# ntampellini/FIRECODE

Measured on AMD Instinct MI355X. Metric: conformer-pair RMSD alignments/s, higher is better.
Workload: dtype f64

## Files before the change

### firecode_amd/_lib.py

```python

from __future__ import annotations

import ctypes as C
import os

import numpy as np

_HERE = os.path.dirname(os.path.abspath(__file__))
LIB_PATH = os.environ.get("FC_LIB_PATH") or os.path.join(_HERE, "libfc_hip.so")

FC_OK = 0
FC_E_INVALID, FC_E_NODEVICE, FC_E_HIP, FC_E_NOMEM, FC_E_LIMIT = -1, -2, -3, -4, -5


class FirecodeHipError(RuntimeError):

    def __init__(self, code, message):
        super().__init__(f"libfc_hip error {code}: {message}")
        self.code = code


class FirecodeHipInputError(FirecodeHipError, ValueError):
    """FC_E_INVALID / FC_E_LIMIT: the arguments were rejected before any launch."""


class FirecodeHipDeviceError(FirecodeHipError):
    """FC_E_NODEVICE / FC_E_HIP / FC_E_NOMEM."""


_lib = None

_p_f64 = C.POINTER(C.c_double)
_p_i64 = C.POINTER(C.c_int64)
_p_u64 = C.POINTER(C.c_uint64)
_p_u8 = C.POINTER(C.c_uint8)
_i64 = C.c_int64
_f64 = C.c_double
_ens = C.c_void_p

_SIGNATURES = {
    "fc_abi_version": [],
    "fc_device_count": [],
    "fc_init": [C.c_int],
    "fc_shutdown": [],
    "fc_warmup": [],
    "fc_device_info": [C.c_char_p, _i64, _p_i64, _p_i64],
    "fc_ensemble_create": [_p_f64, _i64, _i64, _p_u8, C.c_int, C.POINTER(_ens)],
    "fc_ensemble_destroy": [_ens],
    "fc_ensemble_shape": [_ens, _p_i64, _p_i64],
    "fc_kabsch_rmsd_pairs": [_p_f64, _i64, _i64, _p_u8, _p_i64, _p_i64, _i64, C.c_int, _p_f64, _p_f64],
    "fc_ensemble_rmsd_pairs": [_ens, _p_i64, _p_i64, _i64, _p_f64, _p_f64],
    "fc_ensemble_rmsd_matrix": [_ens, _p_f64, _p_f64],
    "fc_ensemble_rmsd_values": [_ens, _p_f64, _p_f64],
    "fc_ensemble_rmsd_and_max_all": [_ens, _p_f64, _p_f64, _p_f64],
    "fc_bench_rmsd_and_max_all": [_ens, _i64, _p_f64, _p_f64, _p_i64],
    "fc_bench_rmsd_and_max_all_sampled": [_ens, _i64, _p_i64, _p_i64, _i64, _p_f64, _p_f64, _p_f64, _p_f64, _p_i64],
    "fc_bench_refine": [_ens, _f64, _f64, _i64, _p_f64, _p_i64],
    "fc_screen_select": [C.c_int],
    "fc_prune_conventions": [C.c_int],
    "fc_prune_similarity": [_p_f64, _i64, _i64, _p_u8, _p_f64, C.c_int, _f64, C.c_int, _f64, _f64, _p_f64, _f64, _i64,
                            _p_u8, _p_u8, _p_i64],
    "fc_alignment_matrices": [_p_f64, _p_f64, _i64, _i64, _p_f64],
    "fc_rmsd_simbits": [_ens, _f64, _f64, _p_f64, _f64, _i64, _i64, _p_u64, _p_i64],
    "fc_prune_rmsd": [_ens, _f64, _f64, _p_f64, _f64, _i64, _p_u8, _p_i64],
    "fc_prune_rmsd_host": [_p_f64, _i64, _i64, _p_u8, C.c_int, _f64, _f64, _p_f64, _f64, _i64, _p_u8, _p_i64],
    "fc_greedy_prune_from_bits": [_p_u64, _i64, _i64, _p_u8],
    "fc_prune_rmsd_begin": [_ens, _f64, _f64, _p_f64, _f64, _i64, _i64, _i64, _p_i64],
    "fc_prune_level": [_ens, _i64, _p_u8, _p_u8],
    "fc_prune_similar_pairs": [_ens, _p_u64, _i64, _p_i64],
    "fc_prune_from_pairs": [_ens, _p_u64, _i64, _i64, _p_u8],
    "fc_prune_rmsd_begin_async": [_ens, _f64, _f64, _i64, _i64, _i64],
    "fc_prune_export_pairs_dev": [_ens, C.c_void_p, _i64],
    "fc_prune_from_gathered_dev": [_ens, C.c_void_p, _i64, _i64, _i64, _p_u8, _p_i64],
    "fc_prune_from_gathered_dev_enqueue": [_ens, C.c_void_p, _i64, _i64, _i64, _i64, _i64],
    "fc_prune_collect": [_ens, _i64, _i64, _p_u8, _p_i64],
    "fc_stream_set": [C.c_void_p],
    "fc_memory_trim": [],
    "fc_host_alloc_pinned": [C.c_int64, C.POINTER(C.c_void_p)],
    "fc_host_free_pinned": [C.c_void_p],
    "fc_inertia_moments": [_p_f64, _i64, _i64, _p_f64, _p_f64],
    "fc_prune_rmsd_rot_corr": [_p_f64, _i64, _i64, _p_u8, _p_i64, _i64, _p_u8, _p_f64, C.POINTER(C.c_int32), _i64,
                               _f64, _f64, _p_f64, _f64, _i64, _p_u8, _p_u64],
    "fc_align_by_moi": [_p_f64, _i64, _i64, _p_f64, _p_f64],
    "fc_prune_moi": [_p_f64, _i64, _i64, _p_f64, _f64, _p_f64, _f64, _i64, _p_u8],
    "fc_align_to_first": [_p_f64, _i64, _i64, _p_i64, _i64, _p_f64],
    "fc_rototranslate": [_p_f64, _i64, _i64, _p_f64, _p_f64, _p_f64],
    "fc_clash_self": [_p_f64, _i64, _i64, _f64, _f64, _p_i64],
    "fc_clash_fragments": [_p_f64, _i64, _i64, _p_i64, _i64, _f64, _i64, _p_i64, _p_u8],
    "fc_clash_graph": [_p_f64, _i64, _i64, _p_u8, _f64, _p_i64],
    "fc_fitness_check": [_p_f64, _i64, _i64, _p_i64, _p_f64, _i64, _f64, _p_f64, _p_u8],
    "fc_embed_poses_clash": [_p_f64, _i64, _i64, _p_f64, _i64, _i64, _p_i64, _p_i64, _p_f64, _p_f64,
                             _p_f64, _p_f64, _i64, _f64, _i64, _p_i64, _p_u8, _p_f64],
    "fc_embed_mol_transforms": [_p_f64, _i64, _i64, _p_i64, _i64, _p_f64, _p_f64, _i64, _p_f64, _i64, _p_f64, _p_f64],
    "fc_embed_trimolecular": [C.POINTER(_p_f64), _p_i64, _p_i64, C.POINTER(_p_i64), _p_i64, _i64, _p_i64, _p_f64,
                              _p_f64, _p_f64, _p_f64, _p_u8, _p_i64, _p_f64, _p_f64, _i64, C.POINTER(C.c_int32),
                              _i64, _f64, _i64, _f64, _p_f64, _p_f64, _p_u8, _p_u8],
    "fc_embed_grid_clash": [_p_f64, _i64, _i64, _p_i64, _i64, _p_f64, _p_f64, _p_f64, _i64, _i64, _p_i64, _i64,
                            _p_f64, _p_f64, _p_f64, _i64, _p_f64, _i64, _f64, _i64, _p_u8,
                            C.POINTER(C.c_int32), _p_f64],
    "fc_embed_grid_dedupe": [_p_f64, _i64, _i64, _p_i64, _i64, _p_f64, _p_f64, _p_f64, _i64, _i64, _p_i64, _i64,
                             _p_f64, _p_f64, _p_f64, _i64, _p_f64, _i64, _f64, _i64, _f64, _p_u8, _p_u8],
    "fc_string_embed": [_p_f64, _i64, _i64, _p_f64, _p_f64, _i64, _p_f64, _i64, _i64, _p_f64, _p_f64, _i64, _p_f64, _i64,
                        _p_i64, _i64, _f64, _i64, _f64, _p_u8, _p_u8, _p_f64, _p_f64],
    "fc_torsion_scan": [_p_f64, _i64, _p_i64, _i64, _p_u8, _p_i64, _i64, _f64, _i64, _p_f64, _p_i64],
    "fc_torsion_scan_fingerprints": [_p_f64, _i64, _p_i64, _i64, _p_u8, _p_i64, _i64, _f64, _i64, _p_i64, _i64,
                                     _p_f64, _p_i64, _p_f64],
    "fc_torsion_scan_tfd": [_p_f64, _i64, _p_i64, _i64, _p_u8, _p_i64, _i64, _f64, _i64, _p_i64, _i64, _f64, _p_i64, _p_u8],
    "fc_torsion_scan_tfd_grid": [_p_f64, _i64, _p_i64, _i64, _p_u8, _p_i64, _p_i64, _f64, _i64, _p_i64, _i64, _f64, _p_i64, _p_u8],
    "fc_torsion_fingerprint": [_p_f64, _i64, _i64, _p_i64, _i64, _p_f64],
    "fc_tfd_simbits": [_p_f64, _i64, _i64, _f64, _i64, _i64, _p_u64],
    "fc_tfd_first_match": [_p_f64, _i64, _i64, _f64, _p_i64],
    "fc_tfd_ladder_from_first_match": [_p_i64, _i64, _p_u8],
    "fc_tfd_prune": [_p_f64, _i64, _i64, _f64, _p_u8],
    "fc_debug_pyset_order_ints": [_p_i64, _i64, _p_i64, _p_i64],
    "fc_debug_pyset_order_pairs": [_p_i64, _i64, _p_i64, _p_i64],
    "fc_debug_pyset_order_pairs_device": [_p_i64, _i64, _p_i64],
    "fc_debug_tfd_ladder_emulate": [_p_i64, _i64, _p_u8],
    "fc_xyz_write": [C.c_char_p, C.POINTER(C.c_char_p), _i64, _p_f64, _i64, C.c_char_p, C.c_int],
    "fc_xyz_scan": [C.c_char_p, _p_i64, _p_i64],
    "fc_cartesian_product_i64": [_p_i64, _p_i64, _i64, _p_i64],
    "fc_cartesian_product_f64": [_p_f64, _p_i64, _i64, _p_f64],
    "fc_xyz_read": [C.c_char_p, _i64, _i64, C.c_char_p, _p_f64],
    "fc_bench_prune_rmsd": [_ens, _f64, _f64, _i64, _p_f64, _p_f64, _p_u8, _p_i64],
    "fc_stream_use": [C.c_void_p],
    "fc_ensemble_twin": [_ens, C.POINTER(_ens)],
    "fc_prune_rmsd_begin_split_async": [_ens, _f64, _f64, _i64, _i64, _i64, C.c_void_p, C.c_int],
    "fc_screen_last_kind": [],
    "fc_debug_mfma_f16_model": [_i64, _p_i64, _p_f64],
    "fc_debug_h2_covariance": [_ens, _i64, _i64, C.POINTER(C.c_float), _p_f64, _p_f64],
    "fc_comm_unique_id": [_p_u8],
    "fc_comm_init": [_i64, _i64, _p_u8],
    "fc_comm_destroy": [],
    "fc_comm_info": [_p_i64, _p_i64],
    "fc_allgather_mask": [_p_u8, _i64, _p_u8],
    "fc_allgather_u8_dev": [C.c_void_p, C.c_void_p, _i64],
    "fc_comm_barrier": [],
    "fc_debug_comm_loopback": [_i64, _i64],
    "fc_prune_rmsd_sharded": [_ens, _f64, _f64, _i64, _i64, _p_u8, _p_i64],
    "fc_bench_prune_rmsd_sharded": [_ens, _f64, _f64, _i64, C.c_int, _p_f64, _p_f64, _p_u8, _p_i64],
    "fc_ensemble_select_diverse": [_ens, _i64, _i64, _f64, _p_i64, _p_f64, C.POINTER(C.c_int32), _p_f64, _p_i64],
    "fc_bench_select_diverse": [_ens, _i64, _i64, _f64, _i64, _p_f64, _p_f64, _p_i64, _p_i64, _p_i64],
    "fc_prune_rmsd_many": [C.POINTER(_ens), _i64, _f64, _f64, _i64, C.POINTER(_p_u8), _p_i64],
}

EXPORTED_SYMBOLS = tuple(_SIGNATURES) + ("fc_last_error",)


def _hip_runtime_mode():
    want = os.environ.get("FC_HIP_RUNTIME", "system")
    if want not in ("system", "torch", "auto"):
        raise FirecodeHipInputError(FC_E_INVALID, f"FC_HIP_RUNTIME={want!r}: expected 'system' or 'torch'")
    return "system" if want == "auto" else want


def _mapped_hip_runtimes():
    try:
        with open("/proc/self/maps") as fh:
            return sorted({ln.split()[-1] for ln in fh if "libamdhip64" in ln})
    except OSError:
        return []


HIP_RUNTIME = None


def _share_torch_hip_runtime():
    import importlib.util
    import sys

    mapped = _mapped_hip_runtimes()
    if "torch" in sys.modules:
        return mapped[0] if mapped else None
    try:
        spec = importlib.util.find_spec("torch")
    except (ImportError, ValueError):
        spec = None
    if spec is None or not spec.origin:
        raise FirecodeHipDeviceError(FC_E_NODEVICE, "FC_HIP_RUNTIME=torch but PyTorch is not installed")
    path = os.path.join(os.path.dirname(spec.origin), "lib", "libamdhip64.so")
    if mapped and os.path.realpath(mapped[0]) != os.path.realpath(path):
        raise FirecodeHipDeviceError(
            FC_E_NODEVICE, f"FC_HIP_RUNTIME=torch but {mapped[0]} is already mapped: a second HIP runtime "
            "in this process would see no GPU")
    if not os.path.exists(path):
        raise FirecodeHipDeviceError(FC_E_NODEVICE, f"FC_HIP_RUNTIME=torch but {path} does not exist")
    with open(path, "rb") as fh:
        if b"libamdhip64.so.7" not in fh.read():
            raise FirecodeHipDeviceError(
                FC_E_NODEVICE, f"{path} does not carry the soname libamdhip64.so.7 that libfc_hip.so binds to")
    C.CDLL(path, mode=C.RTLD_GLOBAL)
    return path


def load():
    global _lib, HIP_RUNTIME
    if _lib is not None:
        return _lib
    import sys

    mode = _hip_runtime_mode()
    if mode == "torch":
        _share_torch_hip_runtime()
    HIP_RUNTIME = "torch" if (mode == "torch" or "torch" in sys.modules) else "system"
    if not os.path.exists(LIB_PATH):
        raise FirecodeHipDeviceError(
            FC_E_NODEVICE,
            f"{LIB_PATH} is missing: build it with `python -c 'import __graft_entry__ as g; g.build()'` "
            "or `make -C firecode_amd/csrc`; firecode_amd has no CPU fallback",
        )
    lib = C.CDLL(LIB_PATH)
    for name, argtypes in _SIGNATURES.items():
        fn = getattr(lib, name)
        fn.argtypes = argtypes
        fn.restype = C.c_int
    lib.fc_last_error.argtypes = []
    lib.fc_last_error.restype = C.c_char_p
    _lib = lib
    return lib


def check(rc):
    if rc == FC_OK:
        return
    msg = load().fc_last_error().decode("utf-8", "replace")
    if rc in (FC_E_INVALID, FC_E_LIMIT):
        raise FirecodeHipInputError(rc, msg)
    raise FirecodeHipDeviceError(rc, msg)


def call(name, *args):
    check(getattr(load(), name)(*args))


def f64(a):
    return np.ascontiguousarray(a, dtype=np.float64)


def i64(a):
    return np.ascontiguousarray(a, dtype=np.int64)


def u8(a):
    return np.ascontiguousarray(a, dtype=np.uint8)


def ptr(a, ctype):
    if a is None:
        return None
    return a.ctypes.data_as(C.POINTER(ctype))


def pf(a):
    return ptr(a, C.c_double)


def pi(a):
    return ptr(a, C.c_int64)


def pb(a):
    return ptr(a, C.c_uint8)


def pw(a):
    return ptr(a, C.c_uint64)


def init(device=0):
    call("fc_init", int(device))


def shutdown():
    call("fc_shutdown")


def stream_set(hip_stream):
    call("fc_stream_set", C.c_void_p(int(hip_stream) if hip_stream else None))


def stream_use(hip_stream):
# ... 7 lines not shown
def screen_select(kind=0):
    call("fc_screen_select", int(kind))


def comm_unique_id():
    buf = np.zeros(128, dtype=np.uint8)
    call("fc_comm_unique_id", pb(buf))
    return buf.tobytes()


def comm_init(rank, world, unique_id):
    buf = np.frombuffer(bytes(unique_id), dtype=np.uint8).copy()
    if buf.shape[0] != 128:
        raise FirecodeHipInputError(FC_E_INVALID, "the RCCL unique id has 128 bytes")
    call("fc_comm_init", int(rank), int(world), pb(buf))


def comm_destroy():
    call("fc_comm_destroy")


def comm_info():
    r, w = C.c_int64(0), C.c_int64(1)
    call("fc_comm_info", C.byref(r), C.byref(w))
    return r.value, w.value


def comm_barrier():
    call("fc_comm_barrier")


def allgather_mask(mask_u8):
    m = u8(mask_u8).reshape(-1)
    _, world = comm_info()
    out = np.zeros((world, m.shape[0]), dtype=np.uint8)
    call("fc_allgather_mask", pb(m), int(m.shape[0]), pb(out))
    return out


def warmup():
    call("fc_warmup")


def memory_trim():
    call("fc_memory_trim")


def device_count():
    return int(load().fc_device_count())


def device_info():
    name = C.create_string_buffer(160)
    ncu, hbm = C.c_int64(0), C.c_int64(0)
    call("fc_device_info", name, 160, C.byref(ncu), C.byref(hbm))
    return {"name": name.value.decode(), "n_cu": ncu.value, "hbm_bytes": hbm.value}


class DeviceEnsemble:

    def __init__(self, coords, atom_mask=None, center=True):
        coords = f64(coords)
        if coords.ndim != 3 or coords.shape[2] != 3:
            raise FirecodeHipInputError(FC_E_INVALID, f"coords must be (N, A, 3), got {coords.shape}")
        self.N, self.A_all = int(coords.shape[0]), int(coords.shape[1])
        m = None if atom_mask is None else u8(np.asarray(atom_mask, dtype=bool))
        if m is not None and m.shape != (self.A_all,):
            raise FirecodeHipInputError(FC_E_INVALID, "atom_mask must have one entry per atom")
        self._h = _ens()
        call("fc_ensemble_create", pf(coords), self.N, self.A_all, pb(m), int(bool(center)), C.byref(self._h))
        self.W = (max(self.N, 1) + 63) // 64

    def close(self):
        if getattr(self, "_h", None):
            load().fc_ensemble_destroy(self._h)
            self._h = None

    def __del__(self):
        try:
            self.close()
        except Exception:
            pass

    def __enter__(self):
        return self

    def __exit__(self, *exc):
        self.close()

    @property
    def handle(self):
        if not self._h:
            raise FirecodeHipInputError(FC_E_INVALID, "ensemble already destroyed")
        return self._h

    def rmsd_pairs(self, pair_i, pair_j):
        pi_, pj_ = i64(pair_i), i64(pair_j)
        P = int(pi_.shape[0])
        r, m = np.empty(P), np.empty(P)
        call("fc_ensemble_rmsd_pairs", self.handle, pi(pi_), pi(pj_), P, pf(r), pf(m))
        return r, m

    def select_diverse(self, n_max, start=0, stop_rmsd=None):
        n_max, start = int(n_max), int(start)
        stop = -1.0 if stop_rmsd is None else float(stop_rmsd)
        if stop_rmsd is not None and not stop >= 0.0:
            raise FirecodeHipInputError(FC_E_INVALID, f"stop_rmsd={stop_rmsd!r} must be >= 0")
        cap = max(1, min(n_max, self.N))
        idx, rad = np.empty(cap, dtype=np.int64), np.empty(cap)
        lab, dist = np.empty(self.N, dtype=np.int32), np.empty(self.N)
        k = C.c_int64(0)
        call("fc_ensemble_select_diverse", self.handle, n_max, start, stop, pi(idx), pf(rad),
             ptr(lab, C.c_int32), pf(dist), C.byref(k))
        return idx[:k.value], lab, dist, rad[:k.value]

    def bench_select_diverse(self, n_max, start=0, stop_rmsd=None, reps=3):
        stop = -1.0 if stop_rmsd is None else float(stop_rmsd)
        idx = np.empty(max(1, min(int(n_max), self.N)), dtype=np.int64)
        dev, host, k, lanes = C.c_double(0), C.c_double(0), C.c_int64(0), C.c_int64(0)
        call("fc_bench_select_diverse", self.handle, int(n_max), int(start), stop, int(reps), C.byref(dev),
             C.byref(host), pi(idx), C.byref(k), C.byref(lanes))
        return dev.value, host.value, idx[:k.value], lanes.value

    def rmsd_matrix(self):
        r = np.zeros((self.N, self.N))
        m = np.zeros((self.N, self.N))
        call("fc_ensemble_rmsd_matrix", self.handle, pf(r), pf(m))
        return r, m

    def rmsd_values(self, want_matrix=True):
        r = np.zeros((self.N, self.N)) if want_matrix else None
        ms = C.c_double(0)
        call("fc_ensemble_rmsd_values", self.handle, pf(r), C.byref(ms))
        return r, ms.value

    def rmsd_and_max_all(self, want_matrices=True):
        r = np.zeros((self.N, self.N)) if want_matrices else None
        m = np.zeros((self.N, self.N)) if want_matrices else None
        ms = C.c_double(0)
        call("fc_ensemble_rmsd_and_max_all", self.handle, pf(r), pf(m), C.byref(ms))
        return r, m, ms.value

    def bench_refine(self, max_rmsd, max_dev, reps=10):
        ms, n = C.c_double(0), C.c_int64(0)
        call("fc_bench_refine", self.handle, float(max_rmsd), float(max_dev), int(reps), C.byref(ms), C.byref(n))
        return ms.value, n.value

    def bench_rmsd_and_max_all(self, reps=1):
        k, t = C.c_double(0), C.c_double(0)
        stats = np.zeros(3, dtype=np.int64)
        call("fc_bench_rmsd_and_max_all", self.handle, int(reps), C.byref(k), C.byref(t), pi(stats))
        return k.value, t.value, stats

    def bench_rmsd_and_max_all_sampled(self, pair_i, pair_j, reps=1):
        pi_, pj_ = i64(pair_i), i64(pair_j)
        P = int(pi_.shape[0])
        r, m = np.empty(P), np.empty(P)
        k, t = C.c_double(0), C.c_double(0)
        stats = np.zeros(3, dtype=np.int64)
        call("fc_bench_rmsd_and_max_all_sampled", self.handle, int(reps), pi(pi_), pi(pj_), P, pf(r), pf(m),
             C.byref(k), C.byref(t), pi(stats))
        return k.value, t.value, stats, r, m

    def simbits(self, max_rmsd, max_dev, energies=None, max_dE=0.0, row_begin=0, row_end=None):
        row_end = self.N if row_end is None else int(row_end)
        bits = np.zeros((row_end - row_begin, self.W), dtype=np.uint64)
        grey = C.c_int64(0)
        en = None if energies is None else f64(energies)
        call("fc_rmsd_simbits", self.handle, float(max_rmsd), float(max_dev), pf(en), float(max_dE),
             int(row_begin), row_end, pw(bits), C.byref(grey))
        return bits, grey.value

    def prune(self, max_rmsd, max_dev, energies=None, max_dE=0.0, min_per_group=20):
        mask = np.zeros(self.N, dtype=np.uint8)
        stats = np.zeros(6, dtype=np.int64)
        en = None if energies is None else f64(energies)
        call("fc_prune_rmsd", self.handle, float(max_rmsd), float(max_dev), pf(en), float(max_dE),
             int(min_per_group), pb(mask), pi(stats))
        return mask.astype(bool), stats

    def prune_begin(self, max_rmsd, max_dev, rank, world, row_block=128, energies=None, max_dE=0.0):
        stats = np.zeros(6, dtype=np.int64)
        en = None if energies is None else f64(energies)
        call("fc_prune_rmsd_begin", self.handle, float(max_rmsd), float(max_dev), pf(en), float(max_dE),
             int(rank), int(world), int(row_block), pi(stats))
        return stats

    def prune_level(self, k, mask_in):
        mi = u8(mask_in)
        mo = np.zeros(self.N, dtype=np.uint8)
        call("fc_prune_level", self.handle, int(k), pb(mi), pb(mo))
        return mo

    def similar_pairs(self, count_hint=None):
        n = C.c_int64(0)
        if count_hint is None:
            call("fc_prune_similar_pairs", self.handle, None, 0, C.byref(n))
            count_hint = n.value
        out = np.zeros(int(count_hint), dtype=np.uint64)
        call("fc_prune_similar_pairs", self.handle, pw(out), out.shape[0], C.byref(n))
        return out[: n.value]

    def prune_from_pairs(self, pairs, min_per_group=20):
        pairs = np.ascontiguousarray(pairs, dtype=np.uint64)
        mask = np.zeros(self.N, dtype=np.uint8)
        call("fc_prune_from_pairs", self.handle, pw(pairs), int(pairs.shape[0]), int(min_per_group), pb(mask))
        return mask.astype(bool)

    def prune_begin_async(self, max_rmsd, max_dev, rank, world, row_block=128):
        call("fc_prune_rmsd_begin_async", self.handle, float(max_rmsd), float(max_dev), int(rank), int(world),
             int(row_block))

    def prune_begin_split_async(self, max_rmsd, max_dev, rank, world, screen_stream, row_block=128, timed=True):
        call("fc_prune_rmsd_begin_split_async", self.handle, float(max_rmsd), float(max_dev), int(rank),
             int(world), int(row_block), C.c_void_p(int(screen_stream)), int(bool(timed)))

    def twin(self):
        t = getattr(self, "_twin", None)
        if t is None:
            h = _ens()
            call("fc_ensemble_twin", self.handle, C.byref(h))
            t = self._twin = _EnsembleView(self, h)
        return t

    def export_pairs_dev(self, dev_ptr, cap):
        call("fc_prune_export_pairs_dev", self.handle, C.c_void_p(int(dev_ptr)), int(cap))

    def prune_from_gathered_dev(self, dev_ptr, world, cap, min_per_group=20):
        mask = np.zeros(self.N, dtype=np.uint8)
        stats = np.zeros(6, dtype=np.int64)
        call("fc_prune_from_gathered_dev", self.handle, C.c_void_p(int(dev_ptr)), int(world), int(cap),
             int(min_per_group), pb(mask), pi(stats))
        return mask.astype(bool), stats

    def prune_from_gathered_enqueue(self, dev_ptr, world, cap, slot, n_slots, min_per_group=20):
        call("fc_prune_from_gathered_dev_enqueue", self.handle, C.c_void_p(int(dev_ptr)), int(world), int(cap),
             int(min_per_group), int(slot), int(n_slots))

    def prune_collect(self, slot, n_slots):
        mask = np.zeros(self.N, dtype=np.uint8)
        stats = np.zeros(6, dtype=np.int64)
        call("fc_prune_collect", self.handle, int(slot), int(n_slots), pb(mask), pi(stats))
        return mask.astype(bool), stats

    def prune_sharded(self, max_rmsd, max_dev, min_per_group=20, row_block=0):
        mask = np.zeros(self.N, dtype=np.uint8)
        stats = np.zeros(6, dtype=np.int64)
        call("fc_prune_rmsd_sharded", self.handle, float(max_rmsd), float(max_dev), int(min_per_group),
             int(row_block), pb(mask), pi(stats))
        return mask.astype(bool), stats

    def bench_prune_sharded(self, max_rmsd, max_dev, reps=1, overlap=True):
        mask = np.zeros(self.N, dtype=np.uint8)
        stats = np.zeros(8, dtype=np.int64)
        t_k, t_s = C.c_double(0), C.c_double(0)
        call("fc_bench_prune_rmsd_sharded", self.handle, float(max_rmsd), float(max_dev), int(reps),
             int(bool(overlap)), C.byref(t_k), C.byref(t_s), pb(mask), pi(stats))
        return t_k.value, t_s.value, mask.astype(bool), stats

    def bench_prune(self, max_rmsd, max_dev, reps=1, want_mask=True):
        mask = np.zeros(self.N, dtype=np.uint8) if want_mask else None
        stats = np.zeros(8, dtype=np.int64)
        t_k, t_s = C.c_double(0), C.c_double(0)
        call("fc_bench_prune_rmsd", self.handle, float(max_rmsd), float(max_dev), int(reps),
             C.byref(t_k), C.byref(t_s), pb(mask), pi(stats))
        return t_k.value, t_s.value, (None if mask is None else mask.astype(bool)), stats


class _EnsembleView(DeviceEnsemble):

    def __init__(self, parent, handle):
        self._parent = parent
        self._view_h = handle
        self.N, self.A_all, self.W = parent.N, parent.A_all, parent.W

    @property
    def handle(self):
        self._parent.handle
        return self._view_h

    def close(self):
        pass

    def twin(self):
        return self._parent


def prune_many(ensembles, max_rmsd, max_dev, min_per_group=20):
    n = len(ensembles)
    handles = (_ens * max(n, 1))(*[e.handle for e in ensembles])
    masks = [np.zeros(max(int(e.N), 1), dtype=np.uint8) for e in ensembles]
    ptrs = (_p_u8 * max(n, 1))(*[m.ctypes.data_as(_p_u8) for m in masks])
    survivors = np.zeros(max(n, 1), dtype=np.int64)
    call("fc_prune_rmsd_many", handles, n, float(max_rmsd), float(max_dev), int(min_per_group), ptrs,
         survivors.ctypes.data_as(_p_i64))
    return [m[: int(e.N)].astype(bool) for m, e in zip(masks, ensembles)], survivors[:n]


def unpack_bits(bits, n):
    b = np.unpackbits(bits.view(np.uint8), axis=1, bitorder="little")
    return b[:, :n].astype(bool)


def xyz_write(path, atoms, coords, label="", mode=0):
    X = f64(coords)
    if X.ndim == 2:
# ... 43 lines not shown
```

### firecode_amd/csrc/fc_api.cpp

```cpp
#include <algorithm>
#include <atomic>
#include <chrono>
#include <cmath>
#include <cstdlib>
#include <memory>

#include <map>
#include <mutex>
#include <thread>
#include "fc_common.h"
#include "fc_kabsch_math.h"

namespace fc {
struct LadderKs {
  int n;
  int64_t k[24];
};
__global__ void k_store_ladder_ks(LadderKs a, int64_t *__restrict__ out) {
  if ((int)threadIdx.x < a.n) out[threadIdx.x] = a.k[threadIdx.x];
}
}

namespace fc {

// ... 877 lines not shown
}

int fc_memory_trim(void) {
  FC_API_LOCK;
  if (ctx().ready) (void)hipStreamSynchronize(ctx().stream);
  pool_trim();
  return FC_OK;
}

int fc_host_alloc_pinned(int64_t bytes, void **out) {
  FC_API_LOCK;
  FC_REQUIRE(out != nullptr && bytes >= 0, "bad arguments");
  *out = nullptr;
  if (bytes == 0) return FC_OK;
  FC_TRY(ensure_init());
  void *p = nullptr;
  if (hipHostMalloc(&p, (size_t)bytes, hipHostMallocDefault) != hipSuccess) {
    (void)hipGetLastError();
    return set_error(FC_E_NOMEM, "hipHostMalloc of %lld bytes failed", (long long)bytes);
  }
  *out = p;
  return FC_OK;
}

int fc_host_free_pinned(void *p) {
  FC_API_LOCK;
  if (p == nullptr) return FC_OK;
  if (hipHostFree(p) != hipSuccess) return set_error(FC_E_HIP, "hipHostFree failed: %s", hipGetErrorString(hipGetLastError()));
  return FC_OK;
}

int fc_stream_set(void *hip_stream) {
  FC_API_LOCK;
  FC_TRY(ensure_init());
  Context &c = ctx();
  FC_HIP_TRY(hipStreamSynchronize(c.stream));
  c.stream = hip_stream ? static_cast<hipStream_t>(hip_stream) : c.own_stream;
  return FC_OK;
}

int fc_stream_use(void *hip_stream) {
  FC_API_LOCK;
  FC_TRY(ensure_init());
  Context &c = ctx();
  c.stream = hip_stream ? static_cast<hipStream_t>(hip_stream) : c.own_stream;
  return FC_OK;
}

int fc_device_info(char *name, int64_t name_len, int64_t *n_cu, int64_t *hbm_bytes) {
  FC_API_LOCK;
  FC_TRY(ensure_init());
  if (name && name_len > 0) std::snprintf(name, (size_t)name_len, "%s", ctx().name);
  if (n_cu) *n_cu = ctx().n_cu;
  if (hbm_bytes) *hbm_bytes = (int64_t)ctx().hbm;
  return FC_OK;
}

int fc_ensemble_create(const double *coords, int64_t N, int64_t A, const uint8_t *atom_mask,
                       int center, fc_ensemble **out) {
  FC_API_LOCK;
  FC_REQUIRE(out != nullptr, "out is NULL");
  *out = nullptr;
  FC_REQUIRE(coords != nullptr || N == 0, "coords is NULL");
  FC_REQUIRE(N >= 0 && A >= 1, "bad shape N=%lld A=%lld", (long long)N, (long long)A);
  FC_REQUIRE(A <= 32767, "A=%lld exceeds 32767 atoms", (long long)A);
  FC_TRY(ensure_init());
  std::unique_ptr<fc_ensemble> e(new (std::nothrow) fc_ensemble);
  if (!e) return set_error(FC_E_NOMEM, "host allocation failed");
  e->epoch = ctx().epoch;
  FC_TRY(ensemble_build(coords, N, A, atom_mask, center, e.get()));
  *out = e.release();
  return FC_OK;
}

int fc_ensemble_destroy(fc_ensemble *ens) {
  FC_API_LOCK;
  delete ens;
  return FC_OK;
}

int fc_ensemble_shape(const fc_ensemble *ens, int64_t *N, int64_t *A_selected) {
  FC_API_LOCK;
  FC_REQUIRE(ens != nullptr, "ens is NULL");
  if (N) *N = ens->N;
  if (A_selected) *A_selected = ens->A;
  return FC_OK;
}

int fc_ensemble_rmsd_pairs(fc_ensemble *ens, const int64_t *pair_i, const int64_t *pair_j,
                           int64_t P, double *rmsd_out, double *maxdev_out) {
  FC_API_LOCK;
  FC_REQUIRE(ens != nullptr, "ens is NULL");
  FC_REQUIRE(ens->epoch == ctx().epoch, "this ensemble was created before fc_shutdown / a device switch: create it again");
  FC_REQUIRE(P >= 0, "P < 0");
  if (P == 0) return FC_OK;
  FC_REQUIRE(pair_i && pair_j && rmsd_out && maxdev_out, "NULL pointer argument");
  for (int64_t k = 0; k < P; ++k)
    FC_REQUIRE(pair_i[k] >= 0 && pair_i[k] < ens->N && pair_j[k] >= 0 && pair_j[k] < ens->N,
               "pair %lld = (%lld, %lld) out of range [0, %lld)", (long long)k,
               (long long)pair_i[k], (long long)pair_j[k], (long long)ens->N);
  FC_TRY(ensure_init());
  DevBuf di, dj, dr, dm;
  FC_TRY(upload(di, pair_i, (size_t)P));
  FC_TRY(upload(dj, pair_j, (size_t)P));
  FC_TRY(dr.reserve((size_t)P * sizeof(double)));
  FC_TRY(dm.reserve((size_t)P * sizeof(double)));
  FC_TRY(launch_pairs_exact(ens, di.as<int64_t>(), dj.as<int64_t>(), P, dr.as<double>(),
                            dm.as<double>(), nullptr));
  FC_TRY(d2h(rmsd_out, dr.p, (size_t)P * sizeof(double)));
  FC_TRY(d2h(maxdev_out, dm.p, (size_t)P * sizeof(double)));
  return sync();
}

int fc_kabsch_rmsd_pairs(const double *coords, int64_t N, int64_t A, const uint8_t *atom_mask,
                         const int64_t *pair_i, const int64_t *pair_j, int64_t P, int center,
                         double *rmsd_out, double *maxdev_out) {
  FC_API_LOCK;
  fc_ensemble *e = nullptr;
  FC_TRY(fc_ensemble_create(coords, N, A, atom_mask, center, &e));
  const int rc = fc_ensemble_rmsd_pairs(e, pair_i, pair_j, P, rmsd_out, maxdev_out);
  fc_ensemble_destroy(e);
  return rc;
}

static bool rmsd_and_max_tiled(const fc_ensemble *ens) {
  const size_t lds_m = ((size_t)(((ens->A + 3) / 4 + 1) / 2) * 384 + 16 + 128) * sizeof(double) + 1024;
  return lds_m <= (size_t)160 * 1024 && (uint64_t)((ens->A + 3) / 4 * 4) * 3 * (uint64_t)ens->Npad < (1ull << 32);
}

static int rmsd_and_max_all(fc_ensemble *ens, double *rmsd_out, double *maxdev_out, double *ms_kernel) {
  FC_TRY(ensure_init());
  const int64_t N = ens->N;
  if (N == 0) return FC_OK;
  Context &c = ctx();
  DevBuf dr, dm;
  const size_t bytes = (size_t)N * N * sizeof(double);
  FC_TRY(dr.reserve(bytes));
  FC_TRY(dm.reserve(bytes));
  const bool tiled = rmsd_and_max_tiled(ens);
  unsigned long long cnt[16] = {0};
  if (tiled) {
    FC_TRY(ensemble_shard(ens, 0, 1, 256));
    FC_HIP_TRY(hipMemsetAsync(ens->counters.p, 0, 16 * sizeof(uint64_t), c.stream));
  } else {
    FC_HIP_TRY(hipMemsetAsync(dr.p, 0, bytes, c.stream));
    FC_HIP_TRY(hipMemsetAsync(dm.p, 0, bytes, c.stream));
  }
  FC_HIP_TRY(hipEventRecord(c.ev0, c.stream));
  if (tiled) FC_TRY(launch_rmsd_values(ens, 0.0, dr.as<double>(), dm.as<double>()));
  else FC_TRY(launch_matrix_exact(ens, dr.as<double>(), dm.as<double>()));
  FC_HIP_TRY(hipEventRecord(c.ev1, c.stream));
  if (tiled) FC_TRY(d2h(cnt, ens->counters.p, sizeof cnt));
  FC_TRY(sync());
  if (ms_kernel) {
    float ms = 0.f;
    FC_HIP_TRY(hipEventElapsedTime(&ms, c.ev0, c.ev1));
    *ms_kernel = ms;
  }
  if (tiled && cnt[6] > (unsigned long long)ens->pairq_cap) {
    FC_HIP_TRY(hipMemsetAsync(ens->counters.p, 0, 16 * sizeof(uint64_t), c.stream));
    FC_TRY(launch_rmsd_values(ens, 0.0, dr.as<double>(), dm.as<double>(), 0, 1, true));
    FC_TRY(d2h(cnt, ens->counters.p, sizeof cnt));
    FC_TRY(sync());
  }
  if (tiled && cnt[6] > (unsigned long long)ens->pairq_cap) {
    FC_HIP_TRY(hipMemsetAsync(dr.p, 0, bytes, c.stream));
    FC_HIP_TRY(hipMemsetAsync(dm.p, 0, bytes, c.stream));
    FC_TRY(launch_matrix_exact(ens, dr.as<double>(), dm.as<double>()));
  }
  if (rmsd_out) FC_TRY(launch_mirror_upper(dr.as<double>(), N));
  if (maxdev_out) FC_TRY(launch_mirror_upper(dm.as<double>(), N));
  if (rmsd_out) FC_TRY(d2h(rmsd_out, dr.p, bytes));
  if (maxdev_out) FC_TRY(d2h(maxdev_out, dm.p, bytes));
  return sync();
}

static int bench_rmsd_and_max_all(fc_ensemble *ens, int64_t reps, double *ms_kernel_mean, double *ms_total,
                                  int64_t *stats, const int64_t *sample_i = nullptr, const int64_t *sample_j = nullptr,
                                  int64_t P = 0, double *sample_rmsd = nullptr, double *sample_maxdev = nullptr) {
  FC_TRY(ensure_init());
  const int64_t N = ens->N;
  FC_REQUIRE(N >= 2, "needs at least two conformers");
  Context &c = ctx();
  DevBuf dr, dm;
  const size_t bytes = (size_t)N * N * sizeof(double);
  FC_TRY(dr.reserve(bytes));
  FC_TRY(dm.reserve(bytes));
  const bool tiled = rmsd_and_max_tiled(ens);
  const int64_t rank = comm_rank(), world = comm_world();
  FC_REQUIRE(tiled || world == 1, "structures beyond the tiled kernel are not sharded");
  if (tiled) FC_TRY(ensemble_shard(ens, 0, 1, 256));
  std::vector<hipEvent_t> &ev = c.ev_pool;
  while ((int64_t)ev.size() < 2 * reps + 2) {
    hipEvent_t e = nullptr;
    FC_HIP_TRY(hipEventCreate(&e));
    ev.push_back(e);
  }
  FC_HIP_TRY(hipEventRecord(ev[2 * reps], c.stream));
  for (int64_t r = 0; r < reps; ++r) {
    if (tiled) {
      FC_HIP_TRY(hipMemsetAsync(ens->counters.p, 0, 16 * sizeof(uint64_t), c.stream));
      FC_HIP_TRY(hipEventRecord(ev[2 * r], c.stream));
      c.mark_after_screen = ev[2 * r + 1];
      const int rc = launch_rmsd_values(ens, 0.0, dr.as<double>(), dm.as<double>(), rank, world);
      c.mark_after_screen = nullptr;
      FC_TRY(rc);
    } else {
      FC_HIP_TRY(hipEventRecord(ev[2 * r], c.stream));
      FC_TRY(launch_matrix_exact(ens, dr.as<double>(), dm.as<double>()));
      FC_HIP_TRY(hipEventRecord(ev[2 * r + 1], c.stream));
    }
  }
  FC_HIP_TRY(hipEventRecord(ev[2 * reps + 1], c.stream));
  unsigned long long cnt[16] = {0};
  if (tiled) FC_TRY(d2h(cnt, ens->counters.p, sizeof cnt));
  FC_TRY(sync());
  double sum = 0.0;
  for (int64_t r = 0; r < reps; ++r) {
    float ms = 0.f;
    FC_HIP_TRY(hipEventElapsedTime(&ms, ev[2 * r], ev[2 * r + 1]));
    sum += ms;
  }
  float tot = 0.f;
  FC_HIP_TRY(hipEventElapsedTime(&tot, ev[2 * reps], ev[2 * reps + 1]));
  if (ms_kernel_mean) *ms_kernel_mean = sum / (double)reps;
  if (ms_total) *ms_total = tot;
  if (stats) {
    int64_t own = 0;
    const int64_t nb = ceil_div(N, (int64_t)128);
    for (int64_t lb = 0, b; (b = global_block(lb, rank, world)) < nb; ++lb)
      for (int64_t i = b * 128; i < std::min<int64_t>(N, (b + 1) * 128); ++i) own += N - 1 - i;
    stats[0] = own;
    stats[1] = (int64_t)cnt[6];
    stats[2] = tiled ? 1 : 0;
  }
  if (tiled && cnt[6] > (unsigned long long)ens->pairq_cap)
    return set_error(FC_E_LIMIT, "%llu degenerate pairs exceed the fix-up queue (%lld)", cnt[6], (long long)ens->pairq_cap);
  if (P > 0) {
    DevBuf di, dj, sr, sm;
    FC_TRY(upload(di, sample_i, (size_t)P));
    FC_TRY(upload(dj, sample_j, (size_t)P));
    FC_TRY(sr.reserve((size_t)P * sizeof(double)));
    FC_TRY(sm.reserve((size_t)P * sizeof(double)));
    FC_TRY(launch_gather_matrix_pairs(dr.as<double>(), dm.as<double>(), N, di.as<int64_t>(), dj.as<int64_t>(), P,
                                      sr.as<double>(), sm.as<double>()));
    FC_TRY(d2h(sample_rmsd, sr.p, (size_t)P * sizeof(double)));
    FC_TRY(d2h(sample_maxdev, sm.p, (size_t)P * sizeof(double)));
    FC_TRY(sync());
  }
  return FC_OK;
}

static int select_diverse_checked(fc_ensemble *ens, int64_t n_max, int64_t start, double stop_rmsd, int64_t *indices_out,
                                  double *radii_out, int32_t *labels_out, double *dist_out, int64_t *n_selected,
                                  double *ms_device) {
  FC_REQUIRE(ens != nullptr, "ens is NULL");
  FC_REQUIRE(indices_out != nullptr && n_selected != nullptr, "indices_out / n_selected is NULL");
  FC_REQUIRE(n_max >= 1, "n_max=%lld < 1", (long long)n_max);
  FC_REQUIRE(!(stop_rmsd != stop_rmsd), "stop_rmsd is NaN");
  FC_REQUIRE(ens->epoch == ctx().epoch, "this ensemble was created before fc_shutdown / a device switch: create it again");
  *n_selected = 0;
  if (ens->N == 0) return FC_OK;
  FC_REQUIRE(start >= 0 && start < ens->N, "start=%lld outside [0, %lld)", (long long)start, (long long)ens->N);
  FC_REQUIRE(ens->N <= (int64_t)INT32_MAX - 256, "N=%lld: the selection indexes conformers with 32 bits", (long long)ens->N);
  FC_TRY(ensure_init());
  return select_diverse(ens, n_max, start, stop_rmsd, indices_out, radii_out, labels_out, dist_out, n_selected, ms_device);
}

int fc_ensemble_select_diverse(fc_ensemble *ens, int64_t n_max, int64_t start, double stop_rmsd, int64_t *indices_out,
                               double *radii_out, int32_t *labels_out, double *dist_out, int64_t *n_selected) {
  FC_API_LOCK;
  return select_diverse_checked(ens, n_max, start, stop_rmsd, indices_out, radii_out, labels_out, dist_out, n_selected,
                                nullptr);
}

int fc_bench_select_diverse(fc_ensemble *ens, int64_t n_max, int64_t start, double stop_rmsd, int64_t reps,
                            double *ms_device_mean, double *ms_host_mean, int64_t *indices_out, int64_t *n_selected,
                            int64_t *lanes_out) {
  FC_API_LOCK;
  FC_REQUIRE(reps >= 1 && reps <= 4096 && ms_device_mean && ms_host_mean, "bad arguments");
  double dev = 0.0, host = 0.0;
  for (int64_t r = 0; r < reps; ++r) {
    double ms = 0.0;
    const auto t0 = std::chrono::steady_clock::now();
    FC_TRY(select_diverse_checked(ens, n_max, start, stop_rmsd, indices_out, nullptr, nullptr, nullptr, n_selected, &ms));
    host += std::chrono::duration<double, std::milli>(std::chrono::steady_clock::now() - t0).count();
    dev += ms;
  }
  *ms_device_mean = dev / (double)reps;
  *ms_host_mean = host / (double)reps;
  if (lanes_out) *lanes_out = diverse_lanes(ens->N);
  return FC_OK;
}

int fc_ensemble_rmsd_matrix(fc_ensemble *ens, double *rmsd_out, double *maxdev_out) {
  FC_API_LOCK;
  FC_REQUIRE(ens && rmsd_out && maxdev_out, "NULL pointer argument");
  return rmsd_and_max_all(ens, rmsd_out, maxdev_out, nullptr);
}

int fc_ensemble_rmsd_and_max_all(fc_ensemble *ens, double *rmsd_out, double *maxdev_out, double *ms_kernel) {
  FC_API_LOCK;
  FC_REQUIRE(ens != nullptr, "ens is NULL");
  return rmsd_and_max_all(ens, rmsd_out, maxdev_out, ms_kernel);
}

int fc_bench_rmsd_and_max_all(fc_ensemble *ens, int64_t reps, double *ms_kernel_mean, double *ms_total,
                              int64_t *stats) {
  FC_API_LOCK;
  FC_REQUIRE(ens != nullptr && reps >= 1 && reps <= 4096, "bad arguments");
  return bench_rmsd_and_max_all(ens, reps, ms_kernel_mean, ms_total, stats);
}

int fc_bench_rmsd_and_max_all_sampled(fc_ensemble *ens, int64_t reps, const int64_t *pair_i, const int64_t *pair_j,
                                      int64_t P, double *rmsd_out, double *maxdev_out, double *ms_kernel_mean,
                                      double *ms_total, int64_t *stats) {
  FC_API_LOCK;
  FC_REQUIRE(ens != nullptr && reps >= 1 && reps <= 4096, "bad arguments");
  FC_REQUIRE(P >= 0 && (P == 0 || (pair_i && pair_j && rmsd_out && maxdev_out)), "NULL sample arrays");
  for (int64_t p = 0; p < P; ++p)
    FC_REQUIRE(pair_i[p] >= 0 && pair_i[p] < ens->N && pair_j[p] >= 0 && pair_j[p] < ens->N,
               "sample pair %lld out of range", (long long)p);
  return bench_rmsd_and_max_all(ens, reps, ms_kernel_mean, ms_total, stats, pair_i, pair_j, P, rmsd_out, maxdev_out);
}

int fc_ensemble_rmsd_values(fc_ensemble *ens, double *rmsd_out, double *ms_kernel) {
  FC_API_LOCK;
  FC_REQUIRE(ens != nullptr, "ens is NULL");
  FC_TRY(ensure_init());
  const int64_t N = ens->N;
  if (N == 0) return FC_OK;
  FC_TRY(ensemble_shard(ens, 0, 1, 256));
  Context &c = ctx();
  DevBuf dr;
  const size_t bytes = (size_t)N * N * sizeof(double);
  FC_TRY(dr.reserve(bytes));
  FC_HIP_TRY(hipMemsetAsync(dr.p, 0, bytes, c.stream));
  FC_HIP_TRY(hipMemsetAsync(ens->counters.p, 0, 16 * sizeof(uint64_t), c.stream));
  FC_HIP_TRY(hipEventRecord(c.ev0, c.stream));
  FC_TRY(launch_rmsd_values(ens, 0.02, dr.as<double>(), nullptr));
  FC_HIP_TRY(hipEventRecord(c.ev1, c.stream));
  unsigned long long cnt[16];
  FC_TRY(d2h(cnt, ens->counters.p, sizeof cnt));
  if (rmsd_out) {
    FC_TRY(launch_mirror_upper(dr.as<double>(), N));
    FC_TRY(d2h(rmsd_out, dr.p, bytes));
  }
  FC_TRY(sync());
  if (cnt[6] > (unsigned long long)ens->pairq_cap)
    return set_error(FC_E_LIMIT, "%llu pairs closer than 0.02 A exceed the fix-up queue (%lld): "
                     "use fc_ensemble_rmsd_matrix", cnt[6], (long long)ens->pairq_cap);
  if (ms_kernel) {
    float ms = 0.f;
    FC_HIP_TRY(hipEventElapsedTime(&ms, c.ev0, c.ev1));
    *ms_kernel = ms;
  }
  return FC_OK;
}

int fc_alignment_matrices(const double *p, const double *q, int64_t n_pairs, int64_t A,
                          double *M_out) {
  FC_API_LOCK;
  FC_REQUIRE(n_pairs >= 0 && A >= 1, "bad shape");
  if (n_pairs == 0) return FC_OK;
  FC_REQUIRE(p && q && M_out, "NULL pointer argument");
  FC_TRY(ensure_init());
  DevBuf dp, dq, dM;
  FC_TRY(upload(dp, p, (size_t)n_pairs * A * 3));
  FC_TRY(upload(dq, q, (size_t)n_pairs * A * 3));
// ... 1587 lines not shown
    c.stream = overlap ? c.s_lane[k & 1] : home;
    const bool timed = k % stride_ev == 0;
    FC_TRY(begin_split(e, max_rmsd, max_dev, rank, world, row_block, overlap ? c.s_screen : c.stream,
                       timed ? ev[2 * k] : nullptr, timed ? ev[2 * k + 1] : nullptr));
    FC_TRY(fc_prune_export_pairs_dev(e, e->msg_send.as<uint64_t>(), cap));
    FC_TRY(comm_allgather_dev(e->msg_send.p, e->msg_recv.p, (size_t)(cap + 1) * sizeof(uint64_t), (int)(k & 1)));
    FC_TRY(fc_prune_from_gathered_dev_enqueue(e, e->msg_recv.as<uint64_t>(), world, cap, min_per_group, k, steps));
  }
  c.stream = home;
  if (overlap)
    for (hipStream_t s : {c.s_lane[0], c.s_lane[1], c.s_screen}) {
      FC_HIP_TRY(hipEventRecord(ev[2 * steps + 2], s));
      FC_HIP_TRY(hipStreamWaitEvent(home, ev[2 * steps + 2], 0));
    }
  FC_HIP_TRY(hipEventRecord(ev_end, home));
  FC_HIP_TRY(hipEventSynchronize(ev_end));
  if (total_ms) {
    float t = 0.f;
    FC_HIP_TRY(hipEventElapsedTime(&t, ev_begin, ev_end));
    *total_ms = t;
  }
  if (screen_ms_mean) {
    double sum = 0.0;
    int64_t n_timed = 0;
    for (int64_t k = 0; k < steps; k += stride_ev) {
      float a = 0.f;
      FC_HIP_TRY(hipEventElapsedTime(&a, ev[2 * k], ev[2 * k + 1]));
      sum += a;
      ++n_timed;
    }
    *screen_ms_mean = sum / (double)std::max<int64_t>(n_timed, 1);
  }
  return FC_OK;
}

static int64_t owned_pairs(const fc_ensemble *ens) {
  int64_t n = 0;
  const int64_t nb = ceil_div(ens->N, ens->row_block);
  for (int64_t lb = 0, b; (b = global_block(lb, ens->rank, ens->world)) < nb; ++lb)
    for (int64_t i = b * ens->row_block; i < std::min(ens->N, (b + 1) * ens->row_block); ++i) n += ens->N - 1 - i;
  return n;
}

static int sharded_levels_fallback(fc_ensemble *ens, double max_rmsd, double max_dev, int64_t min_per_group,
                                   int64_t row_block, uint8_t *mask_out, int64_t *stats) {
  const int64_t rank = comm_rank(), world = comm_world(), N = ens->N;
  int64_t st[6] = {0};
  FC_TRY(fc_prune_rmsd_begin(ens, max_rmsd, max_dev, nullptr, 0.0, rank, world, row_block, st));
  std::vector<uint8_t> mask((size_t)N, 1), mine((size_t)N), all((size_t)N * (size_t)world);
  for (int64_t k : kLadder) {
    int64_t alive = 0;
    for (uint8_t m : mask) alive += m;
    if (!(k == 1 || min_per_group * k < alive)) continue;
    FC_TRY(fc_prune_level(ens, k, mask.data(), mine.data()));
    FC_TRY(fc_allgather_mask(mine.data(), N, all.data()));
    for (int64_t i = 0; i < N; ++i) {
      uint8_t m = 1;
      for (int64_t r = 0; r < world; ++r) m = std::min(m, all[(size_t)r * N + i]);
      mask[(size_t)i] = m;
    }
  }
  int64_t alive = 0;
  for (int64_t i = 0; i < N; ++i) {
    mask_out[i] = mask[(size_t)i];
    alive += mask[(size_t)i];
  }
  if (stats) {
    for (int k = 0; k < 5; ++k) stats[k] = st[k];
    stats[5] = alive;
  }
  return FC_OK;
}

static int sharded_collect(fc_ensemble *ens, int64_t steps, bool overlap, uint8_t *mask_out, int64_t *stats,
                           bool *all_ok, int64_t *units = nullptr) {
  const int64_t W = ens->W;
  *all_ok = true;
  int64_t survivors = 0;
  for (int64_t k = 0; k < steps; ++k)
    if (!ladder_collect(ens, k, k == steps - 1 ? mask_out : nullptr, nullptr, &survivors, nullptr)) *all_ok = false;
  if (*all_ok && stats) {
    const unsigned long long *local = static_cast<const unsigned long long *>(ctx().pinned) +
                                      (size_t)steps * (size_t)(W + 16) + (size_t)(steps - 1) * 8;
    stats[0] = owned_pairs(ens);
    stats[1] = (int64_t)local[1];
    stats[2] = (int64_t)local[2];
    stats[3] = (int64_t)local[3];
    stats[4] = 0;
    stats[5] = survivors;
  }
  (void)overlap;
  if (*all_ok && units) {
    const uint64_t *cnt_last = static_cast<const uint64_t *>(ctx().pinned) + (size_t)(steps - 1) * (size_t)(W + 16) + W;
    units[0] = (int64_t)cnt_last[13];
    units[1] = (int64_t)cnt_last[15];
  }
  return FC_OK;
}

extern "C" {

int fc_prune_rmsd_sharded(fc_ensemble *ens, double max_rmsd, double max_dev, int64_t min_per_group,
                          int64_t row_block, uint8_t *mask_out, int64_t *stats) {
  FC_API_LOCK;
  FC_REQUIRE(ens && mask_out, "NULL pointer argument");
  FC_REQUIRE(max_rmsd > 0.0 && max_dev > 0.0 && min_per_group >= 1, "bad arguments");
  FC_TRY(ensure_init());
  if (ens->N == 0) return FC_OK;
  if (row_block <= 0) row_block = default_row_block();
  bool ok = false;
  const int64_t world = comm_world();
  const int64_t cap = 1024 + 4 * ens->N / world;
  const bool device_path = (uint64_t)world * (uint64_t)cap <= kPairLadderCap && (size_t)2 * ens->W * sizeof(uint64_t) <= 60 * 1024;
  if (device_path) {
    double ms = 0.0;
    FC_TRY(sharded_pipeline(ens, 1, max_rmsd, max_dev, min_per_group, row_block, false, &ms, nullptr));
    FC_TRY(sharded_collect(ens, 1, false, mask_out, stats, &ok));
    if (ok && stats) stats[4] = (int64_t)(ms * 1e6);
  }
  if (!ok) FC_TRY(sharded_levels_fallback(ens, max_rmsd, max_dev, min_per_group, row_block, mask_out, stats));
  return FC_OK;
}

int fc_bench_prune_rmsd_sharded(fc_ensemble *ens, double max_rmsd, double max_dev, int64_t reps, int overlap,
                                double *ms_screen_kernel, double *ms_step, uint8_t *mask_out, int64_t *stats) {
  FC_API_LOCK;
  FC_REQUIRE(ens && reps >= 1 && reps <= 1024, "bad arguments");
  FC_REQUIRE(max_rmsd > 0.0 && max_dev > 0.0, "thresholds must be positive");
  FC_TRY(ensure_init());
  FC_REQUIRE(ens->N > 0, "empty ensemble");
  const int64_t row_block = default_row_block();
  double ms = 0.0, total = 0.0;
  FC_TRY(sharded_pipeline(ens, reps, max_rmsd, max_dev, 20, row_block, overlap != 0, &ms, &total));
  bool ok = false;
  std::vector<uint8_t> scratch;
  if (!mask_out) {
    scratch.resize((size_t)ens->N);
    mask_out = scratch.data();
  }
  if (stats) stats[6] = stats[7] = 0;
  FC_TRY(sharded_collect(ens, reps, overlap != 0, mask_out, stats, &ok, stats ? stats + 6 : nullptr));
  if (!ok) FC_TRY(sharded_levels_fallback(ens, max_rmsd, max_dev, 20, row_block, mask_out, stats));
  if (ms_screen_kernel) *ms_screen_kernel = ms;
  if (ms_step) *ms_step = total / (double)reps;
  return FC_OK;
}

}

extern "C" {

int fc_screen_last_kind(void) { return last_screen_kind(); }

int fc_prune_conventions(int drop_later) {
  FC_API_LOCK;
  prune_conventions_set(drop_later);
  return FC_OK;
}

int fc_debug_mfma_f16_model(int64_t trials, int64_t *flags_out, double *worst_out) {
  FC_API_LOCK;
  FC_REQUIRE(flags_out && worst_out && trials >= 0 && trials <= (1 << 24), "NULL output or trials outside 0..2^24");
  FC_TRY(ensure_init());
  return h2_model_report(trials, flags_out, worst_out);
}

int fc_debug_h2_covariance(fc_ensemble *ens, int64_t ib, int64_t jb, float *B_out, double *scale_out, double *entry_bound_out) {
  FC_API_LOCK;
  FC_REQUIRE(ens && B_out && scale_out && entry_bound_out, "NULL argument");
  FC_REQUIRE(ib >= 0 && jb >= 0 && ib % 16 == 0 && jb % 16 == 0 && ib + 16 <= ens->Npad && jb + 16 <= ens->Npad,
             "tile origin must be a multiple of 16 inside the padded ensemble");
  FC_TRY(ensure_init());
  FC_REQUIRE(ens->epoch == ctx().epoch, "ensemble belongs to a context that was shut down");
  double scale = 0.0;
  FC_TRY(ensure_h2_operands(ens, &scale));
  *scale_out = scale;
  const int64_t KS2 = (ens->A + 31) / 32;
  *entry_bound_out = kabsch_h2_entry_bound(KS2);
  if (scale == 0.0) return FC_OK;
  DevBuf out;
  FC_TRY(out.reserve(256 * 9 * sizeof(float)));
  FC_TRY(launch_h2_cov_tile(ens, ib, jb, out.as<float>()));
  FC_TRY(d2h(B_out, out.p, 256 * 9 * sizeof(float)));
  return sync();
}

int fc_screen_select(int kind) {
  FC_API_LOCK;
  FC_REQUIRE(kind == 0 || kind == 16 || kind == 32 || kind == 64, "kind must be 0 (automatic), 16, 32 or 64");
  screen_select(kind);
  return FC_OK;
}

int fc_bench_refine(fc_ensemble *ens, double max_rmsd, double max_dev, int64_t reps, double *ms_refine,
                    int64_t *n_candidates) {
  FC_API_LOCK;
  FC_REQUIRE(ens && reps >= 1 && reps <= 4096, "bad arguments");
  FC_TRY(ensure_init());
  FC_TRY(ensemble_shard(ens, 0, 1, default_row_block()));
  Context &c = ctx();
  ens->lean = true;
  FC_HIP_TRY(hipMemsetAsync(ens->counters.p, 0, kCounters * sizeof(uint64_t), c.stream));
  FC_TRY(launch_simbits_screen(ens, max_rmsd * max_rmsd + kScreenMargin));
  {
    unsigned long long h0[8] = {0};
    FC_TRY(d2h(h0, ens->counters.p, sizeof h0));
    FC_TRY(sync());
    note_candidates(ens, h0[6], ens->last_similar < 0 ? 0 : (unsigned long long)ens->last_similar);
  }
  std::vector<hipEvent_t> &ev = c.ev_pool;
  while ((int64_t)ev.size() < 2 * reps) {
    hipEvent_t e = nullptr;
    FC_HIP_TRY(hipEventCreate(&e));
    ev.push_back(e);
  }
  auto *cnt = reinterpret_cast<unsigned long long *>(ens->counters.p);
  for (int64_t r = 0; r < reps; ++r) {
    FC_HIP_TRY(hipMemsetAsync(cnt + 1, 0, 3 * sizeof(uint64_t), c.stream));
    FC_HIP_TRY(hipEventRecord(ev[2 * r], c.stream));
    FC_TRY(launch_simbits_refine(ens, max_rmsd, max_dev, nullptr, 0.0));
    FC_HIP_TRY(hipEventRecord(ev[2 * r + 1], c.stream));
  }
  unsigned long long h[32] = {0};
  FC_TRY(d2h(h, ens->counters.p, sizeof h));
  FC_TRY(sync());
  if (getenv("FC_DEBUG") && h[22])
    fprintf(stderr, "[fc] refine buckets: %llu wave-items, %llu with pairs; mean ticks (100 MHz) staging %.1f, compute %.1f\n", h[22], h[23],
            (double)h[20] / (double)h[22], (double)h[21] / (double)h[22]);
  if (getenv("FC_DEBUG") && h[27])
    fprintf(stderr, "[fc] refine buckets, wave 0 per item (%llu rounds): covariance pass %.1f ticks, polynomial + rotation %.1f, + deviation pass %.1f\n",
            h[27], (double)h[26] / (double)h[27], (double)h[24] / (double)h[27], (double)h[25] / (double)h[27]);
  double sum = 0.0;
  for (int64_t r = 0; r < reps; ++r) {
    float ms = 0.f;
    FC_HIP_TRY(hipEventElapsedTime(&ms, ev[2 * r], ev[2 * r + 1]));
    sum += ms;
  }
  if (ms_refine) *ms_refine = sum / (double)reps;
  if (n_candidates) *n_candidates = (int64_t)h[1];
  if (h[6] > (unsigned long long)ens->pairq_cap)
    return set_error(FC_E_LIMIT, "the candidate-pair queue overflowed (%llu > %lld): this probe times the pair refine only",
                     h[6], (long long)ens->pairq_cap);
  return FC_OK;
}

int fc_bench_prune_rmsd(fc_ensemble *ens, double max_rmsd, double max_dev, int64_t reps,
                        double *ms_simbits_kernel, double *ms_step, uint8_t *mask_out,
                        int64_t *stats) {
  FC_API_LOCK;
  FC_REQUIRE(ens && reps >= 1 && reps <= 4096, "bad arguments");
  FC_TRY(ensure_init());
  FC_TRY(ensemble_shard(ens, 0, 1, default_row_block()));
  static const bool two_lanes = [] {
    const char *v = getenv("FC_BENCH_LANES");
    return !(v && atoi(v) == 1);
  }();
  const bool lanes = two_lanes && reps > 1;
  const int64_t stride = ens->W + 16;
  fc_ensemble *ws[kPruneLanes] = {ens, ens, ens};
  if (lanes) {
    const bool fresh = !ens->twin || !ens->twin->twin;
    for (int l = 1; l < kPruneLanes; ++l) FC_TRY(ensemble_twin(ws[l - 1], &ws[l]));
    if (fresh) FC_TRY(prune_pipeline(ws, kPruneLanes, max_rmsd, max_dev, 20, false, stride, nullptr, nullptr));
  }
  std::vector<fc_ensemble *> work((size_t)reps);
  for (int64_t r = 0; r < reps; ++r) work[(size_t)r] = ws[lanes ? r % kPruneLanes : 0];
  double t_kernel = 0.0, total = 0.0;
  FC_TRY(prune_pipeline(work.data(), reps, max_rmsd, max_dev, 20, lanes, stride, &t_kernel, &total));
  int64_t levels = 0, survivors = 0;
  unsigned long long cnt[8] = {0};
  bool redo = false;
  for (int64_t r = 0; r < reps; ++r)
    if (!ladder_collect(ens, r, mask_out, &levels, &survivors, cnt, stride)) redo = true;
  Context &c = ctx();
  if (redo) {
    ens->lean = false;
    FC_HIP_TRY(hipMemsetAsync(ens->counters.p, 0, kCounters * sizeof(uint64_t), c.stream));
    FC_TRY(launch_simbits_screen(ens, max_rmsd * max_rmsd + kScreenMargin));
    FC_TRY(launch_simbits_refine(ens, max_rmsd, max_dev, nullptr, 0.0));
    FC_TRY(ladder_single(ens, ens->bits.as<uint64_t>(), 20, mask_out, &levels, &survivors, cnt,
                         ens->simq.as<uint64_t>(), false, true));
  }
  if (getenv("FC_DEBUG")) {
    const uint64_t *cnt_host = static_cast<const uint64_t *>(c.pinned) + (size_t)(reps - 1) * (size_t)stride + ens->W;
    fprintf(stderr, "[fc] bench prune: candidates %llu, similar %llu, screen units the subset stage queued: %llu\n",
            (unsigned long long)cnt_host[1], (unsigned long long)cnt_host[2], (unsigned long long)cnt_host[13]);
  }
  if (ms_simbits_kernel) *ms_simbits_kernel = t_kernel;
  if (ms_step) *ms_step = total / (double)reps;
  if (stats) {
    stats[0] = ens->N * (ens->N - 1) / 2;
    stats[1] = (int64_t)cnt[1];
    stats[2] = (int64_t)cnt[2];
    stats[3] = (int64_t)cnt[3];
    stats[4] = levels;
    stats[5] = survivors;
    const uint64_t *cnt_last = static_cast<const uint64_t *>(c.pinned) + (size_t)(reps - 1) * (size_t)stride + ens->W;
    stats[6] = redo ? 0 : (int64_t)cnt_last[13];
    stats[7] = redo ? 0 : (int64_t)cnt_last[15];
  }
  return FC_OK;
}

}
```

### firecode_amd/csrc/fc_common.h

```cpp
#pragma once

#include <hip/hip_runtime.h>

#include <cstdarg>
#include <cstdint>
#include <cstdio>
#include <cstring>
#include <mutex>
#include <new>
#include <string>
#include <vector>

#include "../../include/fc_hip.h"
#include "fc_tuning.h"

namespace fc {

std::string &last_error();
int set_error(int code, const char *fmt, ...);

#define FC_HIP_TRY(expr)                                                              \
  do {                                                                                \
    hipError_t _e = (expr);                                                           \
    if (_e != hipSuccess)                                                             \
// ... 71 lines not shown
inline DevArena *&thread_arena() {
  static thread_local DevArena *a = nullptr;
  return a;
}

struct DevBuf {
  void *p = nullptr;
  size_t bytes = 0;
  uint64_t epoch = 0;
  bool owned = true;
  DevBuf() = default;
  DevBuf(const DevBuf &) = delete;
  DevBuf &operator=(const DevBuf &) = delete;
  ~DevBuf() { release(); }
  void release() {
    if (p && owned) {
      if (ctx().ready && epoch == ctx().epoch) pool_give(p, bytes);
      else (void)hipFree(p);
    }
    p = nullptr;
    bytes = 0;
    owned = true;
  }
  void alias(const DevBuf &o) {
    release();
    p = o.p;
    bytes = o.bytes;
    epoch = o.epoch;
    owned = false;
  }
  int reserve(size_t n, bool any_larger = false) {
    if (n <= bytes && p) return FC_OK;
    release();
    if (n == 0) n = 8;
    if (DevArena *a = thread_arena()) {
      if (void *q = a->take(n)) {
        p = q;
        bytes = (n + 255) & ~(size_t)255;
        epoch = ctx().epoch;
        owned = false;
        return FC_OK;
      }
    }
    size_t cap = 0;
    p = pool_take(n, &cap, any_larger);
    if (!p) return set_error(FC_E_NOMEM, "device allocation of %zu bytes failed", n);
    bytes = cap;
    epoch = ctx().epoch;
    return FC_OK;
  }
  template <class T>
  T *as() const { return static_cast<T *>(p); }
};

struct ArenaScope {
  DevBuf block;
  DevArena arena;
  DevArena *prev = nullptr;
  bool active = false;
  int begin(size_t bytes) {
    prev = thread_arena();
    thread_arena() = nullptr;
    const int rc = block.reserve(bytes, true);
    if (rc != FC_OK) {
      thread_arena() = prev;
      return rc;
    }
    arena.base = static_cast<char *>(block.p), arena.size = block.bytes, arena.used = 0;
    thread_arena() = &arena;
    active = true;
    return FC_OK;
  }
  ~ArenaScope();
};

inline hipStream_t &thread_stream_override() {
  static thread_local hipStream_t s = nullptr;
  return s;
}
inline hipStream_t cur_stream() {
  hipStream_t s = thread_stream_override();
  return s ? s : ctx().stream;
}
inline ArenaScope::~ArenaScope() {
  if (!active) return;
  thread_arena() = prev;
  if (ctx().ready) (void)hipStreamSynchronize(cur_stream());
}

constexpr size_t kStagedCopyMin = (size_t)64 << 10;
#ifndef FC_RB_COLSHIFT
#define FC_RB_COLSHIFT 6
#endif
constexpr int kBucketColShift = FC_RB_COLSHIFT;
#ifndef FC_RB_ROWS
#define FC_RB_ROWS 1024
#endif
constexpr int kBucketRows = FC_RB_ROWS;
bool host_memory_is_pinned(const void *p);
bool staged_uploads();
int h2d_staged(void *dst_dev, const void *src, size_t n, hipStream_t st);
inline int h2d(void *dst, const void *src, size_t n) {
  if (n == 0) return FC_OK;
  if (n >= kStagedCopyMin && staged_uploads() && !host_memory_is_pinned(src)) return h2d_staged(dst, src, n, cur_stream());
  FC_HIP_TRY(hipMemcpyAsync(dst, src, n, hipMemcpyHostToDevice, cur_stream()));
  return FC_OK;
}
inline int d2h(void *dst, const void *src, size_t n) {
  if (n == 0) return FC_OK;
  if (n >= kStagedCopyMin && !host_memory_is_pinned(dst)) return d2h_staged(dst, src, n, cur_stream());
  FC_HIP_TRY(hipMemcpyAsync(dst, src, n, hipMemcpyDeviceToHost, cur_stream()));
  return FC_OK;
}
inline int sync() {
  FC_HIP_TRY(hipStreamSynchronize(cur_stream()));
  return FC_OK;
}
inline int check_launch(const char *what) {
  hipError_t e = hipGetLastError();
  if (e != hipSuccess) return set_error(FC_E_HIP, "launch of %s failed: %s", what, hipGetErrorString(e));
  return FC_OK;
}

inline int64_t ceil_div(int64_t a, int64_t b) { return (a + b - 1) / b; }

constexpr double kScreenMargin = 1e-6;
constexpr unsigned long long kRefineLanesMin = 1ull << 17;

constexpr size_t kCounters = 64 + 20 * 16;
constexpr int kCntLevel = 64, kCntLevelStride = 16;

__host__ __device__ inline int64_t global_block(int64_t local_block, int64_t rank, int64_t world) {
  return local_block * world + ((local_block & 1) ? (world - 1 - rank) : rank);
}
inline int64_t local_block_count(int64_t n_gblocks, int64_t rank, int64_t world) {
  int64_t n = 0;
  while (global_block(n, rank, world) < n_gblocks) ++n;
  return n;
}

}

struct fc_ensemble {
  uint64_t epoch = 0;
  int64_t N = 0, A = 0;
  int64_t Npad = 0, W = 0;
  fc::DevBuf Xs;
  fc::DevBuf Xa;
  fc::DevBuf G;
  fc::DevBuf Xsf;
  fc::DevBuf sub;
  fc::DevBuf unitq;
  bool xsf_valid = false;
  fc::DevBuf Xh;
  bool xh_valid = false;
  double xh_scale = 0.0;
  double g_max = -1.0;
  bool g_max_pending = false;
  std::vector<int32_t> sel_host;
  fc::DevBuf bits;
  fc::DevBuf cand;
  fc::DevBuf pairq;
  int64_t pairq_cap = 0;
  fc::DevBuf simq;
  fc::DevBuf bk, bk_off, bk_list, sortq;
  int64_t bk_buckets = 0;
  int64_t last_candidates = -1;
  int64_t last_similar = -1;
  fc::DevBuf bits_full;
  fc::DevBuf item_table;
  int64_t item_key[4] = {-1, -1, -1, -1}, item_total = 0;
  std::vector<uint64_t> item_host;
  fc::DevBuf gathered;
  fc::DevBuf msg_send, msg_recv;
  fc::DevBuf energies;
  fc::DevBuf maskA, maskB;
  fc::DevBuf mbits;
  fc::DevBuf ladder;
  fc::DevBuf ladder_k;
  fc::DevBuf levelmask;
  std::vector<int64_t> ladder_k_host;
  int ladder_k_n = -1;
  int64_t ladder_k_mpg = -1;
  fc::DevBuf counters;
  int64_t rank = 0, world = 1, row_block = 64;
  int64_t rows_local = 0;
  bool bits_valid = false;
  bool lean = false;
  fc_ensemble *twin = nullptr;
  fc_ensemble *head = nullptr;
  fc_ensemble() = default;
  fc_ensemble(const fc_ensemble &) = delete;
  fc_ensemble &operator=(const fc_ensemble &) = delete;
  ~fc_ensemble() { delete twin; }
};
```

### firecode_amd/csrc/fc_kabsch.hip

```cpp
#include <type_traits>

#include "fc_common.h"
#include <vector>
#include "fc_kabsch_math.h"

#include <algorithm>
#include <cstdlib>

namespace fc {

static constexpr size_t kLdsLimit = 160 * 1024;

__global__ void __launch_bounds__(256)
k_prep(const double *__restrict__ coords, int64_t N, int64_t A_all, const int32_t *__restrict__ sel,
       int64_t A, int center, int64_t Npad, double *__restrict__ Xs, double *__restrict__ G,
       double *__restrict__ Xa, unsigned long long *__restrict__ gmax_bits,
       const int32_t *__restrict__ conf_idx) {
  const int64_t n = (int64_t)blockIdx.x * blockDim.x + threadIdx.x;
  if (n >= Npad) return;
  for (int64_t a = A; a < ((A + 3) & ~(int64_t)3); ++a) {
    Xs[(a * 3 + 0) * Npad + n] = 0.0;
    Xs[(a * 3 + 1) * Npad + n] = 0.0;
    Xs[(a * 3 + 2) * Npad + n] = 0.0;
  }
// ... 372 lines not shown
  if (lane == 0) scnt[2] = (unsigned)__popcll(m);
  return;
#endif
  const unsigned n = (unsigned)__popcll(m);
  unsigned base = 0;
  if (lane == 0) base = atomicAdd(scnt, n);
  base = (unsigned)__builtin_amdgcn_readfirstlane((int)base);
  if (base + n <= (unsigned)CAP) {
    if (may) sq[base + (unsigned)__popcll(m & ((1ull << lane) - 1ull))] = ((uint64_t)i << 32) | (uint64_t)j;
  } else {
#ifndef FC_ABLATE_OVERFLOW
    push_pairs(m, may, i, j, pairq, Q, counters, lane);
#endif
  }
}

template <int WCAP>
__device__ __forceinline__ void stage_pairs_wave(uint64_t m, bool may, unsigned i, unsigned j, uint64_t *__restrict__ sq_wave,
                                                 int &n_staged, uint64_t *__restrict__ pairq, unsigned long long Q,
                                                 unsigned long long *__restrict__ counters, int lane) {
  if (m == 0) return;
  const int n = (int)__popcll(m);
  if (n_staged + n <= WCAP) {
    if (may) sq_wave[n_staged + (int)__popcll(m & ((1ull << lane) - 1ull))] = ((uint64_t)i << 32) | (uint64_t)j;
    n_staged += n;
  } else {
    push_pairs(m, may, i, j, pairq, Q, counters, lane);
  }
}

__device__ __forceinline__ void flush_pairs_wave32(const uint32_t *__restrict__ sq_wave, int n_staged, unsigned i0, unsigned j0,
                                                   uint64_t *__restrict__ pairq, unsigned long long Q,
                                                   unsigned long long *__restrict__ counters, int lane) {
  if (n_staged == 0) return;
  unsigned long long base = 0;
  if (lane == 0) base = atomicAdd(&counters[6], (unsigned long long)n_staged);
  base = __shfl(base, 0);
  for (int idx = lane; idx < n_staged; idx += 64) {
    const uint32_t e = sq_wave[idx];
    const unsigned long long slot = base + (unsigned long long)idx;
    if (slot < Q) pairq[slot] = ((uint64_t)(i0 + (e >> 6)) << 32) | (uint64_t)(j0 + (e & 63u));
  }
}
template <int WCAP>
__device__ __forceinline__ void stage_pairs_wave32(uint64_t m, bool may, unsigned i, unsigned j, unsigned i0, unsigned j0,
                                                   uint32_t *__restrict__ sq_wave, int &n_staged,
                                                   uint64_t *__restrict__ pairq, unsigned long long Q,
                                                   unsigned long long *__restrict__ counters, int lane) {
  if (m == 0) return;
  const int n = (int)__popcll(m);
  if (n > WCAP) {
    push_pairs(m, may, i, j, pairq, Q, counters, lane);
    return;
  }
  if (n_staged + n > WCAP) {
    flush_pairs_wave32(sq_wave, n_staged, i0, j0, pairq, Q, counters, lane);
    n_staged = 0;
  }
  if (may) sq_wave[n_staged + (int)__popcll(m & ((1ull << lane) - 1ull))] = ((i - i0) << 6) | (j - j0);
  n_staged += n;
}

template <bool USE_LDS, int TI, int NW>
__global__ void __launch_bounds__(NW * 64)
k_simbits_screen(const double *__restrict__ Xs, const double *__restrict__ G, int64_t N,
                 int64_t Npad, int A, double A_thr2, int IB, int64_t rank, int64_t world,
                 uint64_t *__restrict__ bits, int64_t W, uint32_t *__restrict__ cand,
                 unsigned long long *__restrict__ counters, uint64_t *__restrict__ pairq,
                 unsigned long long Q) {
  extern __shared__ double lds[];
  const int tid = threadIdx.x;
  const int lane = tid & 63;
  const int wv = __builtin_amdgcn_readfirstlane(tid >> 6);
  const int64_t jt = blockIdx.x;
  const int64_t lb = blockIdx.y;
  const int64_t gb = global_block(lb, rank, world);
  const int64_t i0 = gb * IB;
  if (i0 >= N) return;
  if (jt * 64 + 63 <= i0) return;
  const int64_t j = jt * 64 + lane;

  if (USE_LDS) {
    const int total = A * 3 * 64;
    for (int idx = tid; idx < total; idx += NW * 64) {
      const int ac = idx >> 6, l = idx & 63;
      lds[idx] = Xs[(int64_t)ac * Npad + jt * 64 + l];
    }
    __syncthreads();
  }
  const double Gq = G[j];
  const double *__restrict__ xq = Xs + jt * 64 + lane;

  for (int it = wv; it * TI < IB; it += NW) {
    const int64_t ib = i0 + (int64_t)it * TI;
    if (ib >= N) break;
    if (jt * 64 + 63 <= ib) break;
    double acc[TI][9];
#pragma unroll
    for (int k = 0; k < TI; ++k)
#pragma unroll
      for (int e = 0; e < 9; ++e) acc[k][e] = 0.0;

    const double *__restrict__ xp = Xs + ib;
#pragma unroll 2
    for (int a = 0; a < A; ++a) {
      double qx, qy, qz;
      if (USE_LDS) {
        qx = lds[(a * 3 + 0) * 64 + lane];
        qy = lds[(a * 3 + 1) * 64 + lane];
        qz = lds[(a * 3 + 2) * 64 + lane];
      } else {
        qx = xq[(int64_t)(a * 3 + 0) * Npad];
        qy = xq[(int64_t)(a * 3 + 1) * Npad];
        qz = xq[(int64_t)(a * 3 + 2) * Npad];
      }
      const double *__restrict__ px = xp + (int64_t)(a * 3 + 0) * Npad;
      const double *__restrict__ py = xp + (int64_t)(a * 3 + 1) * Npad;
      const double *__restrict__ pz = xp + (int64_t)(a * 3 + 2) * Npad;
#pragma unroll
      for (int k = 0; k < TI; ++k) {
        const double x = px[k], y = py[k], z = pz[k];
        acc[k][0] = fma(x, qx, acc[k][0]);
        acc[k][1] = fma(x, qy, acc[k][1]);
        acc[k][2] = fma(x, qz, acc[k][2]);
        acc[k][3] = fma(y, qx, acc[k][3]);
        acc[k][4] = fma(y, qy, acc[k][4]);
        acc[k][5] = fma(y, qz, acc[k][5]);
        acc[k][6] = fma(z, qx, acc[k][6]);
        acc[k][7] = fma(z, qy, acc[k][7]);
        acc[k][8] = fma(z, qz, acc[k][8]);
      }
    }
#pragma unroll
    for (int k = 0; k < TI; ++k) {
      const int64_t i = ib + k;
      const double Gp = G[i];
      bool may = kabsch_may_be_below(acc[k], Gp + Gq, A_thr2);
      may = may && (j > i) && (j < N) && (i < N);
      const uint64_t word = __ballot(may);
      push_pairs(word, may, (unsigned)i, (unsigned)j, pairq, Q, counters, lane);
      if (lane == 0 && i < N) {
        const int64_t lrow = (int64_t)(lb * IB) + (int64_t)it * TI + k;
        bits[lrow * W + jt] = word;
        if (word) {
          const unsigned long long slot = atomicAdd(&counters[4], 1ull);
          cand[slot] = (uint32_t)(lrow * W + jt);
        }
      }
    }
  }
}

typedef double d4_t __attribute__((ext_vector_type(4)));

template <int NW, int MODE = 0, int TC = 64, bool EIG = false>
__global__ void __launch_bounds__(NW * 64, 2)
k_simbits_screen_mfma(const double *__restrict__ Xs, const double *__restrict__ G, int64_t N,
                      int64_t Npad, int A, double A_thr2, int IB, int64_t rank, int64_t world,
                      uint64_t *__restrict__ bits, int64_t W, uint32_t *__restrict__ cand,
                      unsigned long long *__restrict__ counters, uint64_t *__restrict__ pairq,
                      unsigned long long Q, const uint64_t *__restrict__ item_table, unsigned long long n_items,
                      double *__restrict__ rmsd_out = nullptr, const unsigned long long *__restrict__ gate = nullptr,
                      double *__restrict__ maxdev_out = nullptr) {
  static_assert(!EIG || MODE == 2, "EIG: the complete alignments");
  constexpr bool VALUES = MODE != 0;
  constexpr int NT = MODE == 2 ? 1 : 2;
  static_assert(TC == 64 || ((TC == 32 || TC == 16) && MODE == 2), "column tiles: 64, or 32 / 16 for the complete alignments");
  constexpr int NU = (TC / 16) / NT;
  constexpr int KPR = TC == 64 ? 2 : 4;
  constexpr int SST = 2048 / TC;
  constexpr int CST = TC == 64 ? 256 : 128;
  auto koff = [](int sl) { return TC == 16 ? (sl >> 1) * 384 + (sl & 1) * 64 : sl * (12 * TC); };
  if (gate != nullptr && *gate == 0ull) return;
  extern __shared__ double lds[];
  const int tid = threadIdx.x;
  const int lane = tid & 63;
  const int wv = __builtin_amdgcn_readfirstlane(tid >> 6);
  const int KS = (A + 3) >> 2;
  double *__restrict__ ldsG = lds + (TC == 16 ? ((KS + 1) >> 1) * 384 : KS * 12 * TC);
  uint64_t *__restrict__ stageQ = reinterpret_cast<uint64_t *>(ldsG + TC + IB);
  uint32_t *__restrict__ stageW = reinterpret_cast<uint32_t *>(stageQ + kStagePairs);
  unsigned *__restrict__ stageN = reinterpret_cast<unsigned *>(stageW + kStageWords);
#ifdef FC_TIMELINE
  unsigned long long *tl = reinterpret_cast<unsigned long long *>(rmsd_out);
#endif
  const unsigned long long b = blockIdx.x;
  if (b >= n_items) return;
#ifdef FC_TIMELINE
  if (!VALUES && tl && tid == 0) {
    tl[(size_t)b * 4] = wall_clock64();
    tl[(size_t)b * 4 + 3] = b;
  }
#endif
  int64_t jt, lb;
  int it_first = 0, it_last = IB >> 4;
  if (item_table != nullptr) {
    const uint64_t it = item_table[b];
    lb = (int64_t)((it >> 32) & 0x7fffffffull);
    jt = (int64_t)(it & 0x7fffffffull);
    if (it & (1ull << 31)) it_last = IB >> 5;
    if (it & (1ull << 63)) it_first = IB >> 5;
  } else {
    const int64_t NT = Npad / TC;
    jt = (int64_t)(b % (unsigned long long)NT);
    lb = (int64_t)(b / (unsigned long long)NT);
  }
  const int64_t j0 = jt * TC;
  const int64_t i0 = global_block(lb, rank, world) * IB;
  if (i0 >= N) return;
  if (j0 + TC - 1 <= i0) return;
  uint32_t *__restrict__ sq32_wave = reinterpret_cast<uint32_t *>(stageQ) + wv * (kStagePairs * 2 / NW);
  int n_staged32 = 0;
  (void)sq32_wave;
  (void)n_staged32;

  {
    const int n_runs = TC == 64 ? KS * 6 : (TC == 32 ? KS * 3 : ((KS + 1) >> 1) * 3);
    const int cs_l = TC == 64 ? lane >> 4 : lane >> 5, k1_l = TC == 64 ? (lane >> 3) & 1 : (lane >> 3) & 3, c15_l = (lane & 7) * 2;
    for (int q = wv; q < n_runs; q += NW) {
      const int sc = TC == 64 ? q >> 1 : q, kh = TC == 64 ? q & 1 : 0;
      const int sg = sc / 3, c = sc - sg * 3;
      int a = sg * 4 + kh * 2 + k1_l;
      if (TC == 16) {
        a = (sg * 2 + cs_l) * 4 + k1_l;
        a = a < KS * 4 ? a : KS * 4 - 1;
      }
      const double *src = Xs + (int64_t)(a * 3 + c) * Npad + j0 + (TC == 16 ? 0 : cs_l * 16) + c15_l;
      __builtin_amdgcn_global_load_lds((const __attribute__((address_space(1))) void *)src,
                                       (__attribute__((address_space(3))) void *)(lds + q * 128), 16, 0, 0);
    }
    for (int idx = tid; idx < TC + IB; idx += NW * 64) {
      const int64_t g = idx < TC ? j0 + idx : i0 + (idx - TC);
      ldsG[idx] = g < Npad ? G[g] : 0.0;
    }
    if (tid < kStagePairs) stageQ[tid] = ~0ull;
    if (tid < kStageWords) stageW[tid] = ~0u;
    if (tid < 2) stageN[tid] = 0u;
    __syncthreads();
#ifdef FC_TIMELINE
    if (!VALUES && tl && tid == 0) tl[(size_t)b * 4 + 1] = wall_clock64();
#endif
  }
  const int kq = lane >> 4, l15 = lane & 15;
  const int lcol = MODE == 2 ? 4 * (l15 & 3) + (l15 >> 2) : l15;
  const int boff = (kq / KPR) * 128 + (kq % KPR) * 16 + lcol;
  uint16_t *bits16 = reinterpret_cast<uint16_t *>(bits);

  double a0[3], a1[3], a2[3];
  int pre_it = -1;
  auto row_offsets = [&](int it_, unsigned (&vo)[3]) {
    const int64_t ib_ = i0 + (int64_t)it_ * 16;
#pragma unroll
    for (int c = 0; c < 3; ++c) vo[c] = (unsigned)(((int64_t)(kq * 3 + c) * Npad + ib_ + l15) * 8);
  };
  auto fetch_a_at = [&](double (&a)[3], unsigned (&vo)[3], int sx) {
    const int sl = sx < KS ? sx : KS - 1;
    const char *__restrict__ xs_s = reinterpret_cast<const char *>(Xs + (int64_t)sl * 12 * Npad);
#pragma unroll
    for (int c = 0; c < 3; ++c) {
      asm volatile("" : "+v"(vo[c]));
      a[c] = *reinterpret_cast<const double *>(xs_s + vo[c]);
    }
  };

  for (int it = it_first + wv; it < it_last; it += NW) {
    const int64_t ib = i0 + (int64_t)it * 16;
    if (ib >= N) break;
    if (j0 + TC - 1 <= ib) break;
    const int64_t lrow0 = lb * IB + (int64_t)it * 16;
    unsigned nz = 0;
    unsigned voff[3];
    row_offsets(it, voff);

#pragma unroll 1
    for (int half = 0; half < NU; ++half) {
      const int cs0 = half * NT;
      if (j0 + (cs0 + NT) * 16 - 1 <= ib) {
        if (!VALUES && lane < 16 && ib + lane < N) {
          bits16[((lrow0 + lane) * W + jt) * 4 + cs0] = 0;
          bits16[((lrow0 + lane) * W + jt) * 4 + cs0 + 1] = 0;
        }
        continue;
      }
      d4_t acc[NT][9];

      const double *__restrict__ lb0 = lds + cs0 * SST + boff;
      double b0[NT][3], b1[NT][3];
      const int KSe = KS;
      auto fetch_a = [&](double (&a)[3], int sx) {
        fetch_a_at(a, voff, sx);
      };
      auto fetch_b = [&](double (&b)[NT][3], int sx) {
        const int sl = sx < KS ? sx : KS - 1;
        const double *__restrict__ lb_s = lb0 + koff(sl);
#pragma unroll
        for (int t = 0; t < NT; ++t)
#pragma unroll
          for (int c = 0; c < 3; ++c) b[t][c] = lb_s[c * CST + t * SST];
      };
      auto mma = [&](const double (&a)[3], const double (&b)[NT][3], auto first_) {
        constexpr bool first = decltype(first_)::value;
#pragma unroll
        for (int x = 0; x < 3; ++x)
#pragma unroll
          for (int y = 0; y < 3; ++y)
#pragma unroll
            for (int t = 0; t < NT; ++t) {
              const d4_t c_in = first ? d4_t{0.0, 0.0, 0.0, 0.0} : acc[t][x * 3 + y];
              acc[t][x * 3 + y] = MODE == 2 ? __builtin_amdgcn_mfma_f64_16x16x4f64(b[t][y], a[x], c_in, 0, 0, 0)
                                            : __builtin_amdgcn_mfma_f64_16x16x4f64(a[x], b[t][y], c_in, 0, 0, 0);
            }
      };
      if (pre_it != it) {
        fetch_a_at(a0, voff, 0);
        fetch_a_at(a1, voff, 1);
        fetch_a_at(a2, voff, 2);
      }
      fetch_b(b0, 0);
      fetch_b(b1, 1);
#define FC_KSTEP(AX, BX, U)             \
  if (sgrp + (U) < KSe) {               \
    mma(AX, BX, std::false_type{});     \
    fetch_a(AX, sgrp + (U) + 3);        \
    fetch_b(BX, sgrp + (U) + 2);        \
  }
      mma(a0, b0, std::true_type{});
      fetch_a(a0, 3);
      fetch_b(b0, 2);
      for (int sgrp = 1; sgrp < KSe; sgrp += 6) {
        FC_KSTEP(a1, b1, 0)
        FC_KSTEP(a2, b0, 1)
        FC_KSTEP(a0, b1, 2)
        FC_KSTEP(a1, b0, 3)
        FC_KSTEP(a2, b1, 4)
        FC_KSTEP(a0, b0, 5)
      }
#undef FC_KSTEP
      {
        const int nit = half < NU - 1 ? it : it + NW;
        const bool more = half < NU - 1 || ((nit < it_last) && (i0 + (int64_t)nit * 16 < N) &&
                                        !(j0 + TC - 1 <= i0 + (int64_t)nit * 16));
        if (more) {
          unsigned vn[3];
          row_offsets(nit, vn);
          fetch_a_at(a0, vn, 0);
          fetch_a_at(a1, vn, 1);
          fetch_a_at(a2, vn, 2);
          pre_it = nit;
        } else {
          pre_it = -1;
        }
      }
      const int n32 = (int)N, ib32 = (int)ib;
#pragma unroll
      for (int t = 0; t < NT; ++t) {
        const int cs = cs0 + t;
        const int j = (int)j0 + cs * 16 + l15;
        const double Gq = ldsG[cs * 16 + l15];
        uint64_t mr[4] = {0, 0, 0, 0};
        if (MODE == 2) {
          const int i = ib32 + l15;
          const int jb = (int)j0 + cs * 16 + 4 * kq;
          const double Gp = ldsG[TC + it * 16 + l15];
          double nR[4][9];
          bool ok4[4];
          double msdA4[4] = {0.0, 0.0, 0.0, 0.0};
          {
            double B4[4][9], GG[4], Q44[4][4], nq4[4], lam4[4];
#pragma unroll
            for (int r = 0; r < 4; ++r) {
              GG[r] = Gp + ldsG[cs * 16 + 4 * kq + r];
#pragma unroll
              for (int e = 0; e < 9; ++e) B4[r][e] = acc[t][e][r];
            }
            kabsch_quaternion_qcp_lean4(B4, GG, Q44, nq4, ok4, EIG ? lam4 : nullptr);
            if constexpr (EIG) {
              const double k_small = 2e-10 / (double)A;
#pragma unroll
              for (int r = 0; r < 4; ++r) {
                msdA4[r] = GG[r] - 2.0 * lam4[r];
                if (!(msdA4[r] > k_small * GG[r] * GG[r])) ok4[r] = false, msdA4[r] = 0.0;
              }
            }
#pragma unroll
            for (int r = 0; r < 4; ++r) {
              if (!ok4[r]) Q44[r][0] = 1.0, Q44[r][1] = 0.0, Q44[r][2] = 0.0, Q44[r][3] = 0.0, nq4[r] = 1.0;
              neg_rotation_from_raw_quaternion(Q44[r], nq4[r], nR[r]);
            }
          }
          typedef double d2_t __attribute__((ext_vector_type(2)));
          const double *__restrict__ qcol = lds + cs * SST + 4 * kq;
          const double *__restrict__ prow_u = Xs + ib;
          const unsigned l15u = (unsigned)l15;
          const int n_rounds = (A + 1) >> 1, n_groups = n_rounds >> 1;
          const bool odd_round = (n_rounds & 1) != 0;
          double ssq[4] = {0.0, 0.0, 0.0, 0.0}, mx[4] = {0.0, 0.0, 0.0, 0.0};
          const int64_t Npad3 = 3 * Npad;
          const double *__restrict__ pa0 = prow_u, *__restrict__ pa1 = prow_u + Npad, *__restrict__ pa2 = prow_u + 2 * Npad;
          const double *__restrict__ qg = qcol;
          auto load_pq = [&](auto u_, double (&P)[3], d2_t (&Qv)[3][2]) {
            constexpr int u = decltype(u_)::value;
            const double *__restrict__ ql = qg + (u / KPR) * 128 + (u % KPR) * 16;
#pragma unroll
            for (int c = 0; c < 3; ++c) {
              Qv[c][0] = *reinterpret_cast<const d2_t *>(ql + c * CST);
              Qv[c][1] = *reinterpret_cast<const d2_t *>(ql + c * CST + 2);
            }
            P[0] = pa0[l15u];
            P[1] = pa1[l15u];
            P[2] = pa2[l15u];
            pa0 += Npad3;
            pa1 += Npad3;
            pa2 += Npad3;
          };
          auto accumulate = [&](const double (&P)[3], const d2_t (&Qv)[3][2]) {
#pragma clang fp contract(fast)
#pragma unroll
            for (int r = 0; r < 4; ++r) {
              const double qx = Qv[0][r >> 1][r & 1], qy = Qv[1][r >> 1][r & 1], qz = Qv[2][r >> 1][r & 1];
              const double dx = fma(nR[r][0], qx, fma(nR[r][1], qy, fma(nR[r][2], qz, P[0])));
              const double dy = fma(nR[r][3], qx, fma(nR[r][4], qy, fma(nR[r][5], qz, P[1])));
              const double dz = fma(nR[r][6], qx, fma(nR[r][7], qy, fma(nR[r][8], qz, P[2])));
              const double s2 = fma(dz, dz, fma(dy, dy, dx * dx));
              if constexpr (!EIG) ssq[r] += s2;
              asm("v_max_f64 %0, %1, %2" : "=v"(mx[r]) : "v"(mx[r]), "v"(s2));
            }
          };
          using U0 = std::integral_constant<int, 0>;
          using U1 = std::integral_constant<int, 1>;
          using U2 = std::integral_constant<int, 2>;
          using U3 = std::integral_constant<int, 3>;
          double PA[3], PB[3];
          d2_t QA[3][2], QB[3][2];
          load_pq(U0{}, PA, QA);
          for (int g = 0; g < n_groups; ++g) {
            load_pq(U1{}, PB, QB);
            __builtin_amdgcn_sched_barrier(0);
            accumulate(PA, QA);
            __builtin_amdgcn_sched_barrier(0);
            load_pq(U2{}, PA, QA);
            __builtin_amdgcn_sched_barrier(0);
            accumulate(PB, QB);
            __builtin_amdgcn_sched_barrier(0);
            load_pq(U3{}, PB, QB);
            __builtin_amdgcn_sched_barrier(0);
            accumulate(PA, QA);
            __builtin_amdgcn_sched_barrier(0);
            qg = TC == 16 ? qcol + koff(g + 1) : qg + 12 * TC;
            if (g + 1 < n_groups || odd_round) load_pq(U0{}, PA, QA);
            __builtin_amdgcn_sched_barrier(0);
            accumulate(PB, QB);
            __builtin_amdgcn_sched_barrier(0);
          }
          if (odd_round) {
            load_pq(U1{}, PB, QB);
            __builtin_amdgcn_sched_barrier(0);
            accumulate(PA, QA);
            __builtin_amdgcn_sched_barrier(0);
            accumulate(PB, QB);
          }
          if constexpr (EIG) {
#pragma unroll
            for (int r = 0; r < 4; ++r) ssq[r] = msdA4[r];
          }
          const bool row_in = i < n32;
          double *__restrict__ ro = rmsd_out + (int64_t)i * N + jb;
          double *__restrict__ mo = maxdev_out + (int64_t)i * N + jb;
          const double invA = 1.0 / (double)A;
          if (row_in && jb > i && jb + 3 < n32 && ((((int64_t)i * N) & 1) == 0)) {
            *reinterpret_cast<d2_t *>(ro) = d2_t{fc_sqrt_nonneg(ssq[0] * invA), fc_sqrt_nonneg(ssq[1] * invA)};
            *reinterpret_cast<d2_t *>(ro + 2) = d2_t{fc_sqrt_nonneg(ssq[2] * invA), fc_sqrt_nonneg(ssq[3] * invA)};
            *reinterpret_cast<d2_t *>(mo) = d2_t{fc_sqrt_nonneg(mx[0]), fc_sqrt_nonneg(mx[1])};
            *reinterpret_cast<d2_t *>(mo + 2) = d2_t{fc_sqrt_nonneg(mx[2]), fc_sqrt_nonneg(mx[3])};
          } else {
#pragma unroll
            for (int r = 0; r < 4; ++r) {
              const int j = jb + r;
              if (row_in && j >= i && j < n32) {
                ro[r] = j == i ? 0.0 : fc_sqrt_nonneg(ssq[r] * invA);
                mo[r] = j == i ? 0.0 : fc_sqrt_nonneg(mx[r]);
              }
            }
          }
#pragma unroll
          for (int r = 0; r < 4; ++r) {
            const int j = jb + r;
            const bool redo = row_in && (j > i) && (j < n32) && !ok4[r];
            stage_pairs(__ballot(redo), redo, (unsigned)i, (unsigned)j, stageQ, stageN, pairq, Q, counters, lane);
          }
          continue;
        }
#pragma unroll
        for (int r = 0; r < 4; ++r) {
          const int i = ib32 + kq + 4 * r;
          const double Gp = ldsG[TC + it * 16 + kq + 4 * r];
          double B9[9];
#pragma unroll
          for (int e = 0; e < 9; ++e) B9[e] = acc[t][e][r];
          if (VALUES) {
            const double lam = kabsch_lambda_max(B9, Gp + Gq);
            const double msdA = (Gp + Gq) - 2.0 * lam;
            const bool in = (j > i) && (j < n32) && (i < n32);
            if (in) rmsd_out[(int64_t)i * N + j] = sqrt(fmax(msdA, 0.0) / (double)A);
            const bool redo = in && (msdA < A_thr2);
            stage_pairs(__ballot(redo), redo, (unsigned)i, (unsigned)j, stageQ, stageN, pairq, Q, counters, lane);
            continue;
          }
          bool may = kabsch_may_be_below(B9, Gp + Gq, A_thr2);
          may = may && (j > i) && (j < n32) && (i < n32);
          mr[r] = __ballot(may);
          if constexpr (MODE == 0)
            stage_pairs_wave32<kStagePairs * 2 / NW>(mr[r], may, (unsigned)i, (unsigned)j, (unsigned)i0, (unsigned)j0, sq32_wave,
                                                     n_staged32, pairq, Q, counters, lane);
          else
            stage_pairs(mr[r], may, (unsigned)i, (unsigned)j, stageQ, stageN, pairq, Q, counters, lane);
        }
        if (!VALUES && lane < 16 && ib32 + lane < n32) {
          const int rr = lane >> 2;
          const uint64_t mine = rr == 0 ? mr[0] : rr == 1 ? mr[1] : rr == 2 ? mr[2] : mr[3];
          const unsigned piece = (unsigned)((mine >> (16 * (lane & 3))) & 0xffffull);
          bits16[((lrow0 + lane) * W + jt) * 4 + cs] = (uint16_t)piece;
          nz |= piece;
        }
      }
    }
    if (!VALUES) {
#ifndef FC_ABLATE_PUSH
      const bool has = lane < 16 && nz != 0;
      const uint64_t mw = __ballot(has);
      if (mw != 0) {
        const unsigned n = (unsigned)__popcll(mw);
        const uint32_t word = (uint32_t)((lrow0 + lane) * W + jt);
        unsigned base = 0;
        if (lane == 0) base = atomicAdd(stageN + 1, n);
        base = (unsigned)__builtin_amdgcn_readfirstlane((int)base);
        const unsigned rank_in = (unsigned)__popcll(mw & ((1ull << lane) - 1ull));
        if (base + n <= (unsigned)kStageWords) {
          if (has) stageW[base + rank_in] = word;
        } else {
          unsigned long long gbase = 0;
          if (lane == 0) gbase = atomicAdd(&counters[4], (unsigned long long)n);
          gbase = __shfl(gbase, 0);
          if (has) cand[gbase + rank_in] = word;
        }
      }
#endif
    }
  }
  if constexpr (MODE == 0) flush_pairs_wave32(sq32_wave, n_staged32, (unsigned)i0, (unsigned)j0, pairq, Q, counters, lane);
  __syncthreads();
#ifdef FC_TIMELINE
  if (!VALUES && tl && tid == 0) tl[(size_t)b * 4 + 2] = wall_clock64();
#endif
  if (wv == 0) {
    if constexpr (MODE != 0) {
      const uint64_t e = lane < kStagePairs ? stageQ[lane] : ~0ull;
      const bool valid = e != ~0ull;
      const uint64_t mv = __ballot(valid);
      if (mv != 0) {
        unsigned long long gbase = 0;
        if (lane == 0) gbase = atomicAdd(&counters[6], (unsigned long long)__popcll(mv));
        gbase = __shfl(gbase, 0);
        if (valid) {
          const unsigned long long slot = gbase + (unsigned long long)__popcll(mv & ((1ull << lane) - 1ull));
          if (slot < Q) pairq[slot] = e;
        }
      }
    }
    if (!VALUES) {
      const uint32_t wq = lane < kStageWords ? stageW[lane] : ~0u;
      const bool valid = wq != ~0u;
      const uint64_t mv = __ballot(valid);
      if (mv != 0) {
        unsigned long long gbase = 0;
        if (lane == 0) gbase = atomicAdd(&counters[4], (unsigned long long)__popcll(mv));
        gbase = __shfl(gbase, 0);
        if (valid) cand[gbase + (unsigned long long)__popcll(mv & ((1ull << lane) - 1ull))] = wq;
      }
    }
  }
}

typedef float f4_t __attribute__((ext_vector_type(4)));

#ifndef FC_F32_WGS
#define FC_F32_WGS 3
#endif
template <int NW, bool BITS = true, bool STAGED = false, int TC = 64>
__global__ void __launch_bounds__(NW * 64, FC_F32_WGS)
k_simbits_screen_mfma_f32(const float *__restrict__ Xsf, const double *__restrict__ G, int64_t N,
                          int64_t Npad, int A, double A_thr2, KabschF32Bounds bd, int IB, int64_t rank,
                          int64_t world, uint64_t *__restrict__ bits, int64_t W, uint32_t *__restrict__ cand,
                          unsigned long long *__restrict__ counters, uint64_t *__restrict__ pairq,
                          unsigned long long Q, const uint64_t *__restrict__ item_table,
                          unsigned long long n_items, const float *__restrict__ sub, KabschF32Bounds bd1,
                          float inv_AS, uint64_t *__restrict__ unitq, int part, int gate) {
  if ((gate == 1 && counters[15] != 0ull) || (gate == 2 && counters[15] == 0ull)) return;
  extern __shared__ double lds_raw[];
  float *__restrict__ lds = reinterpret_cast<float *>(lds_raw);
  static_assert(TC == 64 || (TC == 32 && !BITS && !STAGED), "32-column tiles: lean single-stage launches only");
  const int tid = threadIdx.x;
  const int lane = tid & 63;
  const int wv = __builtin_amdgcn_readfirstlane(tid >> 6);
  const int KS = (A + 3) >> 2;
  constexpr bool two = STAGED;
  static_assert(!(STAGED && BITS), "the subset stage belongs to the lean kernel");
  const float half_A_thr2 = (float)(0.5 * A_thr2);
  float *__restrict__ ldsG = lds + KS * 12 * TC;
  float *__restrict__ ldsS = ldsG + TC + IB;
  uint64_t *__restrict__ stageQ = reinterpret_cast<uint64_t *>(ldsS + (two ? (TC + IB) * 5 : 0));
  uint32_t *__restrict__ stageW = reinterpret_cast<uint32_t *>(stageQ + kStagePairsF32);
  unsigned *__restrict__ stageN = reinterpret_cast<unsigned *>(stageW + kStageWordsF32);
// ... 1733 lines not shown
      pair_exact(Xs, Npad, A, i, j, r, m);
      sim = (r < max_rmsd) && (m < max_dev);
      grey = (fabs(r - max_rmsd) < 1e-9) || (r < max_rmsd && fabs(m - max_dev) < 1e-9);
      if (energies != nullptr) sim = sim && (fabs(energies[i] - energies[j]) < max_dE);
    }
    out = __ballot(sim);
    g = __ballot(grey);
  }
  if (lane == 0) {
    bits[lrow * W + jt] = out;
    atomicAdd(&counters[1], (unsigned long long)__popcll(word));
    atomicAdd(&counters[2], (unsigned long long)__popcll(out));
    if (g) atomicAdd(&counters[3], (unsigned long long)__popcll(g));
  }
  }
}

__global__ void __launch_bounds__(64)
k_align_to_first(const double *__restrict__ coords, int64_t N, int64_t A,
                 const int64_t *__restrict__ idx, int64_t n_idx, double *__restrict__ out) {
  const int64_t t = (int64_t)blockIdx.x * blockDim.x + threadIdx.x;
  if (t >= N) return;
  const double *ref = coords;
  const double *tgt = coords + t * A * 3;
  double rc[3] = {0, 0, 0}, tc[3] = {0, 0, 0};
  for (int64_t k = 0; k < n_idx; ++k) {
    const int64_t a = idx ? idx[k] : k;
    for (int c = 0; c < 3; ++c) {
      rc[c] += ref[a * 3 + c];
      tc[c] += tgt[a * 3 + c];
    }
  }
  for (int c = 0; c < 3; ++c) {
    rc[c] /= (double)n_idx;
    tc[c] /= (double)n_idx;
  }
  double R[9] = {1, 0, 0, 0, 1, 0, 0, 0, 1};
  if (t != 0) {
    double B[9] = {0, 0, 0, 0, 0, 0, 0, 0, 0};
    for (int64_t k = 0; k < n_idx; ++k) {
      const int64_t a = idx ? idx[k] : k;
      const double px = ref[a * 3 + 0] - rc[0], py = ref[a * 3 + 1] - rc[1], pz = ref[a * 3 + 2] - rc[2];
      const double qx = tgt[a * 3 + 0] - tc[0], qy = tgt[a * 3 + 1] - tc[1], qz = tgt[a * 3 + 2] - tc[2];
      B[0] = fma(px, qx, B[0]); B[1] = fma(px, qy, B[1]); B[2] = fma(px, qz, B[2]);
      B[3] = fma(py, qx, B[3]); B[4] = fma(py, qy, B[4]); B[5] = fma(py, qz, B[5]);
      B[6] = fma(pz, qx, B[6]); B[7] = fma(pz, qy, B[7]); B[8] = fma(pz, qz, B[8]);
    }
    (void)kabsch_rotation(B, R);
  }
  double *o = out + t * A * 3;
  for (int64_t a = 0; a < A; ++a) {
    const double x = tgt[a * 3 + 0] - tc[0], y = tgt[a * 3 + 1] - tc[1], z = tgt[a * 3 + 2] - tc[2];
    o[a * 3 + 0] = R[0] * x + R[1] * y + R[2] * z;
    o[a * 3 + 1] = R[3] * x + R[4] * y + R[5] * z;
    o[a * 3 + 2] = R[6] * x + R[7] * y + R[8] * z;
  }
}

__global__ void __launch_bounds__(64)
k_alignment_matrices(const double *__restrict__ p, const double *__restrict__ q, int64_t n,
                     int64_t A, double *__restrict__ M) {
  const int64_t k = (int64_t)blockIdx.x * blockDim.x + threadIdx.x;
  if (k >= n) return;
  const double *pp = p + k * A * 3, *qq = q + k * A * 3;
  double B[9] = {0, 0, 0, 0, 0, 0, 0, 0, 0};
  for (int64_t a = 0; a < A; ++a) {
    const double px = pp[a * 3], py = pp[a * 3 + 1], pz = pp[a * 3 + 2];
    const double qx = qq[a * 3], qy = qq[a * 3 + 1], qz = qq[a * 3 + 2];
    B[0] = fma(px, qx, B[0]); B[1] = fma(px, qy, B[1]); B[2] = fma(px, qz, B[2]);
    B[3] = fma(py, qx, B[3]); B[4] = fma(py, qy, B[4]); B[5] = fma(py, qz, B[5]);
    B[6] = fma(pz, qx, B[6]); B[7] = fma(pz, qy, B[7]); B[8] = fma(pz, qz, B[8]);
  }
  double R[9];
  (void)kabsch_rotation(B, R);
  for (int e = 0; e < 9; ++e) M[k * 9 + e] = R[e];
}

__global__ void __launch_bounds__(256)
k_rmsd_fix_small(const double *__restrict__ Xa, int A, int64_t N, const uint64_t *__restrict__ pairq,
                 const unsigned long long *__restrict__ counters, unsigned long long Q,
                 double *__restrict__ rmsd_out, double *__restrict__ maxdev_out) {
  const int lane = threadIdx.x & 63, sub = lane & 7, slot = lane >> 3;
  const int64_t wave0 = ((int64_t)blockIdx.x * blockDim.x + threadIdx.x) >> 6;
  const int64_t nwaves = ((int64_t)gridDim.x * blockDim.x) >> 6;
  unsigned long long n = counters[6];
  if (n > Q) n = Q;
  for (int64_t base = wave0 * 8; base < (int64_t)n; base += nwaves * 8) {
    const int64_t p = base + slot;
    if (p < (int64_t)n) {
      const uint64_t e = pairq[p];
      const int64_t i = (int64_t)(e >> 32), j = (int64_t)(e & 0xffffffffull);
      double r, m;
      pair_exact_group8(Xa, A, i, j, sub, r, m);
      if (sub == 0) {
        rmsd_out[i * N + j] = r;
        if (maxdev_out) maxdev_out[i * N + j] = m;
      }
    }
  }
}

__global__ void __launch_bounds__(256)
k_scatter_pairs(const uint64_t *__restrict__ pairs, int64_t n_pairs, int64_t N, int64_t W,
                uint64_t *__restrict__ bits) {
  const int64_t p = (int64_t)blockIdx.x * blockDim.x + threadIdx.x;
  if (p >= n_pairs) return;
  const uint64_t e = pairs[p];
  const int64_t i = (int64_t)(e >> 32), j = (int64_t)(e & 0xffffffffull);
  if (i < 0 || j <= i || j >= N) return;
  atomicOr(reinterpret_cast<unsigned long long *>(&bits[i * W + (j >> 6)]), 1ull << (j & 63));
}

static int screen_item_table(fc_ensemble *e, int64_t NT, int64_t n_lblocks, bool halves = true, int64_t tc = 64) {
  const int64_t rb_key = (e->row_block * 2 + (halves ? 1 : 0)) * 128 + tc;
  if (e->item_key[0] == e->N && e->item_key[1] == e->rank && e->item_key[2] == e->world &&
      e->item_key[3] == rb_key)
    return FC_OK;
  e->item_total = 0;
  e->item_key[0] = e->N; e->item_key[1] = e->rank; e->item_key[2] = e->world; e->item_key[3] = rb_key;
  if (e->row_block % tc != 0) return FC_OK;
  const int64_t r = e->row_block / tc;
  std::vector<uint64_t> items;
  for (int64_t l = 0; l < n_lblocks; ++l) {
    const int64_t first = r * global_block(l, e->rank, e->world);
    for (int64_t jt = first; jt < NT; ++jt) items.push_back(((uint64_t)l << 32) | (uint64_t)jt);
  }
  {
    int64_t tail = 2 * (int64_t)ctx().n_cu;
    if (const char *v = getenv("FC_SCREEN_TAIL_SLOTS")) tail = std::strtoll(v, nullptr, 10);
    if (halves && e->row_block == 128 && tail > 0 && (int64_t)items.size() > 4 * tail && e->A <= 52) {
      std::vector<uint64_t> halves;
      for (int64_t k = (int64_t)items.size() - tail; k < (int64_t)items.size(); ++k) {
        halves.push_back(items[(size_t)k] | (1ull << 31));
        halves.push_back(items[(size_t)k] | (1ull << 63));
      }
      items.resize(items.size() - (size_t)tail);
      items.insert(items.end(), halves.begin(), halves.end());
    }
  }
  if (items.empty() || items.size() >= (1ull << 31)) return FC_OK;
  FC_TRY(e->item_table.reserve(items.size() * sizeof(uint64_t)));
  e->item_host.swap(items);
  FC_TRY(h2d(e->item_table.p, e->item_host.data(), e->item_host.size() * sizeof(uint64_t)));
  e->item_total = (int64_t)e->item_host.size();
  return FC_OK;
}

int prebuild_screen_items(fc_ensemble *e) {
  const int64_t n_lblocks = local_block_count(ceil_div(e->N, e->row_block), e->rank, e->world);
  if (n_lblocks <= 0 || (e->Npad >> 6) == 0) return FC_OK;
  return screen_item_table(e, e->Npad >> 6, n_lblocks, true, 64);
}

template <int NW, int TC, bool EIG>
static int launch_complete_variant(fc_ensemble *e, dim3 grid, size_t lds_m, double A_small, int64_t rb, int64_t rank, int64_t world,
                                   unsigned long long *cnt, const uint64_t *item_table_dev, unsigned long long n_items,
                                   double *rmsd_dev, double *maxdev_dev) {
  if (lds_m > 64 * 1024) {
    hipError_t err = hipFuncSetAttribute(reinterpret_cast<const void *>(k_simbits_screen_mfma<NW, 2, TC, EIG>),
                                         hipFuncAttributeMaxDynamicSharedMemorySize, (int)lds_m);
    if (err != hipSuccess) return set_error(FC_E_HIP, "hipFuncSetAttribute failed: %s", hipGetErrorString(err));
  }
  hipLaunchKernelGGL((k_simbits_screen_mfma<NW, 2, TC, EIG>), grid, dim3(NW * 64), lds_m, ctx().stream, e->Xs.as<double>(),
                     e->G.as<double>(), e->N, e->Npad, (int)e->A, A_small, (int)rb, rank, world, nullptr, e->W, nullptr, cnt,
                     e->pairq.as<uint64_t>(), (unsigned long long)e->pairq_cap, item_table_dev, n_items, rmsd_dev, nullptr,
                     maxdev_dev);
  return FC_OK;
}

int launch_rmsd_values(fc_ensemble *e, double small_rmsd, double *rmsd_dev, double *maxdev_dev, int64_t rank,
                       int64_t world, bool explicit_sum) {
  const int64_t rb = 128;
  const int64_t n_lblocks = local_block_count(ceil_div(e->N, rb), rank, world);
  if (n_lblocks <= 0) return FC_OK;
  const size_t lds_64 = ((size_t)((e->A + 3) / 4) * 4 * 3 * 64 + 64 + (size_t)rb) * sizeof(double) + kStageBytes;
  const size_t lds_32 = ((size_t)((e->A + 3) / 4) * 4 * 3 * 32 + 32 + (size_t)rb) * sizeof(double) + kStageBytes;
  const size_t lds_16 = ((size_t)(((e->A + 3) / 4 + 1) / 2) * 384 + 16 + (size_t)rb) * sizeof(double) + kStageBytes;
  const bool narrow = lds_64 > kLdsLimit && maxdev_dev != nullptr;
  const int64_t tc = !narrow ? 64 : (lds_32 <= kLdsLimit ? 32 : 16);
  const size_t lds_m = tc == 64 ? lds_64 : (tc == 32 ? lds_32 : lds_16);
  const int64_t NT = e->Npad / tc;
  if (lds_m > kLdsLimit || NT == 0)
    return set_error(FC_E_LIMIT, "A=%lld atoms exceed the LDS column tile of the value kernel", (long long)e->A);
  const bool fits32 = (uint64_t)((e->A + 3) / 4 * 4) * 3 * (uint64_t)e->Npad < (1ull << 32) &&
                      96 * (uint64_t)e->Npad < (1ull << 32);
  if (!fits32) return set_error(FC_E_LIMIT, "ensemble too large for 32-bit operand offsets");
  auto *cnt = reinterpret_cast<unsigned long long *>(e->counters.p);
  const bool two_blocks = 2 * lds_m <= kLdsLimit;
  const bool complete = maxdev_dev != nullptr;
  const void *fn = two_blocks ? reinterpret_cast<const void *>(k_simbits_screen_mfma<4, 1>)
                              : reinterpret_cast<const void *>(k_simbits_screen_mfma<8, 1>);
  if (!complete && lds_m > 64 * 1024) {
    hipError_t err = hipFuncSetAttribute(fn, hipFuncAttributeMaxDynamicSharedMemorySize, (int)lds_m);
    if (err != hipSuccess) return set_error(FC_E_HIP, "hipFuncSetAttribute failed: %s", hipGetErrorString(err));
  }
  const double A_small = (double)e->A * small_rmsd * small_rmsd;
  const int64_t saved_rank = e->rank, saved_world = e->world, saved_rb = e->row_block;
  e->rank = rank; e->world = world; e->row_block = rb;
  const int rc_tbl = screen_item_table(e, NT, n_lblocks, true, tc);
  e->rank = saved_rank; e->world = saved_world; e->row_block = saved_rb;
  e->item_key[3] = -1;
  if (rc_tbl != FC_OK) return rc_tbl;
  const int compact = e->item_total > 0 ? 1 : 0;
  const unsigned long long n_items =
      compact ? (unsigned long long)e->item_total : (unsigned long long)NT * (unsigned long long)n_lblocks;
  const uint64_t *item_table_dev = compact ? e->item_table.as<uint64_t>() : nullptr;
  if (n_items >= (1ull << 31)) return set_error(FC_E_LIMIT, "too many value-kernel items for one launch");
  const dim3 grid((unsigned)n_items);
#define FC_LAUNCH_VALUES(NW_, MODE_)                                                                      \
  hipLaunchKernelGGL((k_simbits_screen_mfma<NW_, MODE_>), grid, dim3(NW_ * 64), lds_m, ctx().stream,      \
                     e->Xs.as<double>(), e->G.as<double>(), e->N, e->Npad, (int)e->A, A_small, (int)rb,   \
                     rank, world, nullptr, e->W, nullptr, cnt, e->pairq.as<uint64_t>(),                   \
                     (unsigned long long)e->pairq_cap, item_table_dev, n_items, rmsd_dev, nullptr, maxdev_dev)
  const char *eig_env = getenv("FC_COMPLETE_EIG");
  const bool eig = complete && !(eig_env && atoi(eig_env) == 0) && !explicit_sum;
#define FC_LAUNCH_COMPLETE(NW_, TC_)                                                                                        \
  FC_TRY((eig ? launch_complete_variant<NW_, TC_, true>(e, grid, lds_m, A_small, rb, rank, world, cnt, item_table_dev, n_items, \
                                                       rmsd_dev, maxdev_dev)                                               \
              : launch_complete_variant<NW_, TC_, false>(e, grid, lds_m, A_small, rb, rank, world, cnt, item_table_dev,     \
                                                        n_items, rmsd_dev, maxdev_dev)))
  if (narrow && tc == 32) {
    FC_LAUNCH_COMPLETE(8, 32);
  } else if (narrow) {
    FC_LAUNCH_COMPLETE(8, 16);
  } else if (complete) {
    if (two_blocks) FC_LAUNCH_COMPLETE(4, 64);
    else FC_LAUNCH_COMPLETE(8, 64);
  } else {
    if (two_blocks) FC_LAUNCH_VALUES(4, 1);
    else FC_LAUNCH_VALUES(8, 1);
  }
#undef FC_LAUNCH_COMPLETE
#undef FC_LAUNCH_VALUES
  FC_TRY(check_launch("k_simbits_screen_mfma<values>"));
  if (ctx().mark_after_screen) (void)hipEventRecord(ctx().mark_after_screen, ctx().stream);
  hipLaunchKernelGGL(k_rmsd_fix_small, dim3((unsigned)(ctx().n_cu * 4)), dim3(256), 0, ctx().stream,
                     e->Xa.as<double>(), (int)e->A, e->N, e->pairq.as<uint64_t>(), cnt,
                     (unsigned long long)e->pairq_cap, rmsd_dev, maxdev_dev);
  return check_launch("k_rmsd_fix_small");
}

__global__ void __launch_bounds__(256)
k_gather_matrix_pairs(const double *__restrict__ rmsd_m, const double *__restrict__ maxdev_m, int64_t N,
                      const int64_t *__restrict__ pi, const int64_t *__restrict__ pj, int64_t P,
                      double *__restrict__ rmsd_out, double *__restrict__ maxdev_out) {
  const int64_t p = (int64_t)blockIdx.x * blockDim.x + threadIdx.x;
  if (p >= P) return;
  int64_t i = pi[p], j = pj[p];
  if (i > j) { const int64_t t = i; i = j; j = t; }
  rmsd_out[p] = rmsd_m[i * N + j];
  maxdev_out[p] = maxdev_m[i * N + j];
}

int launch_gather_matrix_pairs(const double *rmsd_m, const double *maxdev_m, int64_t N, const int64_t *pi_dev,
                               const int64_t *pj_dev, int64_t P, double *rmsd_out, double *maxdev_out) {
  if (P == 0) return FC_OK;
  hipLaunchKernelGGL(k_gather_matrix_pairs, dim3((unsigned)ceil_div(P, 256)), dim3(256), 0, ctx().stream, rmsd_m,
                     maxdev_m, N, pi_dev, pj_dev, P, rmsd_out, maxdev_out);
  return check_launch("k_gather_matrix_pairs");
}

__global__ void __launch_bounds__(256)
k_mirror_upper(double *__restrict__ m, int64_t N) {
  __shared__ double tile[32][33];
  const int64_t bi = blockIdx.y, bj = blockIdx.x;
  if (bj < bi) return;
  const int tx = threadIdx.x & 31, ty = threadIdx.x >> 5;
  for (int r = ty; r < 32; r += 8) {
    const int64_t i = bi * 32 + r, j = bj * 32 + tx;
    tile[r][tx] = (i < N && j < N) ? m[i * N + j] : 0.0;
  }
  __syncthreads();
  for (int r = ty; r < 32; r += 8) {
    const int64_t j = bj * 32 + r, i = bi * 32 + tx;
    if (i < N && j < N && j > i) m[j * N + i] = tile[tx][r];
  }
}

int launch_mirror_upper(double *m_dev, int64_t N) {
  if (N < 2) return FC_OK;
  const unsigned nb = (unsigned)ceil_div(N, 32);
  hipLaunchKernelGGL(k_mirror_upper, dim3(nb, nb), dim3(256), 0, ctx().stream, m_dev, N);
  return check_launch("k_mirror_upper");
}

int launch_scatter_pairs(const uint64_t *pairs_dev, int64_t n_pairs, int64_t N, int64_t W,
                         uint64_t *bits_dev) {
  if (n_pairs == 0) return FC_OK;
  hipLaunchKernelGGL(k_scatter_pairs, dim3((unsigned)ceil_div(n_pairs, 256)), dim3(256), 0,
                     ctx().stream, pairs_dev, n_pairs, N, W, bits_dev);
  return check_launch("k_scatter_pairs");
}

int launch_prep_begin(fc_ensemble *e) {
  auto *gmax_bits = reinterpret_cast<unsigned long long *>(e->counters.p) + (kCounters - 1);
  FC_HIP_TRY(hipMemsetAsync(gmax_bits, 0, sizeof(unsigned long long), ctx().stream));
  e->xsf_valid = false;
  e->xh_valid = false;
  e->g_max = -1.0;
  return FC_OK;
}
bool prep_by_tiles(int64_t A_all) {
  const size_t lds_tile = (size_t)kPrepTile * (size_t)(A_all * 3 + 1) * sizeof(double) + (size_t)A_all * sizeof(int) + 8;
  return lds_tile + 2048 <= kLdsLimit && (uint64_t)kPrepTile * (uint64_t)(A_all * 3 + 1) < (1ull << 31) &&
         !getenv("FC_PREP_LANES");
}
int launch_prep_tiles(const double *coords_dev, int64_t N, int64_t A_all, const int32_t *sel_dev, int64_t A, int center,
                      fc_ensemble *e, const int32_t *conf_idx_dev, int64_t tile0, int64_t n_tiles) {
  if (n_tiles <= 0) return FC_OK;
  auto *gmax_bits = reinterpret_cast<unsigned long long *>(e->counters.p) + (kCounters - 1);
  constexpr int64_t kPer64 = 64 / kPrepTile;
  const size_t lds_tile = (size_t)kPrepTile * (size_t)(A_all * 3 + 1) * sizeof(double) + (size_t)A_all * sizeof(int) + 8;
  if (lds_tile > 64 * 1024)
    FC_HIP_TRY(hipFuncSetAttribute(reinterpret_cast<const void *>(k_prep_tile<kPrepTile>),
                                   hipFuncAttributeMaxDynamicSharedMemorySize, (int)lds_tile));
  hipLaunchKernelGGL(k_prep_tile<kPrepTile>, dim3((unsigned)(n_tiles * kPer64)), dim3(256), lds_tile, ctx().stream, coords_dev, N,
                     A_all, sel_dev, A, center, e->Npad, e->Xs.as<double>(), e->G.as<double>(), e->Xa.as<double>(), gmax_bits,
                     conf_idx_dev, tile0 * kPer64);
  return check_launch("k_prep_tile");
}
int launch_prep_body(const double *coords_dev, int64_t N, int64_t A_all, const int32_t *sel_dev, int64_t A, int center,
                     fc_ensemble *e, const int32_t *conf_idx_dev);
int launch_prep(const double *coords_dev, int64_t N, int64_t A_all, const int32_t *sel_dev,
                int64_t A, int center, fc_ensemble *e, const int32_t *conf_idx_dev) {
  FC_TRY(launch_prep_begin(e));
  return launch_prep_body(coords_dev, N, A_all, sel_dev, A, center, e, conf_idx_dev);
}
int launch_prep_body(const double *coords_dev, int64_t N, int64_t A_all, const int32_t *sel_dev, int64_t A, int center,
                     fc_ensemble *e, const int32_t *conf_idx_dev) {
  if (prep_by_tiles(A_all))
    return launch_prep_tiles(coords_dev, N, A_all, sel_dev, A, center, e, conf_idx_dev, 0, e->Npad / 64);
  auto *gmax_bits = reinterpret_cast<unsigned long long *>(e->counters.p) + (kCounters - 1);
  const int64_t blocks = ceil_div(e->Npad, 256);
  hipLaunchKernelGGL(k_prep, dim3((unsigned)blocks), dim3(256), 0, ctx().stream, coords_dev, N,
                     A_all, sel_dev, A, center, e->Npad, e->Xs.as<double>(), e->G.as<double>(),
                     e->Xa.as<double>(), gmax_bits, conf_idx_dev);
  return check_launch("k_prep");
}

int launch_pairs_exact(const fc_ensemble *e, const int64_t *pi_dev, const int64_t *pj_dev,
                       int64_t P, double *rmsd_dev, double *maxdev_dev, double *R_dev) {
  if (P == 0) return FC_OK;
  hipLaunchKernelGGL(k_pairs_exact, dim3((unsigned)ceil_div(P, 256)), dim3(256), 0, ctx().stream,
                     e->Xa.as<double>(), (int)e->A, pi_dev, pj_dev, P, rmsd_dev, maxdev_dev, R_dev);
  return check_launch("k_pairs_exact");
}

int launch_matrix_exact(const fc_ensemble *e, double *rmsd_dev, double *maxdev_dev) {
  const int64_t waves = e->N * (e->Npad >> 6);
  if (waves == 0) return FC_OK;
  hipLaunchKernelGGL(k_matrix_exact, dim3((unsigned)ceil_div(waves, 4)), dim3(256), 0,
                     ctx().stream, e->Xs.as<double>(), e->N, e->Npad, (int)e->A, rmsd_dev,
                     maxdev_dev);
  return check_launch("k_matrix_exact");
}


static int g_last_screen = 0;
int last_screen_kind() { return g_last_screen; }
static int g_screen_forced = 0;
void screen_select(int kind) { g_screen_forced = kind; }

int h2_model_ok(bool *ok);

static int ensure_h2_operands_upto(fc_ensemble *e, double *scale_out, int64_t max_ks2) {
  *scale_out = 0.0;
  const int64_t KS2 = (e->A + 31) / 32, A4 = (e->A + 3) / 4 * 4;
  if (KS2 > max_ks2 || (uint64_t)(24 * KS2) * (uint64_t)e->Npad >= (1ull << 32)) return FC_OK;
  if (!(e->g_max > 0.0) || !std::isfinite(e->g_max)) return FC_OK;
  int ex = 0;
  (void)std::frexp(std::sqrt(e->g_max), &ex);
  const double scale = std::ldexp(1.0, 13 - ex);
  if (!e->xh_valid || e->xh_scale != scale) {
    FC_TRY(e->Xh.reserve((size_t)KS2 * 24 * (size_t)e->Npad * 16));
    hipLaunchKernelGGL(k_f64_to_h2, dim3((unsigned)ceil_div(e->Npad, 256), (unsigned)(KS2 * 12)), dim3(256), 0, ctx().stream,
                       e->Xs.as<double>(), e->Npad, (int)A4, (int)KS2, scale, e->Xh.as<h8_t>());
    FC_TRY(check_launch("k_f64_to_h2"));
    e->xh_valid = true;
    e->xh_scale = scale;
  }
  *scale_out = scale;
  return FC_OK;
}
int ensure_h2_operands(fc_ensemble *e, double *scale_out) { return ensure_h2_operands_upto(e, scale_out, kH2MaxKS2); }

int launch_simbits_screen(fc_ensemble *e, double thr2_margin) {
  bool marked = false;
  auto mark_main = [&]() {
    if (!marked && ctx().mark_after_screen) (void)hipEventRecord(ctx().mark_after_screen, ctx().stream);
    if (!marked && ctx().after_main_stream && ctx().after_main_event) {
      (void)hipEventRecord(ctx().after_main_event, ctx().stream);
      (void)hipStreamWaitEvent(ctx().after_main_stream, ctx().after_main_event, 0);
      ctx().stream = ctx().after_main_stream;
    }
    marked = true;
  };
  const int64_t NT = e->Npad >> 6;
  const int64_t n_gblocks = ceil_div(e->N, e->row_block);
  const int64_t n_lblocks = local_block_count(n_gblocks, e->rank, e->world);
  if (n_lblocks <= 0 || NT == 0) {
    mark_main();
    return FC_OK;
  }
  const double A_thr2 = (double)e->A * thr2_margin;
  const size_t lds = (size_t)e->A * 3 * 64 * sizeof(double);
  dim3 grid((unsigned)NT, (unsigned)n_lblocks);
  const char *cfg = getenv("FC_SCREEN_CFG");
  const bool want_valu = cfg && std::strncmp(cfg, "valu", 4) == 0;
  const bool alt = cfg && std::strcmp(cfg, "valu4x8") == 0;
  {
    const int64_t KS2n = (e->A + 31) / 32;
    static const int h2_env_n = [] {
      const char *v = getenv("FC_SCREEN_H2");
      return v ? atoi(v) : 1;
    }();
    const char *f32_env_n = getenv("FC_SCREEN_F32");
    const size_t lds_n = (size_t)KS2n * 24 * 512 + (32 + (size_t)e->row_block) * sizeof(float) + kStageBytesF32;
    if (!want_valu && e->lean && KS2n > kH2MaxKS2 && KS2n <= 13 && h2_env_n != 0 && (g_screen_forced == 0 || g_screen_forced == 16) &&
        !(f32_env_n && f32_env_n[0] == '0') && e->row_block % 32 == 0 && lds_n <= kLdsLimit &&
        (uint64_t)(24 * KS2n) * (uint64_t)e->Npad < (1ull << 32)) {
      if (e->g_max < 0.0) {
        auto *cnt_max = reinterpret_cast<unsigned long long *>(e->counters.p) + (kCounters - 1);
        FC_HIP_TRY(hipMemsetAsync(cnt_max, 0, sizeof(unsigned long long), ctx().stream));
        hipLaunchKernelGGL(k_max_nonneg, dim3((unsigned)std::min<int64_t>(ceil_div(e->Npad, 256), 256)), dim3(256), 0, ctx().stream,
                           e->G.as<double>(), e->Npad, cnt_max);
        FC_TRY(check_launch("k_max_nonneg"));
        unsigned long long bits_max = 0;
        FC_TRY(d2h(&bits_max, cnt_max, sizeof bits_max));
        FC_TRY(sync());
        FC_HIP_TRY(hipMemsetAsync(cnt_max, 0, sizeof(unsigned long long), ctx().stream));
        std::memcpy(&e->g_max, &bits_max, sizeof(double));
      }
      bool model_ok = false;
      FC_TRY(h2_model_ok(&model_ok));
      double scale_n = 0.0;
      if (model_ok) FC_TRY(ensure_h2_operands_upto(e, &scale_n, 13));
      const KabschF32Bounds bdn = kabsch_h2_bounds(KS2n);
      const double s2 = scale_n * scale_n;
      const float hthr = (float)(0.5 * A_thr2 * s2);
      static const double kBandMaxN = [] {
        const char *v = getenv("FC_SCREEN_BAND_MAX");
        const double x = v ? atof(v) : 4.0;
        return x > 0.0 ? x : 4.0;
      }();
      const double band = (double)bdn.p0 * 2.0 * e->g_max / (double)e->A;
      const bool band_ok = g_screen_forced == 16 || (f32_env_n && (f32_env_n[0] == '2' || f32_env_n[0] == '3')) || band <= kBandMaxN * thr2_margin;
      if (scale_n > 0.0 && std::isfinite(hthr) && hthr > 0.f && band_ok) {
        const int64_t NTn = e->Npad / 32;
        FC_TRY(screen_item_table(e, NTn, n_lblocks, false, 32));
        unsigned long long n_items = (unsigned long long)NTn * (unsigned long long)n_lblocks;
        const uint64_t *item_table_dev = nullptr;
        if (e->item_total > 0) n_items = (unsigned long long)e->item_total, item_table_dev = e->item_table.as<uint64_t>();
        if (n_items >= (1ull << 31)) return set_error(FC_E_LIMIT, "too many screen items for one launch");
        auto *cnt = reinterpret_cast<unsigned long long *>(e->counters.p);
        const float tiny_floor = std::max(4.0f * hthr, (float)e->A);
#define FC_LAUNCH_H2N(KS2_)                                                                                                 \
  do {                                                                                                                      \
    const void *fn_ = reinterpret_cast<const void *>(k_simbits_screen_mfma_h2<KS2_, false, 32>);                            \
    FC_HIP_TRY(hipFuncSetAttribute(fn_, hipFuncAttributeMaxDynamicSharedMemorySize, (int)lds_n));                           \
    hipLaunchKernelGGL((k_simbits_screen_mfma_h2<KS2_, false, 32>), dim3((unsigned)n_items), dim3(256), lds_n, ctx().stream, \
                       e->Xh.as<h8_t>(), e->G.as<double>(), e->N, e->Npad, hthr, tiny_floor, (float)s2, bdn, (int)e->row_block, \
                       e->rank, e->world, nullptr, e->W, e->cand.as<uint32_t>(), cnt, e->pairq.as<uint64_t>(),              \
                       (unsigned long long)e->pairq_cap, item_table_dev, n_items);                                          \
  } while (0)
        switch (KS2n) {
          case 7: FC_LAUNCH_H2N(7); break;
          case 8: FC_LAUNCH_H2N(8); break;
          case 9: FC_LAUNCH_H2N(9); break;
          case 10: FC_LAUNCH_H2N(10); break;
          case 11: FC_LAUNCH_H2N(11); break;
          case 12: FC_LAUNCH_H2N(12); break;
          default: FC_LAUNCH_H2N(13); break;
        }
#undef FC_LAUNCH_H2N
        FC_TRY(check_launch("k_simbits_screen_mfma_h2<narrow>"));
        e->item_key[3] = -1;
        g_last_screen = 16;
        mark_main();
        return FC_OK;
      }
    }
  }
  {
    const int64_t A4n = (e->A + 3) / 4 * 4;
    const char *f32_env_n = getenv("FC_SCREEN_F32");
    const size_t lds_wide = (size_t)A4n * 3 * 64 * sizeof(float) + (64 + (size_t)e->row_block) * sizeof(float) + kStageBytesF32;
    const size_t lds_n = (size_t)A4n * 3 * 32 * sizeof(float) + (32 + (size_t)e->row_block) * sizeof(float) + kStageBytesF32;
    const KabschF32Bounds bfn = kabsch_f32_bounds(A4n);
    if (!want_valu && e->lean && lds_wide > kLdsLimit && lds_n <= kLdsLimit && (g_screen_forced == 0 || g_screen_forced == 32) &&
        !(f32_env_n && f32_env_n[0] == '0') && e->row_block % 32 == 0 && bfn.p0 < 2.0e-3f &&
        (uint64_t)A4n * 3 * (uint64_t)e->Npad < (1ull << 32)) {
      if (e->g_max < 0.0) {
        auto *cnt_max = reinterpret_cast<unsigned long long *>(e->counters.p) + (kCounters - 1);
        FC_HIP_TRY(hipMemsetAsync(cnt_max, 0, sizeof(unsigned long long), ctx().stream));
        hipLaunchKernelGGL(k_max_nonneg, dim3((unsigned)std::min<int64_t>(ceil_div(e->Npad, 256), 256)), dim3(256), 0, ctx().stream,
                           e->G.as<double>(), e->Npad, cnt_max);
        FC_TRY(check_launch("k_max_nonneg"));
        unsigned long long bits_max = 0;
        FC_TRY(d2h(&bits_max, cnt_max, sizeof bits_max));
        FC_TRY(sync());
        FC_HIP_TRY(hipMemsetAsync(cnt_max, 0, sizeof(unsigned long long), ctx().stream));
        std::memcpy(&e->g_max, &bits_max, sizeof(double));
      }
      static const double kBandMaxF = [] {
        const char *v = getenv("FC_SCREEN_BAND_MAX");
        const double x = v ? atof(v) : 4.0;
        return x > 0.0 ? x : 4.0;
      }();
      const double band_f = (double)bfn.p0 * 2.0 * e->g_max / (double)e->A;
      const bool band_ok = g_screen_forced == 32 || (f32_env_n && (f32_env_n[0] == '2' || f32_env_n[0] == '3')) || band_f <= kBandMaxF * thr2_margin;
      if (band_ok && std::isfinite(e->g_max)) {
        if (!e->xsf_valid) {
          const int64_t n = A4n * 3 * e->Npad;
          FC_TRY(e->Xsf.reserve((size_t)n * sizeof(float)));
          hipLaunchKernelGGL(k_f64_to_f32, dim3((unsigned)ceil_div(n, 256)), dim3(256), 0, ctx().stream, e->Xs.as<double>(), n,
                             e->Xsf.as<float>());
          FC_TRY(check_launch("k_f64_to_f32"));
          FC_TRY(e->sub.reserve((size_t)e->Npad * 8 * sizeof(float)));
          hipLaunchKernelGGL(k_subset_stats, dim3((unsigned)ceil_div(e->Npad, 256)), dim3(256), 0, ctx().stream, e->Xs.as<double>(),
                             e->Npad, (int)e->A, e->sub.as<float>());
          FC_TRY(check_launch("k_subset_stats"));
          e->xsf_valid = true;
        }
        const int64_t NTn = e->Npad / 32;
        FC_TRY(screen_item_table(e, NTn, n_lblocks, false, 32));
        unsigned long long n_items = (unsigned long long)NTn * (unsigned long long)n_lblocks;
        const uint64_t *item_table_dev = nullptr;
        if (e->item_total > 0) n_items = (unsigned long long)e->item_total, item_table_dev = e->item_table.as<uint64_t>();
        if (n_items >= (1ull << 31)) return set_error(FC_E_LIMIT, "too many screen items for one launch");
        auto *cnt = reinterpret_cast<unsigned long long *>(e->counters.p);
        const void *fn_ = reinterpret_cast<const void *>(k_simbits_screen_mfma_f32<4, false, false, 32>);
        FC_HIP_TRY(hipFuncSetAttribute(fn_, hipFuncAttributeMaxDynamicSharedMemorySize, (int)lds_n));
        hipLaunchKernelGGL((k_simbits_screen_mfma_f32<4, false, false, 32>), dim3((unsigned)n_items), dim3(256), lds_n, ctx().stream,
                           e->Xsf.as<float>(), e->G.as<double>(), e->N, e->Npad, (int)e->A, A_thr2, bfn, (int)e->row_block, e->rank,
                           e->world, nullptr, e->W, e->cand.as<uint32_t>(), cnt, e->pairq.as<uint64_t>(),
                           (unsigned long long)e->pairq_cap, item_table_dev, n_items, nullptr, bfn, 0.f, nullptr, 0, 0);
        FC_TRY(check_launch("k_simbits_screen_mfma_f32<narrow>"));
        e->item_key[3] = -1;
        g_last_screen = 32;
        mark_main();
        return FC_OK;
      }
    }
  }
  {
    const size_t lds_m = ((size_t)((e->A + 3) / 4) * 4 * 3 * 64 + 64 + (size_t)e->row_block) * sizeof(double) + kStageBytes;
    const bool fits32 = (uint64_t)((e->A + 3) / 4 * 4) * 3 * (uint64_t)e->Npad < (1ull << 32);
    const bool two_blocks_fit = 2 * lds_m <= kLdsLimit;
    const bool mfma64_ok = fits32 && 96 * (uint64_t)e->Npad < (1ull << 32)  &&
                           lds_m <= kLdsLimit && e->row_block % (two_blocks_fit ? 64 : 128) == 0;
    const int64_t A4s = (e->A + 3) / 4 * 4, KS2s = (e->A + 31) / 32;
    const bool single_ok = fits32 && e->row_block % 64 == 0 &&
                           ((size_t)A4s * 3 * 64 * sizeof(float) + (64 + (size_t)e->row_block) * sizeof(float) + kStageBytesF32 <= kLdsLimit ||
                            (KS2s <= kH2MaxKS2 && (size_t)KS2s * 24 * 1024 + (64 + (size_t)e->row_block) * sizeof(float) + kStageBytesF32 <= kLdsLimit));
    bool done = true;
    auto mfma_path = [&]() -> int {
      auto *cnt = reinterpret_cast<unsigned long long *>(e->counters.p);
      const bool two_blocks = 2 * lds_m <= kLdsLimit;
      const void *fn = two_blocks ? reinterpret_cast<const void *>(k_simbits_screen_mfma<4>)
                                  : reinterpret_cast<const void *>(k_simbits_screen_mfma<8>);
      if (mfma64_ok && lds_m > 64 * 1024) {
        hipError_t err = hipFuncSetAttribute(fn, hipFuncAttributeMaxDynamicSharedMemorySize, (int)lds_m);
        if (err != hipSuccess)
          return set_error(FC_E_HIP, "hipFuncSetAttribute(LDS=%zu) failed: %s", lds_m,
                           hipGetErrorString(err));
      }
      if (mfma64_ok && getenv("FC_DEBUG")) {
        int nb = -1;
        (void)hipOccupancyMaxActiveBlocksPerMultiprocessor(&nb, fn, two_blocks ? 256 : 512, lds_m);
        fprintf(stderr, "[fc] screen_mfma<%d>: LDS %zu B, occupancy API says %d blocks/CU\n",
                two_blocks ? 4 : 8, lds_m, nb);
      }
      unsigned long long n_items = (unsigned long long)NT * (unsigned long long)n_lblocks;
      const uint64_t *item_table_dev = nullptr;
      static int use_v2 = -1;
      if (use_v2 < 0) {
        const char *v = getenv("FC_SCREEN_V2");
        use_v2 = (v && v[0] == '1') ? 1 : 0;
      }
      const bool want_v2 = use_v2 && mfma64_ok && two_blocks && e->row_block == 128;
      FC_TRY(screen_item_table(e, NT, n_lblocks, !want_v2));
      if (e->item_total > 0) {
        n_items = (unsigned long long)e->item_total;
        item_table_dev = e->item_table.as<uint64_t>();
      }
      if (n_items >= (1ull << 31)) return set_error(FC_E_LIMIT, "too many screen items for one launch");
      const dim3 mgrid((unsigned)n_items);
      double *dbg = nullptr;
      const unsigned long long *gate = nullptr;
#ifdef FC_TIMELINE
      static DevBuf tlbuf;
      const bool timeline = two_blocks && getenv("FC_TIMELINE_OUT") != nullptr;
      if (timeline) {
        FC_TRY(tlbuf.reserve(n_items * 4 * sizeof(unsigned long long)));
        FC_HIP_TRY(hipMemsetAsync(tlbuf.p, 0, n_items * 4 * sizeof(unsigned long long), ctx().stream));
        dbg = tlbuf.as<double>();
      }
#endif
      if (want_v2 && e->item_total > 0 && dbg == nullptr) {
        const size_t tile = (size_t)((e->A + 3) / 4) * 4 * 3 * 64 * sizeof(double);
        const size_t lds2 = 2 * tile + (size_t)(2 * 64 + 128) * sizeof(double) + kStageBytes;
        if (lds2 <= kLdsLimit) {
          FC_HIP_TRY(hipFuncSetAttribute(reinterpret_cast<const void *>(k_screen_rowsweep),
                                         hipFuncAttributeMaxDynamicSharedMemorySize, (int)lds2));
          const unsigned wgs = (unsigned)std::min<unsigned long long>((unsigned long long)ctx().n_cu,
                                                                      (unsigned long long)e->item_total);
          hipLaunchKernelGGL(k_screen_rowsweep, dim3(wgs), dim3(512), lds2, ctx().stream, e->Xs.as<double>(),
                             e->G.as<double>(), e->N, e->Npad, (int)e->A, A_thr2, e->rank, e->world,
                             e->bits.as<uint64_t>(), e->W, e->cand.as<uint32_t>(), cnt, e->pairq.as<uint64_t>(),
                             (unsigned long long)e->pairq_cap, e->item_table.as<uint64_t>(),
                             (unsigned long long)e->item_total);
          g_last_screen = 64;
          mark_main();
          return check_launch("k_screen_rowsweep");
        }
      }
      const char *f32_env = g_screen_forced == 64 ? "0" : (g_screen_forced == 32 || g_screen_forced == 16) ? "2" : getenv("FC_SCREEN_F32");
      const int64_t A4 = (e->A + 3) / 4 * 4;
      auto ensure_gmax = [&]() -> int {
        if (e->g_max >= 0.0) return FC_OK;
        auto *cnt_max = reinterpret_cast<unsigned long long *>(e->counters.p) + (kCounters - 1);
        FC_HIP_TRY(hipMemsetAsync(cnt_max, 0, sizeof(unsigned long long), ctx().stream));
        hipLaunchKernelGGL(k_max_nonneg, dim3((unsigned)std::min<int64_t>(ceil_div(e->Npad, 256), 256)), dim3(256), 0,
                           ctx().stream, e->G.as<double>(), e->Npad, cnt_max);
        FC_TRY(check_launch("k_max_nonneg"));
        unsigned long long bits_max = 0;
        FC_TRY(d2h(&bits_max, cnt_max, sizeof bits_max));
        FC_TRY(sync());
        FC_HIP_TRY(hipMemsetAsync(cnt_max, 0, sizeof(unsigned long long), ctx().stream));
        std::memcpy(&e->g_max, &bits_max, sizeof(double));
        return FC_OK;
      };
      static const int h2_env = [] {
        const char *v = getenv("FC_SCREEN_H2");
        return v ? atoi(v) : 1;
      }();
      const int64_t KS2 = (e->A + 31) / 32;
      bool use_h2 = false;
      double h2_scale = 1.0;
      const bool f32_allowed = !(f32_env && f32_env[0] == '0') && dbg == nullptr && e->row_block % 64 == 0;
      if (!mfma64_ok && !f32_allowed) {
        done = false;
        return FC_OK;
      }
      if (f32_allowed && h2_env != 0 && g_screen_forced != 32 && KS2 <= kH2MaxKS2 &&
          (uint64_t)(24 * KS2) * (uint64_t)e->Npad < (1ull << 32)) {
        FC_TRY(ensure_gmax());
        bool model_ok = false;
        FC_TRY(h2_model_ok(&model_ok));
        if (model_ok) {
          FC_TRY(ensure_h2_operands(e, &h2_scale));
          const double s2 = h2_scale * h2_scale;
          use_h2 = h2_scale > 0.0 && std::isfinite((float)(0.5 * A_thr2 * s2)) && (float)(0.5 * A_thr2 * s2) > 0.f;
        }
      }
      KabschF32Bounds bd = use_h2 ? kabsch_h2_bounds(KS2) : kabsch_f32_bounds(A4);
      const size_t lds_f32_tile = (size_t)A4 * 3 * 64 * sizeof(float) + (64 + (size_t)e->row_block) * sizeof(float) * 6 + kStageBytesF32;
      bool use_f32 = f32_allowed && bd.p0 < (use_h2 ? 2.5e-3f : 2.0e-3f) && (use_h2 || lds_f32_tile <= kLdsLimit);
      if (g_screen_forced == 16 && !use_h2) return set_error(FC_E_INVALID, "fc_screen_select(16): the split-half screen does not apply to this ensemble");
      bool speculative = f32_env && f32_env[0] == '3';
      if (use_f32 && !(f32_env && (f32_env[0] == '2' || f32_env[0] == '3'))) {
        FC_TRY(ensure_gmax());
        const double band = (double)bd.p0 * 2.0 * e->g_max / (double)e->A;
        static const double kBandMax = [] {
          const char *v = getenv("FC_SCREEN_BAND_MAX");
          const double x = v ? atof(v) : 4.0;
          return x > 0.0 ? x : 4.0;
        }();
        use_f32 = band <= kBandMax * thr2_margin;
        const bool worth_verdict = (double)e->N * (double)e->N > 2.0 * (double)kRefineLanesMin;
        speculative = band > 0.1 * thr2_margin && worth_verdict;
        if (!use_f32 && use_h2 && g_screen_forced != 16 && lds_f32_tile <= kLdsLimit) {
          const KabschF32Bounds bf = kabsch_f32_bounds(A4);
          const double band_f = (double)bf.p0 * 2.0 * e->g_max / (double)e->A;
          if (bf.p0 < 2.0e-3f && band_f <= kBandMax * thr2_margin) {
            use_h2 = false;
            bd = bf;
            use_f32 = true;
            speculative = band_f > 0.1 * thr2_margin && worth_verdict;
          }
        }
      }
      if (!mfma64_ok) {
        if (!use_f32) {
          done = false;
          return FC_OK;
        }
        speculative = false;
      }
      if (use_f32 && use_h2) {
        const size_t lds_h = (size_t)KS2 * 24 * 1024 + (64 + (size_t)e->row_block) * sizeof(float) + kStageBytesF32;
        if (lds_h > kLdsLimit) return set_error(FC_E_LIMIT, "split-half screen: row block of %lld rows does not fit LDS", (long long)e->row_block);
        const double s2 = h2_scale * h2_scale;
        const float hthr = (float)(0.5 * A_thr2 * s2);
        const float tiny_floor = std::max(4.0f * hthr, (float)e->A);
#define FC_LAUNCH_H2(KS2_, BITS_)                                                                                       \
  do {                                                                                                                  \
    const void *fn_ = reinterpret_cast<const void *>(k_simbits_screen_mfma_h2<KS2_, BITS_>);                            \
    if (lds_h > 64 * 1024) FC_HIP_TRY(hipFuncSetAttribute(fn_, hipFuncAttributeMaxDynamicSharedMemorySize, (int)lds_h)); \
    hipLaunchKernelGGL((k_simbits_screen_mfma_h2<KS2_, BITS_>), mgrid, dim3(256), lds_h, ctx().stream, e->Xh.as<h8_t>(), \
                       e->G.as<double>(), e->N, e->Npad, hthr, tiny_floor, (float)s2, bd, (int)e->row_block, e->rank,   \
                       e->world, e->bits.as<uint64_t>(), e->W, e->cand.as<uint32_t>(), cnt, e->pairq.as<uint64_t>(),    \
                       (unsigned long long)e->pairq_cap, item_table_dev, n_items);                                      \
  } while (0)
#define FC_LAUNCH_H2_K(BITS_)                  \
  switch (KS2) {                               \
    case 1: FC_LAUNCH_H2(1, BITS_); break;     \
    case 2: FC_LAUNCH_H2(2, BITS_); break;     \
    case 3: FC_LAUNCH_H2(3, BITS_); break;     \
    case 4: FC_LAUNCH_H2(4, BITS_); break;     \
    case 5: FC_LAUNCH_H2(5, BITS_); break;     \
    default: FC_LAUNCH_H2(6, BITS_); break;    \
  }
#ifdef FC_H2_TIMELINE
        static DevBuf tlbuf;
        const bool h2_timeline = e->lean && getenv("FC_H2_TIMELINE_OUT") != nullptr;
        uint64_t *const bits_saved = e->bits.as<uint64_t>();
        if (h2_timeline) {
          FC_TRY(tlbuf.reserve(n_items * 4 * sizeof(unsigned long long)));
          FC_HIP_TRY(hipMemsetAsync(tlbuf.p, 0, n_items * 4 * sizeof(unsigned long long), ctx().stream));
          e->bits.p = tlbuf.p;
        } else if (e->lean) {
          e->bits.p = nullptr;
        }
#endif
        if (e->lean) {
          FC_LAUNCH_H2_K(false)
        } else {
          FC_LAUNCH_H2_K(true)
        }
#undef FC_LAUNCH_H2_K
#undef FC_LAUNCH_H2
#ifdef FC_H2_TIMELINE
        e->bits.p = bits_saved;
        if (h2_timeline) {
          std::vector<unsigned long long> h(n_items * 4);
          FC_HIP_TRY(hipMemcpyAsync(h.data(), tlbuf.p, n_items * 4 * sizeof(unsigned long long), hipMemcpyDeviceToHost, ctx().stream));
          FC_HIP_TRY(hipStreamSynchronize(ctx().stream));
          if (FILE *f = fopen(getenv("FC_H2_TIMELINE_OUT"), "wb")) {
            fwrite(h.data(), sizeof(unsigned long long), h.size(), f);
            fclose(f);
          }
        }
#endif
        FC_TRY(check_launch("k_simbits_screen_mfma_h2"));
        mark_main();
        g_last_screen = 16;
      } else if (use_f32) {
        static const int stages_env = [] {
          const char *v = getenv("FC_SCREEN_STAGES");
          return v ? atoi(v) : 0;
        }();
        const bool two = e->lean && stages_env != 1 && A4 >= 16 && e->row_block <= 256;
        const size_t lds_f = (size_t)A4 * 3 * 64 * sizeof(float) + (64 + (size_t)e->row_block) * sizeof(float) * (two ? 6 : 1) +
                             kStageBytesF32;
        if (!e->xsf_valid) {
          const int64_t n = A4 * 3 * e->Npad;
          FC_TRY(e->Xsf.reserve((size_t)n * sizeof(float)));
          hipLaunchKernelGGL(k_f64_to_f32, dim3((unsigned)ceil_div(n, 256)), dim3(256), 0, ctx().stream,
                             e->Xs.as<double>(), n, e->Xsf.as<float>());
          FC_TRY(check_launch("k_f64_to_f32"));
          FC_TRY(e->sub.reserve((size_t)e->Npad * 8 * sizeof(float)));
          hipLaunchKernelGGL(k_subset_stats, dim3((unsigned)ceil_div(e->Npad, 256)), dim3(256), 0, ctx().stream,
                             e->Xs.as<double>(), e->Npad, (int)e->A, e->sub.as<float>());
          FC_TRY(check_launch("k_subset_stats"));
          e->xsf_valid = true;
        }
        if (lds_f > 64 * 1024) {
          FC_HIP_TRY(hipFuncSetAttribute(reinterpret_cast<const void *>(k_simbits_screen_mfma_f32<4, true>),
                                         hipFuncAttributeMaxDynamicSharedMemorySize, (int)lds_f));
          FC_HIP_TRY(hipFuncSetAttribute(reinterpret_cast<const void *>(k_simbits_screen_mfma_f32<4, false>),
                                         hipFuncAttributeMaxDynamicSharedMemorySize, (int)lds_f));
          FC_HIP_TRY(hipFuncSetAttribute(reinterpret_cast<const void *>(k_simbits_screen_mfma_f32<4, false, true>),
                                         hipFuncAttributeMaxDynamicSharedMemorySize, (int)lds_f));
        }
        const int64_t KS_all = A4 / 4, KS1 = (KS_all + 1) / 2;
        int64_t A_S = 0;
        for (int64_t a = 0; a < e->A; ++a) A_S += ((a >> 2) & 1) ? 0 : 1;
        const KabschF32Bounds bd1 = kabsch_f32_bounds(4 * KS1 + 8);
        const float inv_AS = (float)(1.0 / (double)std::max<int64_t>(A_S, 1));
        const float *sub_dev = two ? e->sub.as<float>() : nullptr;
        if (two) {
          const unsigned long long units_per_item = (unsigned long long)(e->row_block / 16) * 2ull;
          FC_TRY(e->unitq.reserve((size_t)(n_items * units_per_item) * sizeof(uint64_t)));
          const unsigned long long n_sample = (n_items + 15ull) / 16ull, n_rest = n_items - n_sample;
          const unsigned long long max_sample_units = n_sample * units_per_item / 3ull;
#define FC_LAUNCH_F32_LEAN(GRID, SUB, PART, GATE, STAGED_)                                                            \
  hipLaunchKernelGGL((k_simbits_screen_mfma_f32<4, false, STAGED_>), dim3((unsigned)(GRID)), dim3(256), lds_f, ctx().stream, \
                     e->Xsf.as<float>(), e->G.as<double>(), e->N, e->Npad, (int)e->A, A_thr2, bd, (int)e->row_block,  \
                     e->rank, e->world, e->bits.as<uint64_t>(), e->W, e->cand.as<uint32_t>(), cnt,                    \
                     e->pairq.as<uint64_t>(), (unsigned long long)e->pairq_cap, item_table_dev, n_items, SUB, bd1,    \
                     inv_AS, e->unitq.as<uint64_t>(), PART, GATE)
          FC_LAUNCH_F32_LEAN(n_sample, sub_dev, 1, 0, true);
          hipLaunchKernelGGL(k_screen_density_verdict, dim3(1), dim3(64), 0, ctx().stream, cnt, max_sample_units);
          if (n_rest > 0) FC_LAUNCH_F32_LEAN(n_rest, sub_dev, 2, 1, true);
          FC_TRY(check_launch("k_simbits_screen_mfma_f32<subset stage>"));
          hipLaunchKernelGGL(k_screen_units_f32, dim3((unsigned)(ctx().n_cu * 3)), dim3(256), 0, ctx().stream,
                             e->Xsf.as<float>(), e->G.as<double>(), e->N, e->Npad, (int)e->A, A_thr2, bd,
                             e->unitq.as<uint64_t>(), cnt, e->pairq.as<uint64_t>(), (unsigned long long)e->pairq_cap);
          FC_TRY(check_launch("k_screen_units_f32"));
          FC_LAUNCH_F32_LEAN(n_items, nullptr, 0, 2, false);
#undef FC_LAUNCH_F32_LEAN
        } else if (e->lean)
          hipLaunchKernelGGL((k_simbits_screen_mfma_f32<4, false>), mgrid, dim3(256), lds_f, ctx().stream,
                             e->Xsf.as<float>(), e->G.as<double>(), e->N, e->Npad, (int)e->A, A_thr2, bd,
                             (int)e->row_block, e->rank, e->world, e->bits.as<uint64_t>(), e->W,
                             e->cand.as<uint32_t>(), cnt, e->pairq.as<uint64_t>(),
                             (unsigned long long)e->pairq_cap, item_table_dev, n_items, nullptr, bd1, inv_AS, nullptr, 0, 0);
        else
          hipLaunchKernelGGL((k_simbits_screen_mfma_f32<4, true>), mgrid, dim3(256), lds_f, ctx().stream,
                             e->Xsf.as<float>(), e->G.as<double>(), e->N, e->Npad, (int)e->A, A_thr2, bd,
                             (int)e->row_block, e->rank, e->world, e->bits.as<uint64_t>(), e->W,
                             e->cand.as<uint32_t>(), cnt, e->pairq.as<uint64_t>(),
                             (unsigned long long)e->pairq_cap, item_table_dev, n_items, nullptr, bd1, inv_AS, nullptr, 0, 0);
        FC_TRY(check_launch("k_simbits_screen_mfma_f32"));
        mark_main();
        g_last_screen = 32;
      }
      if (use_f32) {
        if (!speculative) return FC_OK;
        const double owned_pairs = 0.5 * (double)e->N * (double)e->N / (double)e->world;
        const auto max_false = (unsigned long long)std::max(1024.0, 0.015 * ((double)A4 / 52.0) * owned_pairs);
        hipLaunchKernelGGL(k_screen_verdict, dim3(4), dim3(256), 0, ctx().stream, e->Xa.as<double>(),
                           e->G.as<double>(), (int)e->A, A_thr2, e->pairq.as<uint64_t>(),
                           (unsigned long long)e->pairq_cap, max_false, cnt, ctx().optimistic_screen ? 1 : 0);
        FC_TRY(check_launch("k_screen_verdict"));
        if (ctx().optimistic_screen) return FC_OK;
        gate = cnt + 11;
      }
      if (two_blocks)
        hipLaunchKernelGGL(k_simbits_screen_mfma<4>, mgrid, dim3(256), lds_m, ctx().stream,
                           e->Xs.as<double>(), e->G.as<double>(), e->N, e->Npad, (int)e->A, A_thr2,
                           (int)e->row_block, e->rank, e->world, e->bits.as<uint64_t>(), e->W,
                           e->cand.as<uint32_t>(), cnt, e->pairq.as<uint64_t>(),
                           (unsigned long long)e->pairq_cap, item_table_dev, n_items, dbg, gate);
      else
        hipLaunchKernelGGL(k_simbits_screen_mfma<8>, mgrid, dim3(512), lds_m, ctx().stream,
                           e->Xs.as<double>(), e->G.as<double>(), e->N, e->Npad, (int)e->A, A_thr2,
                           (int)e->row_block, e->rank, e->world, e->bits.as<uint64_t>(), e->W,
                           e->cand.as<uint32_t>(), cnt, e->pairq.as<uint64_t>(),
                           (unsigned long long)e->pairq_cap, item_table_dev, n_items, dbg, gate);
      if (gate == nullptr) g_last_screen = 64;
      FC_TRY(check_launch("k_simbits_screen_mfma"));
      mark_main();
#ifdef FC_TIMELINE
      if (timeline) {
        std::vector<unsigned long long> h(n_items * 4);
        FC_HIP_TRY(hipMemcpyAsync(h.data(), tlbuf.p, n_items * 4 * sizeof(unsigned long long),
                                  hipMemcpyDeviceToHost, ctx().stream));
        FC_HIP_TRY(hipStreamSynchronize(ctx().stream));
        if (FILE *f = fopen(getenv("FC_TIMELINE_OUT"), "wb")) {
          fwrite(h.data(), sizeof(unsigned long long), h.size(), f);
          fclose(f);
        }
      }
#endif
      return FC_OK;
    };
    if (!want_valu && (mfma64_ok || single_ok)) {
      FC_TRY(mfma_path());
      if (done) return FC_OK;
    }
  }
#define FC_LAUNCH_SCREEN(LDSFLAG, TI_, NW_, SMEM)                                                   \
  hipLaunchKernelGGL((k_simbits_screen<LDSFLAG, TI_, NW_>), grid, dim3(NW_ * 64), SMEM,            \
                     ctx().stream, e->Xs.as<double>(), e->G.as<double>(), e->N, e->Npad,           \
                     (int)e->A, A_thr2, (int)e->row_block, e->rank, e->world,                      \
                     e->bits.as<uint64_t>(), e->W, e->cand.as<uint32_t>(),                         \
                     reinterpret_cast<unsigned long long *>(e->counters.p),                        \
                     e->pairq.as<uint64_t>(), (unsigned long long)e->pairq_cap)
  if (lds <= kLdsLimit) {
    const void *fn = alt ? reinterpret_cast<const void *>(k_simbits_screen<true, 4, 8>)
                         : reinterpret_cast<const void *>(k_simbits_screen<true, 8, 4>);
    if (lds > 64 * 1024) {
      hipError_t err = hipFuncSetAttribute(fn, hipFuncAttributeMaxDynamicSharedMemorySize, (int)lds);
      if (err != hipSuccess)
        return set_error(FC_E_HIP, "hipFuncSetAttribute(LDS=%zu) failed: %s", lds,
                         hipGetErrorString(err));
    }
    if (alt) FC_LAUNCH_SCREEN(true, 4, 8, lds);
    else FC_LAUNCH_SCREEN(true, 8, 4, lds);
  } else {
    if (alt) FC_LAUNCH_SCREEN(false, 4, 8, 0);
    else FC_LAUNCH_SCREEN(false, 8, 4, 0);
  }
#undef FC_LAUNCH_SCREEN
  g_last_screen = 1;
  mark_main();
  return check_launch("k_simbits_screen");
}

int launch_simbits_refine(fc_ensemble *e, double max_rmsd, double max_dev, const double *energies_dev,
                          double max_dE) {
  if (e->rows_local * e->W == 0) return FC_OK;
  static const bool lanes = [] {
    const char *v = getenv("FC_REFINE_LANES");
    return !(v && atoi(v) == 0);
  }();
  static const bool buckets = [] {
    const char *v = getenv("FC_REFINE_BUCKETS");
    return !(v && atoi(v) == 0);
  }();
  const size_t lds_bk = (size_t)(((e->A + 3) & ~(int64_t)3) * 3 * (1 << kBucketColShift)) * sizeof(double);
  static const size_t lds_bk_static = [] {
    hipFuncAttributes fa{};
    return hipFuncGetAttributes(&fa, reinterpret_cast<const void *>(k_refine_buckets)) == hipSuccess ? (size_t)fa.sharedSizeBytes
                                                                                                        : (size_t)(16 * 1024);
  }();
  static const bool debug_form = getenv("FC_DEBUG") != nullptr;
  const bool bucket_form = lanes && buckets && e->bk_buckets > 0 && lds_bk + lds_bk_static <= kLdsLimit &&
                           e->last_candidates > (int64_t)kRefineLanesMin;
  if (debug_form)
    fprintf(stderr, "[fc] refine form: %s (last prune seen: %lld candidates, %lld similar)\n",
            bucket_form ? "bucket sort + k_refine_buckets" : (lanes ? "k_refine_pairs / k_simbits_refine" : "k_simbits_refine"),
            (long long)e->last_candidates, (long long)e->last_similar);
  if (bucket_form) {
    auto *cnt = reinterpret_cast<unsigned long long *>(e->counters.p);
    const unsigned NT = (unsigned)(e->Npad >> kBucketColShift);
    const BucketGeom geom{NT, (NT + 7) / 8};
    const int64_t nb = e->bk_buckets;
// ... 79 lines not shown
```

### include/fc_hip.h

```cpp
#ifndef FC_HIP_H
#define FC_HIP_H

#include <stdint.h>

#ifdef __cplusplus
extern "C" {
#endif

#define FC_OK 0
#define FC_E_INVALID (-1)
#define FC_E_NODEVICE (-2)
#define FC_E_HIP (-3)
#define FC_E_NOMEM (-4)
#define FC_E_LIMIT (-5)

int fc_abi_version(void);
int fc_device_count(void);
int fc_init(int device);
int fc_shutdown(void);
const char *fc_last_error(void);
int fc_warmup(void);
int fc_stream_set(void *hip_stream);
int fc_stream_use(void *hip_stream);
int fc_memory_trim(void);
// ... 27 lines not shown
int fc_prune_rmsd(fc_ensemble *ens, double max_rmsd, double max_dev, const double *energies,
                  double max_dE, int64_t min_per_group, uint8_t *mask_out, int64_t *stats);
int fc_prune_rmsd_host(const double *coords, int64_t N, int64_t A, const uint8_t *atom_mask, int center, double max_rmsd,
                       double max_dev, const double *energies, double max_dE, int64_t min_per_group, uint8_t *mask_out,
                       int64_t *stats);
int fc_prune_conventions(int drop_later);
int fc_greedy_prune_from_bits(const uint64_t *bits, int64_t N, int64_t min_per_group,
                              uint8_t *mask_out);

int fc_prune_rmsd_begin(fc_ensemble *ens, double max_rmsd, double max_dev,
                        const double *energies, double max_dE, int64_t rank, int64_t world,
                        int64_t row_block, int64_t *stats);
int fc_prune_level(fc_ensemble *ens, int64_t k, const uint8_t *mask_in, uint8_t *mask_out);
int fc_prune_similar_pairs(fc_ensemble *ens, uint64_t *pairs_out, int64_t capacity, int64_t *n_out);
int fc_prune_from_pairs(fc_ensemble *ens, const uint64_t *pairs, int64_t n_pairs,
                        int64_t min_per_group, uint8_t *mask_out);
int fc_prune_rmsd_begin_async(fc_ensemble *ens, double max_rmsd, double max_dev, int64_t rank,
                              int64_t world, int64_t row_block);
int fc_prune_export_pairs_dev(fc_ensemble *ens, uint64_t *dev_out, int64_t cap);
int fc_prune_from_gathered_dev(fc_ensemble *ens, const uint64_t *dev_gathered, int64_t world,
                               int64_t cap, int64_t min_per_group, uint8_t *mask_out, int64_t *stats);
int fc_prune_from_gathered_dev_enqueue(fc_ensemble *ens, const uint64_t *dev_gathered, int64_t world,
                                       int64_t cap, int64_t min_per_group, int64_t slot, int64_t n_slots);
int fc_prune_collect(fc_ensemble *ens, int64_t slot, int64_t n_slots, uint8_t *mask_out, int64_t *stats);
int fc_ensemble_twin(fc_ensemble *ens, fc_ensemble **twin_out);
int fc_prune_rmsd_begin_split_async(fc_ensemble *ens, double max_rmsd, double max_dev, int64_t rank,
                                    int64_t world, int64_t row_block, void *screen_stream, int timed);

#define FC_COMM_ID_BYTES 128
int fc_comm_unique_id(uint8_t *id_out);
int fc_comm_init(int64_t rank, int64_t world, const uint8_t *id);
int fc_comm_destroy(void);
int fc_comm_info(int64_t *rank, int64_t *world);
int fc_allgather_mask(const uint8_t *mask_local, int64_t n_local, uint8_t *mask_global);
int fc_allgather_u8_dev(const uint8_t *send_dev, uint8_t *recv_dev, int64_t bytes_per_rank);
int fc_comm_barrier(void);
int fc_debug_comm_loopback(int64_t rank, int64_t world);
int fc_prune_rmsd_sharded(fc_ensemble *ens, double max_rmsd, double max_dev, int64_t min_per_group,
                          int64_t row_block, uint8_t *mask_out, int64_t *stats);

int fc_prune_rmsd_rot_corr(const double *coords, int64_t N, int64_t A, const uint8_t *heavy_mask,
                           const int64_t *torsions, int64_t T, const uint8_t *rotation_masks,
                           const double *angles, const int32_t *n_angles, int64_t max_angles,
                           double max_rmsd, double max_dev, const double *energies, double max_dE,
                           int64_t min_per_group, uint8_t *mask_out, uint64_t *bits_out);

int fc_align_by_moi(const double *coords, int64_t N, int64_t A, const double *masses, double *out);

int fc_inertia_moments(const double *coords, int64_t N, int64_t A, const double *masses,
                       double *moments_out);
int fc_prune_moi(const double *coords, int64_t N, int64_t A, const double *masses,
                 double max_deviation, const double *energies, double max_dE,
                 int64_t min_per_group, uint8_t *mask_out);

int fc_prune_similarity(const double *coords, int64_t N, int64_t A, const uint8_t *heavy_mask, const double *masses,
                        int do_moi, double moi_tol, int do_rmsd, double max_rmsd, double max_dev,
                        const double *energies, double max_dE, int64_t min_per_group, uint8_t *mask_moi_out,
                        uint8_t *mask_out, int64_t *counts);

int fc_align_to_first(const double *coords, int64_t N, int64_t A, const int64_t *idx,
                      int64_t n_idx, double *out);

int fc_rototranslate(const double *coords, int64_t n, int64_t A, const double *R,
                     const double *t, double *out);

int fc_clash_self(const double *coords, int64_t N, int64_t A, double lo, double hi,
                  int64_t *counts_out);
int fc_clash_fragments(const double *coords, int64_t N, int64_t A, const int64_t *ids,
                       int64_t n_ids, double thresh, int64_t max_clashes,
                       int64_t *counts_out, uint8_t *pass_out);

int fc_clash_graph(const double *coords, int64_t N, int64_t A, const uint8_t *adj, double thresh,
                   int64_t *counts_out);
int fc_fitness_check(const double *coords, int64_t N, int64_t A, const int64_t *pairs,
                     const double *targets, int64_t C, double threshold, double *error_out,
                     uint8_t *pass_out);

int fc_embed_poses_clash(const double *m1, int64_t n1, int64_t A1, const double *m2,
                         int64_t n2, int64_t A2, const int64_t *c1, const int64_t *c2,
                         const double *R1, const double *t1, const double *R2,
                         const double *t2, int64_t P, double thresh, int64_t max_clashes,
                         int64_t *counts_out, uint8_t *pass_out, double *poses_out);

int fc_embed_mol_transforms(const double *coords, int64_t n, int64_t A, const int64_t *reactive,
                            int64_t nr, const double *pivot_start, const double *pivot_end,
                            int64_t mol, const double *angles, int64_t na, double *R_out,
                            double *t_out);
int fc_embed_grid_clash(const double *m1, int64_t n1, int64_t A1, const int64_t *reactive1,
                        int64_t nr1, const double *ps1, const double *pe1, const double *m2,
                        int64_t n2, int64_t A2, const int64_t *reactive2, int64_t nr2,
                        const double *ps2, const double *pe2, const double *angles1, int64_t na1,
                        const double *angles2, int64_t na2, double thresh, int64_t max_clashes,
                        uint8_t *pass_out, int32_t *counts_out, double *ms_kernel);
int fc_embed_grid_dedupe(const double *m1, int64_t n1, int64_t A1, const int64_t *reactive1,
                         int64_t nr1, const double *ps1, const double *pe1, const double *m2,
                         int64_t n2, int64_t A2, const int64_t *reactive2, int64_t nr2,
                         const double *ps2, const double *pe2, const double *angles1, int64_t na1,
                         const double *angles2, int64_t na2, double thresh, int64_t max_clashes,
                         double rmsd_thr, uint8_t *pass_out, uint8_t *accept_out);

int fc_embed_trimolecular(const double *const coords[3], const int64_t n_conf[3], const int64_t n_atoms[3],
                          const int64_t *const reactive[3], const int64_t n_reactive[3], int64_t J,
                          const int64_t *conf, const double *piv_start, const double *piv_end,
                          const double *vecs, const double *dirs0, const uint8_t *run, const int64_t *rtab,
                          const double *norms, const double *ua, int64_t U, const int32_t *aidx, int64_t S,
                          double thresh, int64_t max_clashes, double rmsd_thr, double *dirs_out,
                          double *Rt_out, uint8_t *pass_out, uint8_t *accept_out);

int fc_string_embed(const double *m1, int64_t n1, int64_t A1, const double *centers1,
                    const double *orbvecs1, int64_t K1, const double *m2, int64_t n2, int64_t A2,
                    const double *centers2, const double *orbvecs2, int64_t K2,
                    const double *angles, int64_t nA, const int64_t *quads, int64_t Q,
                    double thresh, int64_t max_clashes, double tfd_thresh, uint8_t *pass_out,
                    uint8_t *accept_out, double *R2_out, double *t2_out);

int fc_torsion_scan(const double *base, int64_t A, const int64_t *torsions, int64_t T,
                    const uint8_t *rotmasks, const int64_t *angles, int64_t S, double thresh,
                    int64_t backoff_deg, double *coords_out, int64_t *rotated_bonds_out);
int fc_torsion_scan_fingerprints(const double *base, int64_t A, const int64_t *torsions, int64_t T,
                                 const uint8_t *rotmasks, const int64_t *angles, int64_t S, double thresh,
                                 int64_t backoff_deg, const int64_t *quads, int64_t Q, double *tf_out,
                                 int64_t *rotated_bonds_out, double *coords_out);
int fc_torsion_scan_tfd(const double *base, int64_t A, const int64_t *torsions, int64_t T, const uint8_t *rotmasks,
                        const int64_t *angles, int64_t S, double thresh, int64_t backoff_deg, const int64_t *quads,
                        int64_t Q, double tfd_thresh, int64_t *rotated_bonds_out, uint8_t *keep_out);
int fc_torsion_scan_tfd_grid(const double *base, int64_t A, const int64_t *torsions, int64_t T, const uint8_t *rotmasks,
                             const int64_t *values, const int64_t *counts, double thresh, int64_t backoff_deg,
                             const int64_t *quads, int64_t Q, double tfd_thresh, int64_t *rotated_bonds_out, uint8_t *keep_out);

int fc_torsion_fingerprint(const double *coords, int64_t N, int64_t A, const int64_t *quads,
                           int64_t Q, double *tf_out);
int fc_tfd_simbits(const double *tf, int64_t N, int64_t Q, double thresh, int64_t row_begin,
                   int64_t row_end, uint64_t *bits_out);

int fc_tfd_first_match(const double *tf, int64_t N, int64_t Q, double thresh, int64_t *first_out);
int fc_tfd_ladder_from_first_match(const int64_t *first_match, int64_t N, uint8_t *mask_out);
int fc_tfd_prune(const double *tf, int64_t N, int64_t Q, double thresh, uint8_t *mask_out);
int fc_debug_pyset_order_ints(const int64_t *keys, int64_t n, int64_t *order_out, int64_t *n_out);
int fc_debug_pyset_order_pairs(const int64_t *pairs, int64_t n, int64_t *order_out, int64_t *n_out);
int fc_debug_pyset_order_pairs_device(const int64_t *pairs, int64_t n, int64_t *order_out);
int fc_debug_tfd_ladder_emulate(const int64_t *first_match, int64_t N, uint8_t *mask_out);

int fc_xyz_write(const char *path, const char *const *atoms, int64_t A, const double *coords,
                 int64_t N, const char *label, int mode);
int fc_xyz_scan(const char *path, int64_t *N_out, int64_t *A_out);
int fc_cartesian_product_i64(const int64_t *values, const int64_t *counts, int64_t T, int64_t *out);
int fc_cartesian_product_f64(const double *values, const int64_t *counts, int64_t T, double *out);
int fc_xyz_read(const char *path, int64_t N, int64_t A, char *atoms_out, double *coords_out);

int fc_prune_rmsd_many(fc_ensemble *const *ens, int64_t n, double max_rmsd, double max_dev,
                       int64_t min_per_group, uint8_t *const *mask_out, int64_t *survivors_out);

int fc_screen_last_kind(void);
int fc_screen_select(int kind);
int fc_debug_mfma_f16_model(int64_t trials, int64_t *flags_out, double *worst_out);
int fc_debug_h2_covariance(fc_ensemble *ens, int64_t ib, int64_t jb, float *B_out, double *scale_out,
                           double *entry_bound_out);
int fc_bench_prune_rmsd(fc_ensemble *ens, double max_rmsd, double max_dev, int64_t reps,
                        double *ms_simbits_kernel, double *ms_step, uint8_t *mask_out,
                        int64_t *stats);
int fc_bench_refine(fc_ensemble *ens, double max_rmsd, double max_dev, int64_t reps, double *ms_refine,
                    int64_t *n_candidates);
int fc_bench_rmsd_and_max_all(fc_ensemble *ens, int64_t reps, double *ms_kernel_mean, double *ms_total,
                              int64_t *stats);
int fc_bench_rmsd_and_max_all_sampled(fc_ensemble *ens, int64_t reps, const int64_t *pair_i, const int64_t *pair_j,
                                      int64_t P, double *rmsd_out, double *maxdev_out, double *ms_kernel_mean,
                                      double *ms_total, int64_t *stats);
int fc_bench_select_diverse(fc_ensemble *ens, int64_t n_max, int64_t start, double stop_rmsd, int64_t reps,
                            double *ms_device_mean, double *ms_host_mean, int64_t *indices_out, int64_t *n_selected,
                            int64_t *lanes_out);
int fc_bench_prune_rmsd_sharded(fc_ensemble *ens, double max_rmsd, double max_dev, int64_t reps, int overlap,
                                double *ms_screen_kernel, double *ms_step, uint8_t *mask_out, int64_t *stats);

#ifdef __cplusplus
}
#endif
#endif
```

Before: 19.47 billion.

## Add f32 max-deviation pass with exact f64 recheck of top atoms

The complete-alignment kernel (EIG mode, 32-column tile) now computes per-atom squared deviations in packed f32. It tracks the top three atoms with tagged med3/max, then recomputes only the top one or two atoms exactly in f64. A rigorous error bound decides per wave whether to fall back to the full f64 atom loop. This replaces most of the f64 per-atom work with cheaper f32 math, but adds LDS for f32 coordinates, an extra global-to-LDS load, and a wave-level fallback path. Stats counters and a query API are added.

```diff
diff --git a/firecode_amd/_lib.py b/firecode_amd/_lib.py
--- a/firecode_amd/_lib.py
+++ b/firecode_amd/_lib.py
@@ -126,6 +126,7 @@
     "fc_ensemble_twin": [_ens, C.POINTER(_ens)],
     "fc_prune_rmsd_begin_split_async": [_ens, _f64, _f64, _i64, _i64, _i64, C.c_void_p, C.c_int],
     "fc_screen_last_kind": [],
+    "fc_complete_f32pass_stats": [_ens, _p_i64],
     "fc_debug_mfma_f16_model": [_i64, _p_i64, _p_f64],
     "fc_debug_h2_covariance": [_ens, _i64, _i64, C.POINTER(C.c_float), _p_f64, _p_f64],
     "fc_comm_unique_id": [_p_u8],
@@ -439,6 +440,11 @@
         call("fc_bench_rmsd_and_max_all", self.handle, int(reps), C.byref(k), C.byref(t), pi(stats))
         return k.value, t.value, stats
 
+    def complete_f32pass_stats(self):
+        stats = np.zeros(3, dtype=np.int64)
+        call("fc_complete_f32pass_stats", self.handle, pi(stats))
+        return stats
+
     def bench_rmsd_and_max_all_sampled(self, pair_i, pair_j, reps=1):
         pi_, pj_ = i64(pair_i), i64(pair_j)
         P = int(pi_.shape[0])
diff --git a/firecode_amd/csrc/fc_api.cpp b/firecode_amd/csrc/fc_api.cpp
--- a/firecode_amd/csrc/fc_api.cpp
+++ b/firecode_amd/csrc/fc_api.cpp
@@ -1053,6 +1053,7 @@
   FC_HIP_TRY(hipEventRecord(c.ev1, c.stream));
   if (tiled) FC_TRY(d2h(cnt, ens->counters.p, sizeof cnt));
   FC_TRY(sync());
+  if (tiled) ens->f32p_last[1] = (int64_t)cnt[5], ens->f32p_last[2] = (int64_t)cnt[7];
   if (ms_kernel) {
     float ms = 0.f;
     FC_HIP_TRY(hipEventElapsedTime(&ms, c.ev0, c.ev1));
@@ -1116,6 +1117,7 @@
   unsigned long long cnt[16] = {0};
   if (tiled) FC_TRY(d2h(cnt, ens->counters.p, sizeof cnt));
   FC_TRY(sync());
+  if (tiled) ens->f32p_last[1] = (int64_t)cnt[5], ens->f32p_last[2] = (int64_t)cnt[7];
   double sum = 0.0;
   for (int64_t r = 0; r < reps; ++r) {
     float ms = 0.f;
@@ -3009,6 +3011,13 @@
 
 int fc_screen_last_kind(void) { return last_screen_kind(); }
 
+int fc_complete_f32pass_stats(fc_ensemble *ens, int64_t *stats_out) {
+  FC_API_LOCK;
+  FC_REQUIRE(ens != nullptr && stats_out != nullptr, "ens / stats_out is NULL");
+  for (int k = 0; k < 3; ++k) stats_out[k] = ens->f32p_last[k];
+  return FC_OK;
+}
+
 int fc_prune_conventions(int drop_later) {
   FC_API_LOCK;
   prune_conventions_set(drop_later);
diff --git a/firecode_amd/csrc/fc_common.h b/firecode_amd/csrc/fc_common.h
--- a/firecode_amd/csrc/fc_common.h
+++ b/firecode_amd/csrc/fc_common.h
@@ -247,6 +247,7 @@
   fc::DevBuf sub;
   fc::DevBuf unitq;
   bool xsf_valid = false;
+  int64_t f32p_last[3] = {0, 0, 0};
   fc::DevBuf Xh;
   bool xh_valid = false;
   double xh_scale = 0.0;
diff --git a/firecode_amd/csrc/fc_kabsch.hip b/firecode_amd/csrc/fc_kabsch.hip
--- a/firecode_amd/csrc/fc_kabsch.hip
+++ b/firecode_amd/csrc/fc_kabsch.hip
@@ -548,8 +548,103 @@
 }
 
 typedef double d4_t __attribute__((ext_vector_type(4)));
-
-template <int NW, int MODE = 0, int TC = 64, bool EIG = false>
+typedef float f2_t __attribute__((ext_vector_type(2)));
+typedef float f4_t __attribute__((ext_vector_type(4)));
+
+__device__ __forceinline__ void f32p_top3_push(float s, unsigned keep, unsigned tag, float &m1, float &m2, float &m3) {
+  float st;
+  asm("v_bfi_b32 %0, %1, %2, %3" : "=v"(st) : "v"(keep), "v"(s), "s"(tag));
+  asm("v_med3_f32 %0, %1, %2, %3" : "=v"(m3) : "v"(m2), "v"(m3), "v"(st));
+  asm("v_med3_f32 %0, %1, %2, %3" : "=v"(m2) : "v"(m1), "v"(m2), "v"(st));
+  asm("v_max_f32 %0, %1, %2" : "=v"(m1) : "v"(m1), "v"(st));
+}
+
+__device__ __forceinline__ void f32p_atom_pass(const float *__restrict__ qf, const float *__restrict__ prow, unsigned l15u,
+                                               int64_t Npad, int A, const double (&nR)[4][9], float (&m1)[4], float (&m2)[4],
+                                               float (&m3)[4]) {
+  f2_t R2[2][9];
+#pragma unroll
+  for (int h = 0; h < 2; ++h)
+#pragma unroll
+    for (int e = 0; e < 9; ++e) R2[h][e] = f2_t{(float)nR[2 * h][e], (float)nR[2 * h + 1][e]};
+#pragma unroll
+  for (int r = 0; r < 4; ++r) m1[r] = -1.f, m2[r] = -1.f, m3[r] = -1.f;
+  unsigned keep = 0xffffff80u;
+  asm volatile("" : "+v"(keep));
+  const int64_t Npad3 = 3 * Npad;
+  const float *__restrict__ pa0 = prow, *__restrict__ pa1 = prow + Npad, *__restrict__ pa2 = prow + 2 * Npad;
+  const float *__restrict__ qg = qf;
+  auto load = [&](auto u_, float (&P)[3], f4_t (&Q)[3]) {
+    constexpr int u = decltype(u_)::value;
+#pragma unroll
+    for (int c = 0; c < 3; ++c) Q[c] = *reinterpret_cast<const f4_t *>(qg + c * 128 + u * 16);
+    P[0] = pa0[l15u];
+    P[1] = pa1[l15u];
+    P[2] = pa2[l15u];
+    pa0 += Npad3;
+    pa1 += Npad3;
+    pa2 += Npad3;
+  };
+  auto track = [&](unsigned tag, const float (&P)[3], const f4_t (&Q)[3]) {
+    const f2_t px = f2_t{P[0], P[0]}, py = f2_t{P[1], P[1]}, pz = f2_t{P[2], P[2]};
+    f2_t s2[2];
+#pragma unroll
+    for (int h = 0; h < 2; ++h) {
+      const f2_t qx = h ? Q[0].zw : Q[0].xy, qy = h ? Q[1].zw : Q[1].xy, qz = h ? Q[2].zw : Q[2].xy;
+      const f2_t dx = __builtin_elementwise_fma(R2[h][0], qx, __builtin_elementwise_fma(R2[h][1], qy, __builtin_elementwise_fma(R2[h][2], qz, px)));
+      const f2_t dy = __builtin_elementwise_fma(R2[h][3], qx, __builtin_elementwise_fma(R2[h][4], qy, __builtin_elementwise_fma(R2[h][5], qz, py)));
+      const f2_t dz = __builtin_elementwise_fma(R2[h][6], qx, __builtin_elementwise_fma(R2[h][7], qy, __builtin_elementwise_fma(R2[h][8], qz, pz)));
+      s2[h] = __builtin_elementwise_fma(dz, dz, __builtin_elementwise_fma(dy, dy, dx * dx));
+    }
+#pragma unroll
+    for (int r = 0; r < 4; ++r) f32p_top3_push(s2[r >> 1][r & 1], keep, tag, m1[r], m2[r], m3[r]);
+  };
+  using U0 = std::integral_constant<int, 0>;
+  using U1 = std::integral_constant<int, 1>;
+  using U2 = std::integral_constant<int, 2>;
+  using U3 = std::integral_constant<int, 3>;
+  const int n_rounds = (A + 1) >> 1, n_groups = n_rounds >> 1;
+  const bool odd_round = (n_rounds & 1) != 0;
+  float PA[3], PB[3];
+  f4_t QA[3], QB[3];
+  load(U0{}, PA, QA);
+  unsigned tag = 0;
+  for (int g = 0; g < n_groups; ++g, tag += 4) {
+    load(U1{}, PB, QB);
+    __builtin_amdgcn_sched_barrier(0);
+    track(tag, PA, QA);
+    __builtin_amdgcn_sched_barrier(0);
+    load(U2{}, PA, QA);
+    __builtin_amdgcn_sched_barrier(0);
+    track(tag + 1, PB, QB);
+    __builtin_amdgcn_sched_barrier(0);
+    load(U3{}, PB, QB);
+    __builtin_amdgcn_sched_barrier(0);
+    track(tag + 2, PA, QA);
+    __builtin_amdgcn_sched_barrier(0);
+    qg += 384;
+    if (g + 1 < n_groups || odd_round) load(U0{}, PA, QA);
+    __builtin_amdgcn_sched_barrier(0);
+    track(tag + 3, PB, QB);
+    __builtin_amdgcn_sched_barrier(0);
+  }
+  if (odd_round) {
+    load(U1{}, PB, QB);
+    __builtin_amdgcn_sched_barrier(0);
+    track(tag, PA, QA);
+    __builtin_amdgcn_sched_barrier(0);
+    track(tag + 1, PB, QB);
+  }
+}
+
+__device__ __forceinline__ float f32p_limit(float T, float GG) {
+  const float eta = 8.f * 5.9604645e-08f * 1.001f * __builtin_amdgcn_sqrtf(GG);
+  const float sigma = (__builtin_amdgcn_sqrtf(fmaxf(T, 0.f)) + 6.f * eta) * 1.0001f;
+  const float E = 2.f * 1.7320508f * eta * sigma + 3.f * eta * eta + (3.f * 5.9604645e-08f + 1.5258789e-05f) * sigma * sigma + 1e-37f;
+  return T - 2.02f * E;
+}
+
+template <int NW, int MODE = 0, int TC = 64, bool EIG = false, bool F32P = false>
 __global__ void __launch_bounds__(NW * 64, 2)
 k_simbits_screen_mfma(const double *__restrict__ Xs, const double *__restrict__ G, int64_t N,
                       int64_t Npad, int A, double A_thr2, int IB, int64_t rank, int64_t world,
@@ -557,8 +652,9 @@
                       unsigned long long *__restrict__ counters, uint64_t *__restrict__ pairq,
                       unsigned long long Q, const uint64_t *__restrict__ item_table, unsigned long long n_items,
                       double *__restrict__ rmsd_out = nullptr, const unsigned long long *__restrict__ gate = nullptr,
-                      double *__restrict__ maxdev_out = nullptr) {
+                      double *__restrict__ maxdev_out = nullptr, const float *__restrict__ Xsf = nullptr) {
   static_assert(!EIG || MODE == 2, "EIG: the complete alignments");
+  static_assert(!F32P || (MODE == 2 && TC == 32 && EIG), "F32P: the complete alignments with the 32-column tile and the eigenvalue");
   constexpr bool VALUES = MODE != 0;
   constexpr int NT = MODE == 2 ? 1 : 2;
   static_assert(TC == 64 || ((TC == 32 || TC == 16) && MODE == 2), "column tiles: 64, or 32 / 16 for the complete alignments");
@@ -577,6 +673,9 @@
   uint64_t *__restrict__ stageQ = reinterpret_cast<uint64_t *>(ldsG + TC + IB);
   uint32_t *__restrict__ stageW = reinterpret_cast<uint32_t *>(stageQ + kStagePairs);
   unsigned *__restrict__ stageN = reinterpret_cast<unsigned *>(stageW + kStageWords);
+  float *__restrict__ ldsF = reinterpret_cast<float *>(
+      reinterpret_cast<char *>(lds) + ((reinterpret_cast<char *>(stageN + 2) - reinterpret_cast<char *>(lds) + 15) & ~(ptrdiff_t)15));
+  (void)ldsF;
 #ifdef FC_TIMELINE
   unsigned long long *tl = reinterpret_cast<unsigned long long *>(rmsd_out);
 #endif
@@ -625,6 +724,17 @@
       __builtin_amdgcn_global_load_lds((const __attribute__((address_space(1))) void *)src,
                                        (__attribute__((address_space(3))) void *)(lds + q * 128), 16, 0, 0);
     }
+    if constexpr (F32P) {
+      const int n_runs_f = KS * 3;
+      const int l31 = lane & 31, cs_f = l31 >> 4, k_f = (l31 >> 2) & 3, c4_f = (l31 & 3) * 4;
+      for (int h = wv; 2 * h < n_runs_f; h += NW) {
+        const int qr = 2 * h + (lane >> 5) < n_runs_f ? 2 * h + (lane >> 5) : n_runs_f - 1;
+        const int sg = qr / 3, c = qr - sg * 3;
+        const float *src = Xsf + (int64_t)((sg * 4 + k_f) * 3 + c) * Npad + j0 + cs_f * 16 + c4_f;
+        __builtin_amdgcn_global_load_lds((const __attribute__((address_space(1))) void *)src,
+                                         (__attribute__((address_space(3))) void *)(ldsF + h * 256), 16, 0, 0);
+      }
+    }
     for (int idx = tid; idx < TC + IB; idx += NW * 64) {
       const int64_t g = idx < TC ? j0 + idx : i0 + (idx - TC);
       ldsG[idx] = g < Npad ? G[g] : 0.0;
@@ -632,6 +742,7 @@
     if (tid < kStagePairs) stageQ[tid] = ~0ull;
     if (tid < kStageWords) stageW[tid] = ~0u;
     if (tid < 2) stageN[tid] = 0u;
+    if constexpr (F32P) __builtin_amdgcn_s_waitcnt(0x0f70);
     __syncthreads();
 #ifdef FC_TIMELINE
     if (!VALUES && tl && tid == 0) tl[(size_t)b * 4 + 1] = wall_clock64();
@@ -788,72 +899,146 @@
           const double *__restrict__ qcol = lds + cs * SST + 4 * kq;
           const double *__restrict__ prow_u = Xs + ib;
           const unsigned l15u = (unsigned)l15;
-          const int n_rounds = (A + 1) >> 1, n_groups = n_rounds >> 1;
-          const bool odd_round = (n_rounds & 1) != 0;
           double ssq[4] = {0.0, 0.0, 0.0, 0.0}, mx[4] = {0.0, 0.0, 0.0, 0.0};
-          const int64_t Npad3 = 3 * Npad;
-          const double *__restrict__ pa0 = prow_u, *__restrict__ pa1 = prow_u + Npad, *__restrict__ pa2 = prow_u + 2 * Npad;
-          const double *__restrict__ qg = qcol;
-          auto load_pq = [&](auto u_, double (&P)[3], d2_t (&Qv)[3][2]) {
-            constexpr int u = decltype(u_)::value;
-            const double *__restrict__ ql = qg + (u / KPR) * 128 + (u % KPR) * 16;
-#pragma unroll
-            for (int c = 0; c < 3; ++c) {
-              Qv[c][0] = *reinterpret_cast<const d2_t *>(ql + c * CST);
-              Qv[c][1] = *reinterpret_cast<const d2_t *>(ql + c * CST + 2);
+          bool full64 = !F32P;
+          if constexpr (F32P) {
+            float m1[4], m2[4], m3[4];
+            f32p_atom_pass(ldsF + cs * SST + 4 * kq, Xsf + ib, l15u, Npad, A, nR, m1, m2, m3);
+            bool need2[4], any2 = false, any3 = false;
+#pragma unroll
+            for (int r = 0; r < 4; ++r) {
+              const float GGr = (float)(Gp + ldsG[cs * 16 + 4 * kq + r]);
+              const float lim = f32p_limit(m1[r], GGr);
+              const int j = jb + r;
+              const bool valid = i < n32 && j > i && j < n32 && ok4[r];
+              need2[r] = valid && !(m2[r] < lim);
+              any2 |= need2[r];
+              any3 |= valid && (!(m3[r] < lim) || !(GGr >= 1e-20f && GGr <= 1e30f) || !(m1[r] <= 3.0e38f));
             }
-            P[0] = pa0[l15u];
-            P[1] = pa1[l15u];
-            P[2] = pa2[l15u];
-            pa0 += Npad3;
-            pa1 += Npad3;
-            pa2 += Npad3;
-          };
-          auto accumulate = [&](const double (&P)[3], const d2_t (&Qv)[3][2]) {
+            full64 = __builtin_amdgcn_ballot_w64(any3) != 0ull;
+            const bool two = !full64 && __builtin_amdgcn_ballot_w64(any2) != 0ull;
+            if (lane == 0 && two) atomicAdd(&counters[5], 1ull);
+            if (lane == 0 && full64) atomicAdd(&counters[7], 1ull);
+            if (!full64) {
+              const char *__restrict__ xrow = reinterpret_cast<const char *>(Xs + ib);
+              const unsigned npad8 = (unsigned)Npad * 8u;
+              auto atom_of = [&](float tagged) {
+                const unsigned a = __float_as_uint(tagged) & 127u;
+                return a < (unsigned)A ? a : (unsigned)A - 1u;
+              };
+              auto fetch_row = [&](unsigned a, double (&P)[3]) {
+                unsigned off = (a * 3u) * npad8 + l15u * 8u;
+#pragma unroll
+                for (int c = 0; c < 3; ++c) {
+                  asm volatile("" : "+v"(off));
+                  P[c] = *reinterpret_cast<const double *>(xrow + off);
+                  off += npad8;
+                }
+              };
+              auto exact_s2 = [&](auto r_, unsigned a, const double (&P)[3]) -> double {
 #pragma clang fp contract(fast)
-#pragma unroll
-            for (int r = 0; r < 4; ++r) {
-              const double qx = Qv[0][r >> 1][r & 1], qy = Qv[1][r >> 1][r & 1], qz = Qv[2][r >> 1][r & 1];
-              const double dx = fma(nR[r][0], qx, fma(nR[r][1], qy, fma(nR[r][2], qz, P[0])));
-              const double dy = fma(nR[r][3], qx, fma(nR[r][4], qy, fma(nR[r][5], qz, P[1])));
-              const double dz = fma(nR[r][6], qx, fma(nR[r][7], qy, fma(nR[r][8], qz, P[2])));
-              const double s2 = fma(dz, dz, fma(dy, dy, dx * dx));
-              if constexpr (!EIG) ssq[r] += s2;
-              asm("v_max_f64 %0, %1, %2" : "=v"(mx[r]) : "v"(mx[r]), "v"(s2));
+                constexpr int r = decltype(r_)::value;
+                const double *__restrict__ qq = qcol + (a >> 2) * (12 * TC) + (a & 3) * 16 + r;
+                const double qx = qq[0], qy = qq[CST], qz = qq[2 * CST];
+                const double dx = fma(nR[r][0], qx, fma(nR[r][1], qy, fma(nR[r][2], qz, P[0])));
+                const double dy = fma(nR[r][3], qx, fma(nR[r][4], qy, fma(nR[r][5], qz, P[1])));
+                const double dz = fma(nR[r][6], qx, fma(nR[r][7], qy, fma(nR[r][8], qz, P[2])));
+                return fma(dz, dz, fma(dy, dy, dx * dx));
+              };
+              using R0 = std::integral_constant<int, 0>;
+              using R1 = std::integral_constant<int, 1>;
+              using R2 = std::integral_constant<int, 2>;
+              using R3 = std::integral_constant<int, 3>;
+              unsigned w1[4], w2[4];
+              double P1[4][3], P2[4][3];
+#pragma unroll
+              for (int r = 0; r < 4; ++r) {
+                w1[r] = atom_of(m1[r]);
+                w2[r] = atom_of(m2[r]);
+                fetch_row(w1[r], P1[r]);
+                fetch_row(w2[r], P2[r]);
+              }
+              __builtin_amdgcn_sched_barrier(0);
+              mx[0] = exact_s2(R0{}, w1[0], P1[0]);
+              mx[1] = exact_s2(R1{}, w1[1], P1[1]);
+              mx[2] = exact_s2(R2{}, w1[2], P1[2]);
+              mx[3] = exact_s2(R3{}, w1[3], P1[3]);
+              if (two) {
+                const double s2[4] = {exact_s2(R0{}, w2[0], P2[0]), exact_s2(R1{}, w2[1], P2[1]), exact_s2(R2{}, w2[2], P2[2]),
+                                      exact_s2(R3{}, w2[3], P2[3])};
+#pragma unroll
+                for (int r = 0; r < 4; ++r)
+                  if (need2[r] && s2[r] > mx[r]) mx[r] = s2[r];
+              }
             }
-          };
-          using U0 = std::integral_constant<int, 0>;
-          using U1 = std::integral_constant<int, 1>;
-          using U2 = std::integral_constant<int, 2>;
-          using U3 = std::integral_constant<int, 3>;
-          double PA[3], PB[3];
-          d2_t QA[3][2], QB[3][2];
-          load_pq(U0{}, PA, QA);
-          for (int g = 0; g < n_groups; ++g) {
-            load_pq(U1{}, PB, QB);
-            __builtin_amdgcn_sched_barrier(0);
-            accumulate(PA, QA);
-            __builtin_amdgcn_sched_barrier(0);
-            load_pq(U2{}, PA, QA);
-            __builtin_amdgcn_sched_barrier(0);
-            accumulate(PB, QB);
-            __builtin_amdgcn_sched_barrier(0);
-            load_pq(U3{}, PB, QB);
-            __builtin_amdgcn_sched_barrier(0);
-            accumulate(PA, QA);
-            __builtin_amdgcn_sched_barrier(0);
-            qg = TC == 16 ? qcol + koff(g + 1) : qg + 12 * TC;
-            if (g + 1 < n_groups || odd_round) load_pq(U0{}, PA, QA);
-            __builtin_amdgcn_sched_barrier(0);
-            accumulate(PB, QB);
-            __builtin_amdgcn_sched_barrier(0);
           }
-          if (odd_round) {
-            load_pq(U1{}, PB, QB);
-            __builtin_amdgcn_sched_barrier(0);
-            accumulate(PA, QA);
-            __builtin_amdgcn_sched_barrier(0);
-            accumulate(PB, QB);
+          if (full64) {
+            const int n_rounds = (A + 1) >> 1, n_groups = n_rounds >> 1;
+            const bool odd_round = (n_rounds & 1) != 0;
+            const int64_t Npad3 = 3 * Npad;
+            const double *__restrict__ pa0 = prow_u, *__restrict__ pa1 = prow_u + Npad, *__restrict__ pa2 = prow_u + 2 * Npad;
+            const double *__restrict__ qg = qcol;
+            auto load_pq = [&](auto u_, double (&P)[3], d2_t (&Qv)[3][2]) {
+              constexpr int u = decltype(u_)::value;
+              const double *__restrict__ ql = qg + (u / KPR) * 128 + (u % KPR) * 16;
+#pragma unroll
+              for (int c = 0; c < 3; ++c) {
+                Qv[c][0] = *reinterpret_cast<const d2_t *>(ql + c * CST);
+                Qv[c][1] = *reinterpret_cast<const d2_t *>(ql + c * CST + 2);
+              }
+              P[0] = pa0[l15u];
+              P[1] = pa1[l15u];
+              P[2] = pa2[l15u];
+              pa0 += Npad3;
+              pa1 += Npad3;
+              pa2 += Npad3;
+            };
+            auto accumulate = [&](const double (&P)[3], const d2_t (&Qv)[3][2]) {
+#pragma clang fp contract(fast)
+#pragma unroll
+              for (int r = 0; r < 4; ++r) {
+                const double qx = Qv[0][r >> 1][r & 1], qy = Qv[1][r >> 1][r & 1], qz = Qv[2][r >> 1][r & 1];
+                const double dx = fma(nR[r][0], qx, fma(nR[r][1], qy, fma(nR[r][2], qz, P[0])));
+                const double dy = fma(nR[r][3], qx, fma(nR[r][4], qy, fma(nR[r][5], qz, P[1])));
+                const double dz = fma(nR[r][6], qx, fma(nR[r][7], qy, fma(nR[r][8], qz, P[2])));
+                const double s2 = fma(dz, dz, fma(dy, dy, dx * dx));
+                if constexpr (!EIG) ssq[r] += s2;
+                asm("v_max_f64 %0, %1, %2" : "=v"(mx[r]) : "v"(mx[r]), "v"(s2));
+              }
+            };
+            using U0 = std::integral_constant<int, 0>;
+            using U1 = std::integral_constant<int, 1>;
+            using U2 = std::integral_constant<int, 2>;
+            using U3 = std::integral_constant<int, 3>;
+            double PA[3], PB[3];
+            d2_t QA[3][2], QB[3][2];
+            load_pq(U0{}, PA, QA);
+            for (int g = 0; g < n_groups; ++g) {
+              load_pq(U1{}, PB, QB);
+              __builtin_amdgcn_sched_barrier(0);
+              accumulate(PA, QA);
+              __builtin_amdgcn_sched_barrier(0);
+              load_pq(U2{}, PA, QA);
+              __builtin_amdgcn_sched_barrier(0);
+              accumulate(PB, QB);
+              __builtin_amdgcn_sched_barrier(0);
+              load_pq(U3{}, PB, QB);
+              __builtin_amdgcn_sched_barrier(0);
+              accumulate(PA, QA);
+              __builtin_amdgcn_sched_barrier(0);
+              qg = TC == 16 ? qcol + koff(g + 1) : qg + 12 * TC;
+              if (g + 1 < n_groups || odd_round) load_pq(U0{}, PA, QA);
+              __builtin_amdgcn_sched_barrier(0);
+              accumulate(PB, QB);
+              __builtin_amdgcn_sched_barrier(0);
+            }
+            if (odd_round) {
+              load_pq(U1{}, PB, QB);
+              __builtin_amdgcn_sched_barrier(0);
+              accumulate(PA, QA);
+              __builtin_amdgcn_sched_barrier(0);
+              accumulate(PB, QB);
+            }
           }
           if constexpr (EIG) {
 #pragma unroll
@@ -2893,19 +3078,34 @@
   return screen_item_table(e, e->Npad >> 6, n_lblocks, true, 64);
 }
 
-template <int NW, int TC, bool EIG>
+static int ensure_xsf(fc_ensemble *e) {
+  if (e->xsf_valid) return FC_OK;
+  const int64_t n = (e->A + 3) / 4 * 4 * 3 * e->Npad;
+  FC_TRY(e->Xsf.reserve((size_t)n * sizeof(float)));
+  hipLaunchKernelGGL(k_f64_to_f32, dim3((unsigned)ceil_div(n, 256)), dim3(256), 0, ctx().stream, e->Xs.as<double>(), n,
+                     e->Xsf.as<float>());
+  FC_TRY(check_launch("k_f64_to_f32"));
+  FC_TRY(e->sub.reserve((size_t)e->Npad * 8 * sizeof(float)));
+  hipLaunchKernelGGL(k_subset_stats, dim3((unsigned)ceil_div(e->Npad, 256)), dim3(256), 0, ctx().stream, e->Xs.as<double>(),
+                     e->Npad, (int)e->A, e->sub.as<float>());
+  FC_TRY(check_launch("k_subset_stats"));
+  e->xsf_valid = true;
+  return FC_OK;
+}
+
+template <int NW, int TC, bool EIG, bool F32P = false>
 static int launch_complete_variant(fc_ensemble *e, dim3 grid, size_t lds_m, double A_small, int64_t rb, int64_t rank, int64_t world,
                                    unsigned long long *cnt, const uint64_t *item_table_dev, unsigned long long n_items,
                                    double *rmsd_dev, double *maxdev_dev) {
   if (lds_m > 64 * 1024) {
-    hipError_t err = hipFuncSetAttribute(reinterpret_cast<const void *>(k_simbits_screen_mfma<NW, 2, TC, EIG>),
+    hipError_t err = hipFuncSetAttribute(reinterpret_cast<const void *>(k_simbits_screen_mfma<NW, 2, TC, EIG, F32P>),
                                          hipFuncAttributeMaxDynamicSharedMemorySize, (int)lds_m);
     if (err != hipSuccess) return set_error(FC_E_HIP, "hipFuncSetAttribute failed: %s", hipGetErrorString(err));
   }
-  hipLaunchKernelGGL((k_simbits_screen_mfma<NW, 2, TC, EIG>), grid, dim3(NW * 64), lds_m, ctx().stream, e->Xs.as<double>(),
+  hipLaunchKernelGGL((k_simbits_screen_mfma<NW, 2, TC, EIG, F32P>), grid, dim3(NW * 64), lds_m, ctx().stream, e->Xs.as<double>(),
                      e->G.as<double>(), e->N, e->Npad, (int)e->A, A_small, (int)rb, rank, world, nullptr, e->W, nullptr, cnt,
                      e->pairq.as<uint64_t>(), (unsigned long long)e->pairq_cap, item_table_dev, n_items, rmsd_dev, nullptr,
-                     maxdev_dev);
+                     maxdev_dev, F32P ? e->Xsf.as<float>() : nullptr);
   return FC_OK;
 }
 
@@ -2918,8 +3118,16 @@
   const size_t lds_32 = ((size_t)((e->A + 3) / 4) * 4 * 3 * 32 + 32 + (size_t)rb) * sizeof(double) + kStageBytes;
   const size_t lds_16 = ((size_t)(((e->A + 3) / 4 + 1) / 2) * 384 + 16 + (size_t)rb) * sizeof(double) + kStageBytes;
   const bool narrow = lds_64 > kLdsLimit && maxdev_dev != nullptr;
-  const int64_t tc = !narrow ? 64 : (lds_32 <= kLdsLimit ? 32 : 16);
-  const size_t lds_m = tc == 64 ? lds_64 : (tc == 32 ? lds_32 : lds_16);
+  const bool complete = maxdev_dev != nullptr;
+  const char *eig_env = getenv("FC_COMPLETE_EIG");
+  const bool eig = complete && !(eig_env && atoi(eig_env) == 0) && !explicit_sum;
+  const size_t lds_f32p = ((lds_32 + 15) & ~(size_t)15) + (size_t)((3 * ((e->A + 3) / 4) + 1) / 2) * 1024;
+  const char *f32p_env = getenv("FC_COMPLETE_F32PASS");
+  const bool f32p = eig && !narrow && 2 * lds_f32p <= kLdsLimit && e->A >= 4 && e->A <= 127 && !(f32p_env && atoi(f32p_env) == 0) &&
+                    (uint64_t)((e->A + 3) / 4 * 4) * 3 * (uint64_t)e->Npad * sizeof(double) < (1ull << 32);
+  e->f32p_last[0] = f32p ? 1 : 0;
+  const int64_t tc = f32p ? 32 : !narrow ? 64 : (lds_32 <= kLdsLimit ? 32 : 16);
+  const size_t lds_m = f32p ? lds_f32p : tc == 64 ? lds_64 : (tc == 32 ? lds_32 : lds_16);
   const int64_t NT = e->Npad / tc;
   if (lds_m > kLdsLimit || NT == 0)
     return set_error(FC_E_LIMIT, "A=%lld atoms exceed the LDS column tile of the value kernel", (long long)e->A);
@@ -2928,7 +3136,6 @@
   if (!fits32) return set_error(FC_E_LIMIT, "ensemble too large for 32-bit operand offsets");
   auto *cnt = reinterpret_cast<unsigned long long *>(e->counters.p);
   const bool two_blocks = 2 * lds_m <= kLdsLimit;
-  const bool complete = maxdev_dev != nullptr;
   const void *fn = two_blocks ? reinterpret_cast<const void *>(k_simbits_screen_mfma<4, 1>)
                               : reinterpret_cast<const void *>(k_simbits_screen_mfma<8, 1>);
   if (!complete && lds_m > 64 * 1024) {
@@ -2953,14 +3160,16 @@
                      e->Xs.as<double>(), e->G.as<double>(), e->N, e->Npad, (int)e->A, A_small, (int)rb,   \
                      rank, world, nullptr, e->W, nullptr, cnt, e->pairq.as<uint64_t>(),                   \
                      (unsigned long long)e->pairq_cap, item_table_dev, n_items, rmsd_dev, nullptr, maxdev_dev)
-  const char *eig_env = getenv("FC_COMPLETE_EIG");
-  const bool eig = complete && !(eig_env && atoi(eig_env) == 0) && !explicit_sum;
 #define FC_LAUNCH_COMPLETE(NW_, TC_)                                                                                        \
   FC_TRY((eig ? launch_complete_variant<NW_, TC_, true>(e, grid, lds_m, A_small, rb, rank, world, cnt, item_table_dev, n_items, \
                                                        rmsd_dev, maxdev_dev)                                               \
               : launch_complete_variant<NW_, TC_, false>(e, grid, lds_m, A_small, rb, rank, world, cnt, item_table_dev,     \
                                                         n_items, rmsd_dev, maxdev_dev)))
-  if (narrow && tc == 32) {
+  if (f32p) {
+    FC_TRY(ensure_xsf(e));
+    FC_TRY((launch_complete_variant<4, 32, true, true>(e, grid, lds_m, A_small, rb, rank, world, cnt, item_table_dev, n_items,
+                                                      rmsd_dev, maxdev_dev)));
+  } else if (narrow && tc == 32) {
     FC_LAUNCH_COMPLETE(8, 32);
   } else if (narrow) {
     FC_LAUNCH_COMPLETE(8, 16);
@@ -3251,18 +3460,7 @@
       const double band_f = (double)bfn.p0 * 2.0 * e->g_max / (double)e->A;
       const bool band_ok = g_screen_forced == 32 || (f32_env_n && (f32_env_n[0] == '2' || f32_env_n[0] == '3')) || band_f <= kBandMaxF * thr2_margin;
       if (band_ok && std::isfinite(e->g_max)) {
-        if (!e->xsf_valid) {
-          const int64_t n = A4n * 3 * e->Npad;
-          FC_TRY(e->Xsf.reserve((size_t)n * sizeof(float)));
-          hipLaunchKernelGGL(k_f64_to_f32, dim3((unsigned)ceil_div(n, 256)), dim3(256), 0, ctx().stream, e->Xs.as<double>(), n,
-                             e->Xsf.as<float>());
-          FC_TRY(check_launch("k_f64_to_f32"));
-          FC_TRY(e->sub.reserve((size_t)e->Npad * 8 * sizeof(float)));
-          hipLaunchKernelGGL(k_subset_stats, dim3((unsigned)ceil_div(e->Npad, 256)), dim3(256), 0, ctx().stream, e->Xs.as<double>(),
-                             e->Npad, (int)e->A, e->sub.as<float>());
-          FC_TRY(check_launch("k_subset_stats"));
-          e->xsf_valid = true;
-        }
+        FC_TRY(ensure_xsf(e));
         const int64_t NTn = e->Npad / 32;
         FC_TRY(screen_item_table(e, NTn, n_lblocks, false, 32));
         unsigned long long n_items = (unsigned long long)NTn * (unsigned long long)n_lblocks;
@@ -3495,18 +3693,7 @@
         const bool two = e->lean && stages_env != 1 && A4 >= 16 && e->row_block <= 256;
         const size_t lds_f = (size_t)A4 * 3 * 64 * sizeof(float) + (64 + (size_t)e->row_block) * sizeof(float) * (two ? 6 : 1) +
                              kStageBytesF32;
-        if (!e->xsf_valid) {
-          const int64_t n = A4 * 3 * e->Npad;
-          FC_TRY(e->Xsf.reserve((size_t)n * sizeof(float)));
-          hipLaunchKernelGGL(k_f64_to_f32, dim3((unsigned)ceil_div(n, 256)), dim3(256), 0, ctx().stream,
-                             e->Xs.as<double>(), n, e->Xsf.as<float>());
-          FC_TRY(check_launch("k_f64_to_f32"));
-          FC_TRY(e->sub.reserve((size_t)e->Npad * 8 * sizeof(float)));
-          hipLaunchKernelGGL(k_subset_stats, dim3((unsigned)ceil_div(e->Npad, 256)), dim3(256), 0, ctx().stream,
-                             e->Xs.as<double>(), e->Npad, (int)e->A, e->sub.as<float>());
-          FC_TRY(check_launch("k_subset_stats"));
-          e->xsf_valid = true;
-        }
+        FC_TRY(ensure_xsf(e));
         if (lds_f > 64 * 1024) {
           FC_HIP_TRY(hipFuncSetAttribute(reinterpret_cast<const void *>(k_simbits_screen_mfma_f32<4, true>),
                                          hipFuncAttributeMaxDynamicSharedMemorySize, (int)lds_f));
diff --git a/include/fc_hip.h b/include/fc_hip.h
--- a/include/fc_hip.h
+++ b/include/fc_hip.h
@@ -203,6 +203,7 @@
                        int64_t min_per_group, uint8_t *const *mask_out, int64_t *survivors_out);
 
 int fc_screen_last_kind(void);
+int fc_complete_f32pass_stats(fc_ensemble *ens, int64_t *stats_out);
 int fc_screen_select(int kind);
 int fc_debug_mfma_f16_model(int64_t trials, int64_t *flags_out, double *worst_out);
 int fc_debug_h2_covariance(fc_ensemble *ens, int64_t ib, int64_t jb, float *B_out, double *scale_out,
```

Result: faster. 20.08 billion (median of 6 runs) (+3.1%).
